# caumente/multi_task_breast_cancer

Hardware: AMD Instinct MI355X
Metric: training images/sec (1-ch 256x256, U-Net++ MT) (higher is better)
Workload: dtype bf16; 1 GPU; MTUNetPlusPlus seg+cls deep-supervision step (Dice+Focal, alpha=0.5, Adam eps 1e-4), per-GPU batch 32, 1x256x256, bf16 MFMA operands (3x3 convs, ConvT) and 16-bit stored conv outputs / activations; fp32 accumulation, gradient sums, statistics, losses, parameters and optimizer, random-init weights (BASELINE.json configs[1]); global_batch=32, parallelism=dp1

## Files before the change

### include/mtbc.h

```cpp
#ifndef MTBC_H
#define MTBC_H

#include <stddef.h>
#include <stdint.h>

#ifdef __cplusplus
extern "C" {
#endif

#define MTBC_VERSION 203
#define MTBC_MAX_SEGS 6
#define MTBC_STEM_MAX_CIN 5

enum {
    MTBC_OK = 0,
    MTBC_E_BADSHAPE = -1,
    MTBC_E_BADARG = -2,
    MTBC_E_WORKSPACE = -3,
    MTBC_E_LAUNCH = -4,
    MTBC_E_UNSUPPORTED = -5
};

int mtbc_version(void);
const char* mtbc_strerror(int code);
// ... 57 lines not shown
size_t mtbc_conv3x3_packed_dgrad_elems(int32_t Cin, int32_t Cout);
int mtbc_conv3x3_pack_fwd(const float* w, float* packed, int32_t Cin, int32_t Cout, void* stream);
int mtbc_conv3x3_pack_dgrad(const float* w, float* packed, int32_t Cin, int32_t Cout, void* stream);
size_t mtbc_conv3x3_packed_lp_elems(int32_t Cin, int32_t Cout, int32_t dgrad);
int mtbc_conv3x3_pack_lp(const float* w, void* packed, int32_t Cin, int32_t Cout, int32_t dgrad, int32_t compute, void* stream);

typedef struct mtbc_pack_desc {
    const float* w;
    void* packed;
    int32_t Cin, Cout;
    int32_t kind, compute;
} mtbc_pack_desc;
int mtbc_conv3x3_pack_many(const mtbc_pack_desc* descs, int32_t n, void* stream);
int32_t mtbc_conv3x3_stats_slots(const mtbc_conv3x3_args* a);
size_t mtbc_conv3x3_wgrad_workspace(const mtbc_conv3x3_args* a);
size_t mtbc_conv3x3_wgrad_sync_bytes(const mtbc_conv3x3_args* a);
int mtbc_conv3x3_kernel_name(const mtbc_conv3x3_args* a, int32_t op, char* buf, int32_t len);
int mtbc_conv3x3_fwd(const mtbc_conv3x3_args* a, void* stream);
int mtbc_conv3x3_dgrad(const mtbc_conv3x3_args* a, void* stream);
int mtbc_conv3x3_wgrad(const mtbc_conv3x3_args* a, void* stream);

typedef struct {
    int32_t N, C, H, W;
    float eps, slope;
    const float* z;
    const float* gamma;
    const float* beta;
    float* y;
    int64_t y_batch_stride;
    float* mean;
    float* rstd;
    const float* dy;
    int64_t dy_batch_stride;
    int32_t n_dy_extra;
    const float* dy_extra[4];
    float* dz;
    float* dgamma;
    float* dbeta;
    float* dbias_pre;
    int32_t accumulate_dparams;
    void* workspace;
    size_t workspace_bytes;
    void* y16;
    void* dz16;
    int32_t out16_type;
    void* y8;
    void* dz8;
    void* coop_state;
    int32_t coop_reserve_cus;
    int32_t z_layout;
    int32_t dy_layout;
    const float* stats_partial;
    int32_t stats_slots;
    int32_t z_type;
    const float* dy_rank1;
    const float* dy_rank1_w;
    float* dy_rank1_dw;
    float* dy_rank1_db;
    int32_t dy_rank1_accumulate;
    const float* dy_pool;
    const void* dy_pool_arg;
    void* pool_y8;
    void* pool_arg;
    int32_t defer_dparams;
} mtbc_instnorm_args;
size_t mtbc_instnorm_coop_state_bytes(void);
size_t mtbc_instnorm_coop_error_offset(void);
int mtbc_instnorm_c8_supported(const mtbc_instnorm_args* a, int32_t backward);
int32_t mtbc_instnorm_bwd_team(const mtbc_instnorm_args* a);
typedef struct mtbc_dparam_desc {
    const float* part;
    float* dgamma;
    float* dbeta;
    float* dbias_pre;
    int32_t N, C, T, accumulate;
} mtbc_dparam_desc;
int mtbc_instnorm_dparam_many(const mtbc_dparam_desc* descs, int32_t n, void* stream);

size_t mtbc_instnorm_fwd_workspace(const mtbc_instnorm_args* a);
int mtbc_instnorm_kernel_name(const mtbc_instnorm_args* a, int32_t backward, char* buf, int32_t len);
int mtbc_instnorm_lrelu_fwd(const mtbc_instnorm_args* a, void* stream);
int mtbc_instnorm_lrelu_bwd(const mtbc_instnorm_args* a, void* stream);

typedef struct {
    int32_t N, C, H, W;
    const float* x;  int64_t x_batch_stride;
    float* y;        int64_t y_batch_stride;
    const float* dy; int64_t dy_batch_stride;
    float* dx;       int64_t dx_batch_stride;
    int32_t accumulate_dx;
    int32_t layout;
    int32_t type16;
    void* argmax;
} mtbc_maxpool_args;

int mtbc_maxpool2_fwd(const mtbc_maxpool_args* a, void* stream);
int mtbc_maxpool2_bwd(const mtbc_maxpool_args* a, void* stream);

typedef struct {
    int32_t N, C, H, W;
    const void* x;   int64_t x_batch_stride;
    void* y;         int64_t y_batch_stride;
    int32_t layout;
    int32_t type16;
    const float* dy; int64_t dy_batch_stride;
    float* dx;       int64_t dx_batch_stride;
    int32_t accumulate_dx;
} mtbc_upsample2_args;
int mtbc_upsample2_fwd(const mtbc_upsample2_args* a, void* stream);
int mtbc_upsample2_bwd(const mtbc_upsample2_args* a, void* stream);

typedef struct {
    int32_t N, H, W, Cin, Cout, k;
    const float* x;  int64_t x_batch_stride;
    const float* w;
    const float* bias;
    float* y;        int64_t y_batch_stride;
    const float* dy; int64_t dy_batch_stride;
    float* dx;       int64_t dx_batch_stride;
    int32_t accumulate_dx;
    float* dw;       float* dbias;
    int32_t accumulate_dw;
    void* workspace; size_t workspace_bytes;
    int32_t compute;
    int32_t y_layout;
    int32_t y_type;
    int32_t x_layout;
    int32_t dy_type16;
    int32_t x_type16;
} mtbc_convT_args;
int mtbc_convT_fwd_c8_supported(const mtbc_convT_args* a);

size_t mtbc_convT_wgrad_workspace(const mtbc_convT_args* a);
int mtbc_convT_fwd(const mtbc_convT_args* a, void* stream);
int mtbc_convT_dgrad(const mtbc_convT_args* a, void* stream);
int mtbc_convT_wgrad(const mtbc_convT_args* a, void* stream);
int mtbc_convT_kernel_name(const mtbc_convT_args* a, int32_t op, const mtbc_convT_args* dgrad_next, char* buf, int32_t len);

typedef struct {
    int32_t N, H, W, Cin, Cout;
    const float* x;  int64_t x_batch_stride;
    const float* w;
    const float* bias;
    float* y;
    const float* dy;
    float* dx;       int64_t dx_batch_stride;
    int32_t accumulate_dx;
    float* dw;       float* dbias;
    int32_t accumulate_dw;
    void* workspace; size_t workspace_bytes;
    int32_t x_layout;
    int32_t x_type;
} mtbc_conv1x1_args;

size_t mtbc_conv1x1_wgrad_workspace(const mtbc_conv1x1_args* a);
int mtbc_conv1x1_fwd(const mtbc_conv1x1_args* a, void* stream);
int mtbc_conv1x1_dgrad(const mtbc_conv1x1_args* a, void* stream);
int mtbc_conv1x1_wgrad(const mtbc_conv1x1_args* a, void* stream);

typedef struct {
    int32_t N, C, H, W;
    const float* x;  float* y;
    const float* dy; float* dx;
} mtbc_gap_args;
int mtbc_gap_fwd(const mtbc_gap_args* a, void* stream);
int mtbc_gap_bwd(const mtbc_gap_args* a, void* stream);
// ... 293 lines not shown
```

### multi_task_breast_cancer_amd/_lib.py

```python
from __future__ import annotations

import ctypes as C
import os
from typing import Optional

_HERE = os.path.dirname(os.path.abspath(__file__))
LIB_PATH = os.environ.get("MTBC_LIB") or os.path.join(_HERE, "libmtbc_hip.so")

MAX_SEGS = 6
STEM_MAX_CIN = 5
c_float_p = C.POINTER(C.c_float)


class MtbcError(RuntimeError):
    pass


LAYOUT_PLANAR, LAYOUT_C8 = 0, 1


class Seg(C.Structure):
    _fields_ = [("ptr", C.c_void_p), ("batch_stride", C.c_int64), ("channels", C.c_int32), ("accumulate", C.c_int32)]


# ... 206 lines not shown
    _fields_ = [("part", C.c_void_p), ("dgamma", C.c_void_p), ("dbeta", C.c_void_p), ("dbias_pre", C.c_void_p),
                ("N", C.c_int32), ("C", C.c_int32), ("T", C.c_int32), ("accumulate", C.c_int32)]


class _SyncArgs(C.Structure):
    _fields_ = [("event", C.c_void_p), ("index", C.c_int32)]


class _WViewArgs(C.Structure):
    _fields_ = [("w", C.c_void_p), ("dst", C.c_void_p), ("Cout", C.c_int32), ("Cin", C.c_int32), ("ci_off", C.c_int32),
                ("ci_cnt", C.c_int32), ("mode", C.c_int32), ("k_off", C.c_int32), ("K", C.c_int32)]


class HeadFuseArgs(C.Structure):
    _fields_ = [("Cin", C.c_int32), ("Cmid", C.c_int32), ("R", C.c_int32), ("k", C.c_int32),
                ("wT", C.c_void_p), ("bT", C.c_void_p), ("w1", C.c_void_p), ("b1", C.c_void_p),
                ("Wc", C.c_void_p), ("bc", C.c_void_p), ("G", C.c_void_p), ("gb", C.c_void_p),
                ("dwT", C.c_void_p), ("dbT", C.c_void_p), ("dw1", C.c_void_p), ("db1", C.c_void_p),
                ("acc_wT", C.c_int32), ("acc_bT", C.c_int32), ("acc_w1", C.c_int32), ("acc_b1", C.c_int32)]


class _OpUnion(C.Union):
    _fields_ = [("conv3", Conv3x3Args), ("inorm", InstNormArgs), ("pool", MaxPoolArgs), ("convT", ConvTArgs),
                ("conv1", Conv1x1Args), ("gap", GapArgs), ("linear", LinearArgs), ("dice", DiceArgs),
                ("focal", FocalArgs), ("optim", OptimArgs), ("pack", _PackArgs), ("mix", _MixArgs),
                ("memset0", _MemsetArgs), ("counts", _CountsArgs), ("head", HeadFuseArgs), ("c8pack", _C8PackArgs), ("wview", _WViewArgs), ("dparam", DparamDesc), ("sync", _SyncArgs),
                ("softmax", SoftmaxArgs), ("up2", Upsample2Args)]


class Op(C.Structure):
    _fields_ = [("kind", C.c_int32), ("tag", C.c_int32), ("u", _OpUnion)]


(OP_CONV3_FWD, OP_CONV3_DGRAD, OP_CONV3_WGRAD, OP_CONV3_PACK_FWD, OP_CONV3_PACK_DGRAD,
 OP_IN_FWD, OP_IN_BWD, OP_POOL_FWD, OP_POOL_BWD, OP_CONVT_FWD, OP_CONVT_DGRAD, OP_CONVT_WGRAD,
 OP_CONV1_FWD, OP_CONV1_DGRAD, OP_CONV1_WGRAD, OP_GAP_FWD, OP_GAP_BWD, OP_LINEAR_FWD, OP_LINEAR_BWD,
 OP_DICE_FWD, OP_DICE_BWD, OP_FOCAL, OP_LOSS_MIX, OP_OPTIM, OP_MEMSET, OP_DICE_COUNTS, OP_CONV3_PACK_LP,
 OP_HEAD_COMBINE, OP_HEAD_EXPAND, OP_C8_PACK, OP_C8_PACK16, OP_CONV3_WVIEW,
 OP_SET_STREAM, OP_EVENT_RECORD, OP_EVENT_WAIT, OP_IN_DPARAM) = range(1, 37)
OP_SOFTMAX = 37
OP_UPSAMPLE2_FWD, OP_UPSAMPLE2_BWD = 38, 39
LINEAR_WIDE_MIN_IN = 4096

OP_UNION_FIELD = {
    OP_CONV3_FWD: "conv3", OP_CONV3_DGRAD: "conv3", OP_CONV3_WGRAD: "conv3",
    OP_CONV3_PACK_FWD: "pack", OP_CONV3_PACK_DGRAD: "pack",
    OP_IN_FWD: "inorm", OP_IN_BWD: "inorm", OP_POOL_FWD: "pool", OP_POOL_BWD: "pool",
    OP_CONVT_FWD: "convT", OP_CONVT_DGRAD: "convT", OP_CONVT_WGRAD: "convT",
    OP_CONV1_FWD: "conv1", OP_CONV1_DGRAD: "conv1", OP_CONV1_WGRAD: "conv1",
    OP_GAP_FWD: "gap", OP_GAP_BWD: "gap", OP_LINEAR_FWD: "linear", OP_LINEAR_BWD: "linear",
    OP_DICE_FWD: "dice", OP_DICE_BWD: "dice", OP_FOCAL: "focal", OP_LOSS_MIX: "mix", OP_OPTIM: "optim",
    OP_MEMSET: "memset0", OP_DICE_COUNTS: "counts", OP_CONV3_PACK_LP: "pack",
    OP_HEAD_COMBINE: "head", OP_HEAD_EXPAND: "head", OP_C8_PACK: "c8pack", OP_C8_PACK16: "c8pack", OP_CONV3_WVIEW: "wview",
    OP_SET_STREAM: "sync", OP_EVENT_RECORD: "sync", OP_EVENT_WAIT: "sync", OP_IN_DPARAM: "dparam",
    OP_SOFTMAX: "softmax", OP_UPSAMPLE2_FWD: "up2", OP_UPSAMPLE2_BWD: "up2",
}

class PackDesc(C.Structure):
    _fields_ = [("w", C.c_void_p), ("packed", C.c_void_p), ("Cin", C.c_int32), ("Cout", C.c_int32),
                ("kind", C.c_int32), ("compute", C.c_int32)]


class WViewDesc(C.Structure):
    _fields_ = [("w", C.c_void_p), ("dst", C.c_void_p), ("Cout", C.c_int32), ("Cin", C.c_int32), ("ci_off", C.c_int32),
                ("ci_cnt", C.c_int32), ("mode", C.c_int32), ("k_off", C.c_int32), ("K", C.c_int32)]


EXPORTS = [
    "mtbc_version", "mtbc_strerror", "mtbc_arch",
    "mtbc_conv3x3_packed_elems", "mtbc_conv3x3_packed_dgrad_elems", "mtbc_conv3x3_pack_fwd",
    "mtbc_conv3x3_pack_dgrad", "mtbc_conv3x3_packed_lp_elems", "mtbc_conv3x3_pack_lp", "mtbc_conv3x3_pack_many", "mtbc_c8_pack", "mtbc_c8_unpack", "mtbc_c8_pack16", "mtbc_conv3x3_weight_view", "mtbc_conv3x3_weight_view_many", "mtbc_augment_flip_rotate", "mtbc_convT_head_combine", "mtbc_convT_head_expand", "mtbc_conv3x3_wgrad_workspace", "mtbc_conv3x3_wgrad_sync_bytes", "mtbc_conv3x3_stats_slots", "mtbc_conv3x3_kernel_name", "mtbc_conv3x3_fwd", "mtbc_conv3x3_dgrad",
    "mtbc_conv3x3_wgrad", "mtbc_instnorm_fwd_workspace", "mtbc_instnorm_coop_state_bytes", "mtbc_instnorm_coop_error_offset", "mtbc_instnorm_c8_supported", "mtbc_instnorm_bwd_team", "mtbc_instnorm_dparam_many", "mtbc_instnorm_kernel_name", "mtbc_instnorm_lrelu_fwd", "mtbc_instnorm_lrelu_bwd", "mtbc_maxpool2_fwd",
    "mtbc_maxpool2_bwd", "mtbc_convT_wgrad_workspace", "mtbc_convT_fwd_c8_supported", "mtbc_convT_kernel_name", "mtbc_convT_fwd", "mtbc_convT_dgrad", "mtbc_convT_wgrad",
    "mtbc_conv1x1_wgrad_workspace", "mtbc_conv1x1_fwd", "mtbc_conv1x1_dgrad", "mtbc_conv1x1_wgrad",
    "mtbc_gap_fwd", "mtbc_gap_bwd", "mtbc_linear_fwd", "mtbc_linear_bwd", "mtbc_dice_fwd", "mtbc_dice_bwd",
    "mtbc_focal_fwd_bwd", "mtbc_loss_mix", "mtbc_loss_scale_begin", "mtbc_loss_scale_check",
    "mtbc_loss_scale_update_host", "mtbc_loss_scale_begin_host", "mtbc_optim_step", "mtbc_optim_dynamic", "mtbc_loss_scale_optim", "mtbc_optim_step_host",
    "mtbc_dice_counts", "mtbc_program_run",
    "mtbc_program_run_ms", "mtbc_event_create", "mtbc_event_destroy", "mtbc_op_kernel_name",
    "mtbc_seg_metrics_workspace_size", "mtbc_seg_metrics", "mtbc_batch_assemble", "mtbc_train_metrics",
    "mtbc_eval_metrics", "mtbc_seg_step_metrics", "mtbc_fill_holes", "mtbc_fill_holes_host",
    "mtbc_softmax_rows", "mtbc_softmax_rows_host", "mtbc_cls_step_metrics", "mtbc_cls_test_rows",
    "mtbc_upsample2_fwd", "mtbc_upsample2_bwd", "mtbc_linear_workspace", "mtbc_linear_wide_enable",
]

ABI_VERSION = 203
_lib: Optional[C.CDLL] = None


def load() -> C.CDLL:
    global _lib
    if _lib is not None:
        return _lib
    if not os.path.exists(LIB_PATH):
        raise MtbcError(
            f"{LIB_PATH} not found: the HIP extension is not built. Run `python -c 'import __graft_entry__ as g; "
            f"g.build()'` (or `make -C multi_task_breast_cancer_amd/csrc`). There is no CPU fallback.")
    import torch
    lib = C.CDLL(LIB_PATH)
    lib.mtbc_version.restype = C.c_int
    if lib.mtbc_version() != ABI_VERSION:
        raise MtbcError(f"{LIB_PATH} reports ABI version {lib.mtbc_version()}, this binding is written for {ABI_VERSION}: rebuild "
                        f"(`make -C multi_task_breast_cancer_amd/csrc`)")
    lib.mtbc_strerror.restype = C.c_char_p
    lib.mtbc_strerror.argtypes = [C.c_int]
    lib.mtbc_arch.restype = C.c_char_p
    for name in ("mtbc_conv3x3_packed_elems", "mtbc_conv3x3_packed_dgrad_elems"):
        getattr(lib, name).restype = C.c_size_t
        getattr(lib, name).argtypes = [C.c_int32, C.c_int32]
    lib.mtbc_conv3x3_packed_lp_elems.restype = C.c_size_t
    lib.mtbc_conv3x3_packed_lp_elems.argtypes = [C.c_int32, C.c_int32, C.c_int32]
    for _n in ("mtbc_convT_head_combine", "mtbc_convT_head_expand"):
        getattr(lib, _n).restype = C.c_int
        getattr(lib, _n).argtypes = [C.POINTER(HeadFuseArgs), C.c_void_p]
    lib.mtbc_conv3x3_stats_slots.restype = C.c_int32
    lib.mtbc_conv3x3_stats_slots.argtypes = [C.POINTER(Conv3x3Args)]
    lib.mtbc_conv3x3_kernel_name.restype = C.c_int
    lib.mtbc_conv3x3_kernel_name.argtypes = [C.POINTER(Conv3x3Args), C.c_int32, C.c_char_p, C.c_int32]
    lib.mtbc_instnorm_kernel_name.restype = C.c_int
    lib.mtbc_instnorm_kernel_name.argtypes = [C.POINTER(InstNormArgs), C.c_int32, C.c_char_p, C.c_int32]
    lib.mtbc_convT_kernel_name.restype = C.c_int
    lib.mtbc_convT_kernel_name.argtypes = [C.POINTER(ConvTArgs), C.c_int32, C.POINTER(ConvTArgs), C.c_char_p, C.c_int32]
    lib.mtbc_instnorm_fwd_workspace.restype = C.c_size_t
    lib.mtbc_instnorm_fwd_workspace.argtypes = [C.POINTER(InstNormArgs)]
    lib.mtbc_augment_flip_rotate.restype = C.c_int
    lib.mtbc_augment_flip_rotate.argtypes = [C.c_void_p, C.c_void_p, C.c_void_p, C.c_int32, C.c_int32, C.c_int32, C.c_int32, C.c_void_p]
    lib.mtbc_conv3x3_pack_many.restype = C.c_int
    lib.mtbc_conv3x3_pack_many.argtypes = [C.POINTER(PackDesc), C.c_int32, C.c_void_p]
    lib.mtbc_c8_pack.restype = C.c_int
    lib.mtbc_c8_pack.argtypes = [C.c_void_p, C.c_int64, C.c_void_p, C.c_int32, C.c_int32, C.c_int32, C.c_int32, C.c_void_p]
    lib.mtbc_conv3x3_weight_view.restype = C.c_int
    lib.mtbc_conv3x3_weight_view.argtypes = [C.c_void_p, C.c_void_p] + [C.c_int32] * 7 + [C.c_void_p]
    lib.mtbc_conv3x3_weight_view_many.restype = C.c_int
    lib.mtbc_conv3x3_weight_view_many.argtypes = [C.POINTER(WViewDesc), C.c_int32, C.c_void_p]
    lib.mtbc_c8_pack16.restype = C.c_int
    lib.mtbc_c8_pack16.argtypes = [C.c_void_p, C.c_int64, C.c_void_p, C.c_int32, C.c_int32, C.c_int32, C.c_void_p]
    lib.mtbc_c8_unpack.restype = C.c_int
    lib.mtbc_c8_unpack.argtypes = [C.c_void_p, C.c_void_p, C.c_int32, C.c_int32, C.c_int32, C.c_int32, C.c_void_p]
    lib.mtbc_conv3x3_pack_lp.restype = C.c_int
    lib.mtbc_conv3x3_pack_lp.argtypes = [C.c_void_p, C.c_void_p, C.c_int32, C.c_int32, C.c_int32, C.c_int32, C.c_void_p]
    for name in ("mtbc_conv3x3_pack_fwd", "mtbc_conv3x3_pack_dgrad"):
        getattr(lib, name).restype = C.c_int
        getattr(lib, name).argtypes = [C.c_void_p, C.c_void_p, C.c_int32, C.c_int32, C.c_void_p]
    for name, typ in (("mtbc_conv3x3_wgrad_workspace", Conv3x3Args), ("mtbc_conv3x3_wgrad_sync_bytes", Conv3x3Args), ("mtbc_convT_wgrad_workspace", ConvTArgs),
                      ("mtbc_conv1x1_wgrad_workspace", Conv1x1Args)):
        getattr(lib, name).restype = C.c_size_t
        getattr(lib, name).argtypes = [C.POINTER(typ)]
    for name, typ in (("mtbc_conv3x3_fwd", Conv3x3Args), ("mtbc_conv3x3_dgrad", Conv3x3Args),
                      ("mtbc_conv3x3_wgrad", Conv3x3Args), ("mtbc_instnorm_lrelu_fwd", InstNormArgs),
                      ("mtbc_instnorm_lrelu_bwd", InstNormArgs), ("mtbc_maxpool2_fwd", MaxPoolArgs),
                      ("mtbc_maxpool2_bwd", MaxPoolArgs), ("mtbc_convT_fwd", ConvTArgs),
                      ("mtbc_convT_dgrad", ConvTArgs), ("mtbc_convT_wgrad", ConvTArgs),
                      ("mtbc_conv1x1_fwd", Conv1x1Args), ("mtbc_conv1x1_dgrad", Conv1x1Args),
                      ("mtbc_conv1x1_wgrad", Conv1x1Args), ("mtbc_gap_fwd", GapArgs), ("mtbc_gap_bwd", GapArgs),
                      ("mtbc_linear_fwd", LinearArgs), ("mtbc_linear_bwd", LinearArgs),
                      ("mtbc_dice_fwd", DiceArgs), ("mtbc_dice_bwd", DiceArgs), ("mtbc_focal_fwd_bwd", FocalArgs)):
        getattr(lib, name).restype = C.c_int
        getattr(lib, name).argtypes = [C.POINTER(typ), C.c_void_p]
    lib.mtbc_instnorm_coop_state_bytes.restype = C.c_size_t
    lib.mtbc_instnorm_coop_state_bytes.argtypes = []
    lib.mtbc_instnorm_coop_error_offset.restype = C.c_size_t
    lib.mtbc_instnorm_coop_error_offset.argtypes = []
    lib.mtbc_instnorm_bwd_team.restype = C.c_int32
    lib.mtbc_instnorm_bwd_team.argtypes = [C.POINTER(InstNormArgs)]
    lib.mtbc_instnorm_dparam_many.restype = C.c_int
    lib.mtbc_instnorm_dparam_many.argtypes = [C.POINTER(DparamDesc), C.c_int32, C.c_void_p]
    lib.mtbc_instnorm_c8_supported.restype = C.c_int
    lib.mtbc_instnorm_c8_supported.argtypes = [C.POINTER(InstNormArgs), C.c_int32]
    lib.mtbc_convT_fwd_c8_supported.restype = C.c_int
    lib.mtbc_convT_fwd_c8_supported.argtypes = [C.POINTER(ConvTArgs)]
    lib.mtbc_loss_mix.restype = C.c_int
    lib.mtbc_loss_mix.argtypes = [C.c_void_p, C.c_void_p, C.c_float, C.c_void_p, C.c_void_p]
    lib.mtbc_dice_counts.restype = C.c_int
    lib.mtbc_dice_counts.argtypes = [C.c_void_p, C.c_void_p, C.c_int64, C.c_void_p, C.c_void_p]
    for name in ("mtbc_loss_scale_begin", "mtbc_loss_scale_check"):
        getattr(lib, name).restype = C.c_int
        getattr(lib, name).argtypes = [C.POINTER(LossScaleArgs), C.c_void_p]
    for name in ("mtbc_loss_scale_update_host", "mtbc_loss_scale_begin_host"):
        getattr(lib, name).restype = C.c_int
        getattr(lib, name).argtypes = [C.POINTER(LossScaleArgs)]
    lib.mtbc_optim_step.restype = C.c_int
    lib.mtbc_optim_step.argtypes = [C.POINTER(OptimArgs), C.c_void_p]
    lib.mtbc_optim_dynamic.restype = C.c_int
    lib.mtbc_optim_dynamic.argtypes = [C.POINTER(OptimArgs), C.POINTER(C.c_float * 4)]
    lib.mtbc_loss_scale_optim.restype = C.c_int
    lib.mtbc_loss_scale_optim.argtypes = [C.POINTER(LossScaleArgs), C.POINTER(OptimArgs), C.c_void_p]
    lib.mtbc_optim_step_host.restype = C.c_int
    lib.mtbc_optim_step_host.argtypes = [C.POINTER(OptimArgs)]
    lib.mtbc_program_run.restype = C.c_int
    lib.mtbc_program_run.argtypes = [C.POINTER(Op), C.c_int32, C.c_int32, C.c_void_p, C.POINTER(C.c_int32)]
    lib.mtbc_program_run_ms.restype = C.c_int
    lib.mtbc_program_run_ms.argtypes = [C.POINTER(Op), C.c_int32, C.c_int32, C.POINTER(C.c_void_p), C.c_int32, C.POINTER(C.c_int32)]
    lib.mtbc_event_create.restype = C.c_int
    lib.mtbc_event_create.argtypes = [C.POINTER(C.c_void_p)]
    lib.mtbc_event_destroy.restype = C.c_int
    lib.mtbc_event_destroy.argtypes = [C.c_void_p]
    lib.mtbc_op_kernel_name.restype = C.c_int
    lib.mtbc_op_kernel_name.argtypes = [C.POINTER(Op), C.c_char_p, C.c_int32]
    lib.mtbc_seg_metrics_workspace_size.restype = C.c_size_t
# ... 50 lines not shown
```

### multi_task_breast_cancer_amd/csrc/common.h

```cpp
#pragma once
#include <hip/hip_runtime.h>
#include <stdint.h>
#include <stdlib.h>
#include "../../include/mtbc.h"

#define MTBC_WAVE 64

typedef float f32x4 __attribute__((ext_vector_type(4)));

#define MTBC_CHECK_LAUNCH()                                   \
    do {                                                      \
        hipError_t e__ = hipGetLastError();                   \
        if (e__ != hipSuccess) return MTBC_E_LAUNCH;          \
    } while (0)

#ifdef MTBC_PROBES
#include <stdlib.h>
static inline int mtbc_probe_int(const char* name, int dflt) { const char* v = getenv(name); return v ? atoi(v) : dflt; }
static inline bool mtbc_probe_set(const char* name) { return getenv(name) != nullptr; }
#define MTBC_DBG_BIT(p, bit) ((p).dbg & (bit))
#else
#define mtbc_probe_int(name, dflt) (dflt)
#define mtbc_probe_set(name) (false)
#define MTBC_DBG_BIT(p, bit) (0)
// ... 45 lines not shown
        t->ptr[i] = nullptr; t->bstride[i] = 0; t->accumulate[i] = 0; t->cbegin[i] = c;
        if (i < n) {
            if (!segs[i].ptr || segs[i].channels <= 0) return MTBC_E_BADARG;
            t->ptr[i] = segs[i].ptr; t->bstride[i] = segs[i].batch_stride;
            t->accumulate[i] = segs[i].accumulate;
            c += segs[i].channels;
        }
    }
    t->cbegin[MTBC_MAX_SEGS] = c;
    for (int i = n; i <= MTBC_MAX_SEGS; ++i) t->cbegin[i] = c;
    t->n = n;
    return c == expect_channels ? MTBC_OK : MTBC_E_BADSHAPE;
}

struct SegRef { float* ptr; long long bs; int cb; int acc; };
__device__ __forceinline__ SegRef seg_ref(const SegTable& t, int c) {
    SegRef r{t.ptr[0], t.bstride[0], 0, t.accumulate[0]};
#pragma unroll
    for (int i = 1; i < MTBC_MAX_SEGS; ++i) {
        const bool hit = i < t.n && c >= t.cbegin[i];
        r.ptr = hit ? t.ptr[i] : r.ptr;
        r.bs = hit ? t.bstride[i] : r.bs;
        r.cb = hit ? t.cbegin[i] : r.cb;
        r.acc = hit ? t.accumulate[i] : r.acc;
    }
    return r;
}

__device__ __forceinline__ float wave_sum(float v) {
#pragma unroll
    for (int o = 32; o > 0; o >>= 1) v += __shfl_xor(v, o, 64);
    return v;
}
__device__ __forceinline__ double wave_sum_d(double v) {
#pragma unroll
    for (int o = 32; o > 0; o >>= 1) v += __shfl_xor(v, o, 64);
    return v;
}

__host__ __device__ __forceinline__ float sigmoidf_(float v) { return 1.0f / (1.0f + expf(-v)); }

__device__ __forceinline__ bool flip_rotate_src(int x, int y, int H, int W, float ca, float sa, bool fh, bool fv, int& xs, int& ys) {
    const float xo = (float)x - 0.5f * (float)W + 0.5f, yo = (float)y - 0.5f * (float)H + 0.5f;
    const float hw = 0.5f * (float)W, hh = 0.5f * (float)H;
    const float gx = fmaf(yo, -sa / hw, xo * (ca / hw));
    const float gy = fmaf(yo, ca / hh, xo * (sa / hh));
    const float ix = ((gx + 1.f) * (float)W - 1.f) * 0.5f, iy = ((gy + 1.f) * (float)H - 1.f) * 0.5f;
    const float rx = nearbyintf(ix), ry = nearbyintf(iy);
    const bool inb = rx >= 0.f && rx < (float)W && ry >= 0.f && ry < (float)H;
    xs = inb ? (int)rx : 0; ys = inb ? (int)ry : 0;
    if (fh) xs = W - 1 - xs;
    if (fv) ys = H - 1 - ys;
    return inb;
}

__device__ __forceinline__ float block_sum(float v, float* red) {
    const int lane = threadIdx.x & 63, wid = threadIdx.x >> 6, nw = (blockDim.x + 63) >> 6;
    v = wave_sum(v);
    __syncthreads();
    if (lane == 0) red[wid] = v;
    __syncthreads();
    float s = 0.f;
    for (int i = 0; i < nw; ++i) s += red[i];
    return s;
}

enum NormKernel {
    NK_FWD_C8, NK_BWD_C8,
    NK_STATS_FIN, NK_APPLY_FWD, NK_BSTATS_FIN, NK_APPLY_BWD,
    NK_R1_FIN, NK_DPARAM,
    NK_FWD_REG, NK_CHUNK_STATS, NK_CHUNK_APPLY, NK_FWD_STREAM, NK_BWD, NK_BWD_REG
};
struct NormLaunch { int k; int t[6]; int threads; int T, rounds; };
struct NormChoice {
    static constexpr int MAX = 4;
    int n; NormLaunch l[MAX];
    void add(int k, int t0 = 0, int t1 = 0, int t2 = 0, int t3 = 0, int t4 = 0, int t5 = 0) { if (n == MAX) abort(); l[n++] = NormLaunch{k, {t0, t1, t2, t3, t4, t5}, 0, 0, 0}; }
    void add(const NormLaunch& k) { if (n == MAX) abort(); l[n++] = k; }
    NormLaunch& last() { return l[n - 1]; }
};
extern "C" int mtbc_i_instnorm_fwd_c8(const mtbc_instnorm_args* a, hipStream_t st, NormChoice* query);
extern "C" int mtbc_i_instnorm_bwd_c8(const mtbc_instnorm_args* a, float* part, hipStream_t st, NormChoice* query);
extern "C" int mtbc_i_instnorm_bwd_c8_team(const mtbc_instnorm_args* a);
#include <stdarg.h>
#include <stdio.h>
struct OpChoice {
    int n, len; char s[512];
    void add(const char* fmt, ...) __attribute__((format(printf, 2, 3))) {
        if (n++ && len < (int)sizeof s - 4) { s[len++] = ' '; s[len++] = '+'; s[len++] = ' '; }
        va_list ap; va_start(ap, fmt);
        const int w = vsnprintf(s + len, sizeof s - len, fmt, ap);
        va_end(ap);
        if (w < 0 || w >= (int)sizeof s - len) abort();
        len += w;
    }
};
static inline const char* mtbc_tf(bool b) { return b ? "true" : "false"; }
int mtbc_i_maxpool_c8_fwd(const mtbc_maxpool_args* a, hipStream_t st, OpChoice* query);
int mtbc_i_maxpool_c8_bwd(const mtbc_maxpool_args* a, hipStream_t st, OpChoice* query);
int mtbc_i_conv1x1_c8_fwd(const mtbc_conv1x1_args* a, hipStream_t st, OpChoice* query);
size_t mtbc_i_conv1x1_c8_wgrad_workspace(const mtbc_conv1x1_args* a);
int mtbc_i_conv1x1_c8_wgrad(const mtbc_conv1x1_args* a, hipStream_t st, OpChoice* query);
int mtbc_i_maxpool2_fwd(const mtbc_maxpool_args* a, hipStream_t st, OpChoice* query);
int mtbc_i_maxpool2_bwd(const mtbc_maxpool_args* a, hipStream_t st, OpChoice* query);
int mtbc_i_upsample2_fwd(const mtbc_upsample2_args* a, hipStream_t st, OpChoice* query);
int mtbc_i_upsample2_bwd(const mtbc_upsample2_args* a, hipStream_t st, OpChoice* query);
int mtbc_i_conv1x1_fwd(const mtbc_conv1x1_args* a, hipStream_t st, OpChoice* query);
int mtbc_i_conv1x1_dgrad(const mtbc_conv1x1_args* a, hipStream_t st, OpChoice* query);
int mtbc_i_conv1x1_wgrad(const mtbc_conv1x1_args* a, hipStream_t st, OpChoice* query);
int mtbc_i_head_combine(const mtbc_head_fuse_args* a, hipStream_t st, OpChoice* query);
int mtbc_i_head_expand(const mtbc_head_fuse_args* a, hipStream_t st, OpChoice* query);
int mtbc_i_gap_fwd(const mtbc_gap_args* a, hipStream_t st, OpChoice* query);
int mtbc_i_gap_bwd(const mtbc_gap_args* a, hipStream_t st, OpChoice* query);
int mtbc_i_linear_fwd(const mtbc_linear_args* a, hipStream_t st, OpChoice* query);
int mtbc_i_linear_bwd(const mtbc_linear_args* a, hipStream_t st, OpChoice* query);
int mtbc_i_splitk_reduce(const float* partial, float* out, int nsplit, size_t elems, int accumulate, hipStream_t st);
int mtbc_i_splitk_reduce2(const float* partial, float* out, float* out2, int nsplit, size_t elems1, size_t elems2, int accumulate, hipStream_t st, OpChoice* query = nullptr);
enum ConvTKernel {
    CTK_FWD_LP_C8, CTK_FWD_C8, CTK_FWD_LDS,
    CTK_DGRAD_LDS, CTK_DGRAD2,
    CTK_WGRAD16, CTK_WGRAD2, CTK_BWD_FUSED,
    CTK_FWD, CTK_DGRAD, CTK_WGRAD,
    CTK_SPLITK, CTK_CHANNEL_SUMS
};
struct ConvTLaunch { int k; int t[4]; int xcd, splits; };
struct ConvTChoice {
    static constexpr int MAX = 4;
    int n; ConvTLaunch l[MAX];
    void add(int k, int t0 = 0, int t1 = 0, int t2 = 0, int t3 = 0) { if (n == MAX) abort(); l[n++] = ConvTLaunch{k, {t0, t1, t2, t3}, 0, 0}; }
    void add(const ConvTLaunch& k) { if (n == MAX) abort(); l[n++] = k; }
    ConvTLaunch& last() { return l[n - 1]; }
};
bool mtbc_i_convT2_fwd_ok(const mtbc_convT_args* a);
int mtbc_i_convT2_fwd(const mtbc_convT_args* a, hipStream_t st, ConvTChoice* query);
bool mtbc_i_convT2_fwd_c8_ok(const mtbc_convT_args* a);
int mtbc_i_convT2_fwd_c8(const mtbc_convT_args* a, hipStream_t st, ConvTChoice* query);
bool mtbc_i_convT2_fwd_lp_c8_ok(const mtbc_convT_args* a);
int mtbc_i_convT2_fwd_lp_c8(const mtbc_convT_args* a, hipStream_t st, ConvTChoice* query);
bool mtbc_i_convT2_dgrad_ok(const mtbc_convT_args* a);
bool mtbc_i_convT2_wgrad_ok(const mtbc_convT_args* a);
void mtbc_i_convT2_wgrad_plan(const mtbc_convT_args* a, int* steps_per_split, int* nsplit);
int mtbc_i_convT2_dgrad(const mtbc_convT_args* a, int compute, hipStream_t st, ConvTChoice* query);
int mtbc_i_convT2_wgrad(const mtbc_convT_args* a, int compute, float* partial, float* dbias_part, int steps_per_split, int nsplit, hipStream_t st, ConvTChoice* query);
bool mtbc_i_convT2_bwd_fused_ok(const mtbc_convT_args* wg, const mtbc_convT_args* dg);
int mtbc_i_convT2_bwd_fused(const mtbc_convT_args* wg, const mtbc_convT_args* dg, float* partial, float* dbias_part, int steps_per_split, int nsplit, hipStream_t st, ConvTChoice* query);
int mtbc_i_convT_bwd_pair(const mtbc_convT_args* wg, const mtbc_convT_args* dg, void* stream, bool* fused, ConvTChoice* query = nullptr);
int mtbc_i_channel_sums(const float* x, float* planes_ws, float* out, int N, int C, int HW, int accumulate, hipStream_t st, OpChoice* query = nullptr);
```

### multi_task_breast_cancer_amd/csrc/conv3x3.hip

```cpp
#include "common.h"
#include <type_traits>
#include <utility>
#include <cstdlib>
#include <cstdio>
#include <cstring>

namespace {

__device__ __forceinline__ void pack_fwd_elem(const float* __restrict__ w, float* __restrict__ p, int Cin, int Cout, int idx) {
    int i = idx & 15, tap = (idx >> 4) % 9, ci = (idx / 144) % Cin, mt = idx / (144 * Cin);
    int co = mt * 16 + i;
    p[idx] = co < Cout ? w[((size_t)co * Cin + ci) * 9 + tap] : 0.f;
}
__device__ __forceinline__ void pack_dgrad_elem(const float* __restrict__ w, float* __restrict__ p, int Cin, int Cout, int idx) {
    int i = idx & 15, tap = (idx >> 4) % 9, co = (idx / 144) % Cout, mt = idx / (144 * Cout);
    int ci = mt * 16 + i;
    p[idx] = ci < Cin ? w[((size_t)co * Cin + ci) * 9 + (8 - tap)] : 0.f;
}
__global__ void pack_fwd_kernel(const float* __restrict__ w, float* __restrict__ p, int Cin, int Cout, int total) {
    int idx = blockIdx.x * blockDim.x + threadIdx.x;
    if (idx < total) pack_fwd_elem(w, p, Cin, Cout, idx);
}
__global__ void pack_dgrad_kernel(const float* __restrict__ w, float* __restrict__ p, int Cin, int Cout, int total) {
    int idx = blockIdx.x * blockDim.x + threadIdx.x;
// ... 727 lines not shown
                        const unsigned voff = ok ? (unsigned)((((mt0 + mt) * nchunks + ch) * (9 * 16 * WROW / 8) + r) * 16) : 0xfffffff0u;
                        if (idx < W16)
                            __builtin_amdgcn_raw_ptr_buffer_load_lds(wrsrc, (lds_ptr_t)(Ws + inst * 512), 16, voff, 0, 0, 0);
                    }
                }
                w_have = ch;
            }
#pragma unroll
            for (int q = 0; q < XQ; ++q) {
                const int hp = lane + 64 * q;
                if (hp < HP) *reinterpret_cast<typename T::frag*>(Xs + hp * LPROW + 8 * wvu) = T::pack(xf[q]);
            }
            bool fetched = false;
            if (ch + 1 < nchunks) { fetch_x(ch + 1); fetched = true; }
            else if (tile + tstep < tend) { tile_geom(tile + tstep); fetch_x(0); fetched = true; }
            if (wload) {
                if (fetched) wait_vmcnt<8 * XQ>(); else wait_vmcnt<0>();
            }
            lds_barrier();
#pragma unroll
            for (int tap = 0; tap < 9; ++tap) {
                const int toff = ((tap / 3) * HC + tap % 3) * LPROW + 8 * kg;
                typename T::frag a[MT], b[4];
#pragma unroll
                for (int m = 0; m < MT; ++m)
                    a[m] = *reinterpret_cast<const typename T::frag*>(Ws + ((m * 9 + tap) * 16 + j) * WROW + 8 * (kg ^ ((j >> 1) & 3)));
#pragma unroll
                for (int g = 0; g < 4; ++g)
                    b[g] = *reinterpret_cast<const typename T::frag*>(Xs + bpix[g] * LPROW + toff);
#pragma unroll
                for (int m = 0; m < MT; ++m)
#pragma unroll
                    for (int g = 0; g < 4; ++g) acc[m][g] = T::mfma(b[g], a[m], acc[m][g]);
            }
        }
        const int n = GEO == 2 ? n0 + wv : n0;
        if MTBC_DBG_BIT(p, 2) { if (acc[0][0][0] != 12345.678f) continue; }
        int poff[4];
#pragma unroll
        for (int g = 0; g < 4; ++g) {
            int y, x;
            if (GEO == 0) { y = y0 + 2 * wv + (g >> 1); x = x0 + 16 * (g & 1) + 4 * kg; }
            else if (GEO == 1) { y = y0 + 4 * wv + g; x = x0 + 4 * kg; }
            else { y = y0 + 2 * g + (kg >> 1); x = x0 + 4 * (kg & 1); }
            poff[g] = (n < p.N && y < p.H && x < p.W) ? y * p.W + x : -1;
        }
#pragma unroll
        for (int m = 0; m < MT; ++m) {
            const int co = (mt0 + m) * 16 + j;
            if (co >= p.Cout) continue;
            const SegL so = segl_ref(seg_out, co);
            gfloat* cb = (gfloat*)so.ptr + (size_t)n * so.bs + (size_t)(co - so.cb) * HW;
            const float bv = bias_s[m * 16 + j];
            if (so.acc) {
                f32x4 old[4];
#pragma unroll
                for (int g = 0; g < 4; ++g) old[g] = poff[g] >= 0 ? *(const gf32x4*)(cb + poff[g]) : (f32x4){0.f, 0.f, 0.f, 0.f};
#pragma unroll
                for (int g = 0; g < 4; ++g)
                    if (poff[g] >= 0) *(gf32x4*)(cb + poff[g]) = old[g] + (acc[m][g] + bv);
            } else {
#pragma unroll
                for (int g = 0; g < 4; ++g)
                    if (poff[g] >= 0) *(gf32x4*)(cb + poff[g]) = acc[m][g] + bv;
            }
        }
    }
}

__device__ __forceinline__ float row16_sum(float v) {
    v += __builtin_bit_cast(float, __builtin_amdgcn_update_dpp(0, __builtin_bit_cast(int, v), 0x118, 0xf, 0xf, true));
    v += __builtin_bit_cast(float, __builtin_amdgcn_update_dpp(0, __builtin_bit_cast(int, v), 0x114, 0xf, 0xf, true));
    v += __builtin_bit_cast(float, __builtin_amdgcn_update_dpp(0, __builtin_bit_cast(int, v), 0x112, 0xf, 0xf, true));
    v += __builtin_bit_cast(float, __builtin_amdgcn_update_dpp(0, __builtin_bit_cast(int, v), 0x111, 0xf, 0xf, true));
    return v;
}

__device__ __forceinline__ float wave_sum_rows(float v) {
    const int r = __builtin_bit_cast(int, row16_sum(v));
    return ((__builtin_bit_cast(float, __builtin_amdgcn_readlane(r, 15)) + __builtin_bit_cast(float, __builtin_amdgcn_readlane(r, 31))) +
            __builtin_bit_cast(float, __builtin_amdgcn_readlane(r, 47))) + __builtin_bit_cast(float, __builtin_amdgcn_readlane(r, 63));
}

template <int MT, int GEO, bool F16, int NW, int O8, bool FULL, typename ZPRE>
__device__ __forceinline__ void c8_epilogue(const ConvP& p, f32x4 (&acc)[MT][4], const SegL* seg_out, const float* bias_s, const int n0,
                                            const int y0, const int x0, const int tx, const int ty, const int mt0, const int wv,
                                            const int j, const int kg, const int HW, ZPRE& zpre) {
    using T = LP<F16>;
    using TO = LP<F16 || O8 == 3>;
    typedef unsigned pre_u32x2 __attribute__((ext_vector_type(2)));
    const int n = GEO == 2 ? n0 + wv : n0;
    if MTBC_DBG_BIT(p, 2) { if (acc[0][0][0] != 12345.678f) return; }
    if constexpr (O8 != 0) {
        typedef unsigned ep_u32x2 __attribute__((ext_vector_type(2)));
        typedef unsigned ep_u32x4 __attribute__((ext_vector_type(4)));
        typedef __attribute__((address_space(1))) ep_u32x2 guint2;
        int pix[4];
#pragma unroll
        for (int g = 0; g < 4; ++g) {
            int y, x;
            if (GEO == 0) { y = y0 + 2 * wv + (g >> 1); x = x0 + 16 * (g & 1) + j; }
            else if (GEO == 1) { y = y0 + 4 * wv + g; x = x0 + j; }
            else { y = y0 + 2 * g + (j >> 3); x = x0 + (j & 7); }
            pix[g] = (FULL || (n < p.N && y < p.H && x < p.W)) ? y * p.W + x : -1;
        }
        const bool want_stats = O8 == 2 || p.stats != nullptr;
#pragma unroll
        for (int m = 0; m < MT; ++m) {
            const int co = (mt0 + m) * 16 + 4 * kg;
            if (co >= p.Cout) continue;
            const SegL so = segl_ref_n(seg_out, co, p.out.n);
            const size_t poff8 = 2 * ((size_t)n * so.bs + (size_t)((co - so.cb) >> 3) * HW * 8) + 2 * ((co - so.cb) & 7);
            gchar* cb = (gchar*)so.ptr + poff8;
            const f32x4 bv = *reinterpret_cast<const f32x4*>(bias_s + m * 16 + 4 * kg);
            f32x4 ss = (f32x4){0.f, 0.f, 0.f, 0.f}, sq = (f32x4){0.f, 0.f, 0.f, 0.f};
            if constexpr (O8 == 2) {
                const size_t plane = (size_t)n * p.Cout + co;
                f32x4 mean4 = (f32x4){0.f, 0.f, 0.f, 0.f}, rstd4 = mean4, ga4 = (f32x4){1.f, 1.f, 1.f, 1.f}, be4 = mean4;
                if (n < p.N) { mean4 = *reinterpret_cast<const f32x4*>(p.nmean + plane); rstd4 = *reinterpret_cast<const f32x4*>(p.nrstd + plane); }
                if (p.ngamma) { ga4 = *reinterpret_cast<const f32x4*>(p.ngamma + co); be4 = *reinterpret_cast<const f32x4*>(p.nbeta + co); }
                const float* eb = p.extra ? p.extra + plane * HW : nullptr;
#pragma unroll
                for (int g = 0; g < 4; ++g)
                    if (FULL || pix[g] >= 0) {
                        const pre_u32x2 zw = zpre[m][g];
                        f32x4 ex = (f32x4){0.f, 0.f, 0.f, 0.f};
                        if (eb) ex = (f32x4){eb[pix[g]], eb[(size_t)HW + pix[g]], eb[2 * (size_t)HW + pix[g]], eb[3 * (size_t)HW + pix[g]]};
                        const f32x4 r = acc[m][g] + ex;
                        const float q[8] = {r[0], r[1], r[2], r[3], 0.f, 0.f, 0.f, 0.f};
                        const ep_u32x4 u = __builtin_bit_cast(ep_u32x4, T::pack(q));
                        *(guint2*)(cb + 16 * (size_t)pix[g]) = (ep_u32x2){u[0], u[1]};
                        const unsigned u0 = u[0], u1 = u[1], z0 = zw[0], z1 = zw[1];
                        const f32x4 dyv = (f32x4){T::lo(u0), T::hi(u0), T::lo(u1), T::hi(u1)};
                        const f32x4 xh = ((f32x4){T::lo(z0), T::hi(z0), T::lo(z1), T::hi(z1)} - mean4) * rstd4;
                        const f32x4 pre = xh * ga4 + be4;
                        f32x4 gg;
#pragma unroll
                        for (int e = 0; e < 4; ++e) gg[e] = dyv[e] * (pre[e] > 0.f ? 1.f : p.nslope);
                        ss += gg; sq += gg * xh;
                    }
            } else {
#pragma unroll
                for (int g = 0; g < 4; ++g)
                    if (FULL || pix[g] >= 0) {
                        f32x4 r = acc[m][g] + bv;
                        if constexpr (O8 == 3) {
#pragma unroll
                            for (int e = 0; e < 4; ++e) r[e] = __builtin_amdgcn_fmed3f(r[e], -65504.f, 65504.f);
                        }
                        const float q[8] = {r[0], r[1], r[2], r[3], 0.f, 0.f, 0.f, 0.f};
                        const ep_u32x4 u = __builtin_bit_cast(ep_u32x4, TO::pack(q));
                        *(guint2*)(cb + 16 * (size_t)pix[g]) = (ep_u32x2){u[0], u[1]};
                        if (p.stats) {
                            const unsigned u0 = u[0], u1 = u[1];
                            const f32x4 v = (f32x4){TO::lo(u0), TO::hi(u0), TO::lo(u1), TO::hi(u1)};
                            ss += v; sq += v * v;
                        }
                    }
            }
            if (want_stats) {
#pragma unroll
                for (int e = 0; e < 4; ++e) { ss[e] = row16_sum(ss[e]); sq[e] = row16_sum(sq[e]); }
                if (j == 15 && (FULL || n < p.N)) {
                    const int slots = GEO == 2 ? 1 : p.tiles_x * p.tiles_y * NW;
                    const int slot = GEO == 2 ? 0 : (ty * p.tiles_x + tx) * NW + wv;
                    float* sp = p.stats + (((size_t)n * slots + slot) * p.Cout + co) * 2;
                    *reinterpret_cast<f32x4*>(sp) = (f32x4){ss[0], sq[0], ss[1], sq[1]};
                    *reinterpret_cast<f32x4*>(sp + 4) = (f32x4){ss[2], sq[2], ss[3], sq[3]};
                }
            }
        }
        return;
    }
    int poff[4];
#pragma unroll
    for (int g = 0; g < 4; ++g) {
        int y, x;
        if (GEO == 0) { y = y0 + 2 * wv + (g >> 1); x = x0 + 16 * (g & 1) + 4 * kg; }
        else if (GEO == 1) { y = y0 + 4 * wv + g; x = x0 + 4 * kg; }
        else { y = y0 + 2 * g + (kg >> 1); x = x0 + 4 * (kg & 1); }
        poff[g] = (FULL || (n < p.N && y < p.H && x < p.W)) ? y * p.W + x : -1;
    }
#pragma unroll
    for (int m = 0; m < MT; ++m) {
        const int co = (mt0 + m) * 16 + j;
        if (co >= p.Cout) continue;
        const SegL so = segl_ref_n(seg_out, co, p.out.n);
        gfloat* cb = (gfloat*)so.ptr + (size_t)n * so.bs + (size_t)(co - so.cb) * HW;
        const float bv = bias_s[m * 16 + j];
        if (so.acc == 2) {
            typedef unsigned ep_u32x2 __attribute__((ext_vector_type(2)));
            typedef unsigned ep_u32x4 __attribute__((ext_vector_type(4)));
            typedef __attribute__((address_space(1))) ep_u32x2 guint2;
            gchar* c16 = (gchar*)so.ptr + 2 * ((size_t)n * so.bs + (size_t)(co - so.cb) * HW);
#pragma unroll
            for (int g = 0; g < 4; ++g)
                if (FULL || poff[g] >= 0) {
                    const float q[8] = {acc[m][g][0] + bv, acc[m][g][1] + bv, acc[m][g][2] + bv, acc[m][g][3] + bv, 0.f, 0.f, 0.f, 0.f};
                    const typename T::frag h = T::pack(q);
                    const ep_u32x4 u = __builtin_bit_cast(ep_u32x4, h);
                    *(guint2*)(c16 + 2 * (size_t)poff[g]) = (ep_u32x2){u[0], u[1]};
                }
        } else if (so.acc) {
            f32x4 old[4];
#pragma unroll
            for (int g = 0; g < 4; ++g) old[g] = (FULL || poff[g] >= 0) ? *(const gf32x4*)(cb + poff[g]) : (f32x4){0.f, 0.f, 0.f, 0.f};
#pragma unroll
            for (int g = 0; g < 4; ++g)
                if (FULL || poff[g] >= 0) *(gf32x4*)(cb + poff[g]) = old[g] + (acc[m][g] + bv);
        } else {
#pragma unroll
            for (int g = 0; g < 4; ++g)
                if (FULL || poff[g] >= 0) *(gf32x4*)(cb + poff[g]) = acc[m][g] + bv;
        }
    }
}

template <int GEO> __device__ __forceinline__ constexpr int c8_goff(int g, int HC) { return GEO == 0 ? (g >> 1) * HC + 16 * (g & 1) : GEO == 1 ? g * HC : 2 * g * HC; }

template <int MT, int GEO, bool F16, int NW, int O8>
__global__ __launch_bounds__(64 * NW, NW == 4 ? 3 : 4) void conv3x3_igemm_c8_kernel(const ConvP p) {
    using G = GeoLP<GEO>;
    using T = LP<F16>;
    static_assert(NW == 4 || (NW == 8 && GEO == 0), "8-wave blocks: wide-map geometry only");
    constexpr int TH = GEO == 0 ? 2 * NW : G::TH;
    constexpr int HR = TH + 2, HC = G::TW + 2, HP = G::IMG * HR * HC;
    constexpr int HPP = (HP + 15) / 16 * 16;
    constexpr int XB = 4 * HPP * 8;
    constexpr int WB = MT * 9 * 16 * WROW;
    constexpr int XQ = (HPP + 63) / 64;
    constexpr int XPW = NW == 4 ? XQ : (XQ + 1) / 2;
    extern __shared__ __attribute__((aligned(16))) unsigned short smem16[];
    unsigned short* Xs = smem16;
    unsigned short* Ws = smem16 + XB;
    SegL* seg_in = reinterpret_cast<SegL*>(smem16 + XB + WB);
    SegL* seg_out = seg_in + MTBC_MAX_SEGS;
    float* bias_s = reinterpret_cast<float*>(seg_out + MTBC_MAX_SEGS);
    const int tid = threadIdx.x, lane = tid & 63, wv = tid >> 6;
    const int wvu = __builtin_amdgcn_readfirstlane(tid >> 6);
    const int HW = p.H * p.W;
    const int mt0 = blockIdx.y * MT;
    float bias_v = 0.f;
    if (tid < MT * 16) { const int co = mt0 * 16 + tid; if (p.bias && co < p.Cout) bias_v = p.bias[co]; }
    segl_fill(seg_in, p.in);
    segl_fill(seg_out, p.out);

    const int nchunks = (p.Cin + LPKC - 1) / LPKC;
    const int j = lane & 15, kg = lane >> 4;
    int bpix0;
    if (GEO == 0) bpix0 = (2 * wvu) * HC + j;
    else if (GEO == 1) bpix0 = (4 * wvu) * HC + j;
    else bpix0 = (wvu * HR + (j >> 3)) * HC + (j & 7);
    const unsigned short* const xlane = Xs + (kg * HPP + bpix0) * 8;
    int w_have = -1;
    constexpr int W16 = WB / 8, WI = (W16 + 63) / 64, WK = (WI + NW - 1) / NW;
    const __amdgpu_buffer_rsrc_t wrsrc = __builtin_amdgcn_make_buffer_rsrc(
        const_cast<float*>(p.wp), 0, (int)((size_t)p.mtiles * nchunks * (9 * 16 * WROW) * 2), 0x00020000);
    unsigned wvoff[WK];
#pragma unroll
    for (int k = 0; k < WK; ++k) {
        const int inst = wvu + NW * k, idx = inst * 64 + lane;
        const int mt = idx / (9 * 16 * WROW / 8), r = idx % (9 * 16 * WROW / 8);
        const bool ok = inst < WI && idx < W16 && (mt0 + mt) < p.mtiles;
        wvoff[k] = ok ? (unsigned)(((mt0 + mt) * nchunks * (9 * 16 * WROW / 8) + r) * 16) : 0xfffffff0u;
    }
    int tile, tstep, tend;
    if ((gridDim.x & 7) == 0 && !MTBC_DBG_BIT(p, 16)) {
        const int per = (p.ntiles + 7) >> 3, xcd = blockIdx.x & 7;
        tile = xcd * per + (blockIdx.x >> 3); tstep = gridDim.x >> 3; tend = min(p.ntiles, (xcd + 1) * per);
    } else { tile = blockIdx.x; tstep = gridDim.x; tend = p.ntiles; }
    const int xgrp_w = NW == 4 ? wvu : (wvu >> 1), xq0 = NW == 4 ? 0 : (wvu & 1) * XPW;
    int hrc[XPW];
#pragma unroll
    for (int q = 0; q < XPW; ++q) {
        const int hp = lane + 64 * (xq0 + q);
        const int img = hp / (HR * HC), rem = hp % (HR * HC);
        hrc[q] = (hp < HP && !MTBC_DBG_BIT(p, 1)) ? ((img << 20) | ((rem / HC) << 10) | (rem % HC)) : -1;
    }
    const int txs = (p.tiles_x & (p.tiles_x - 1)) == 0 ? __builtin_ctz(p.tiles_x) : -1;
    const int tys = (p.tiles_y & (p.tiles_y - 1)) == 0 ? __builtin_ctz(p.tiles_y) : -1;
    int tsk = 0;
    if (tid < MT * 16) bias_s[tid] = bias_v;
    __syncthreads();
    for (; tile < tend; tile += tstep) {
        int t = tile, tx, ty;
        if (txs >= 0 && tys >= 0) { tx = t & (p.tiles_x - 1); t >>= txs; ty = t & (p.tiles_y - 1); t >>= tys; }
        else { tx = t % p.tiles_x; t /= p.tiles_x; ty = t % p.tiles_y; t /= p.tiles_y; }
        const int n0 = t * G::IMG, x0 = tx * G::TW, y0 = ty * TH;
        if (tsk < 3) MTBC_TS(p, 4 * tsk);
        unsigned pixo[XPW];
        int pimg[XPW];
#pragma unroll
        for (int q = 0; q < XPW; ++q) {
            const int rc = hrc[q];
            const int img = G::IMG > 1 ? (rc >> 20) : 0;
            const int y = y0 + ((rc >> 10) & 1023) - 1, x = x0 + (rc & 1023) - 1;
            const bool ok = rc >= 0 && (G::IMG == 1 || n0 + img < p.N) && (unsigned)y < (unsigned)p.H && (unsigned)x < (unsigned)p.W;
            pixo[q] = ok ? 16u * (unsigned)(y * p.W + x) : 0xfffffff0u;
            pimg[q] = ok ? img : 0;
        }
        f32x4 acc[MT][4];
#pragma unroll
        for (int m = 0; m < MT; ++m)
#pragma unroll
            for (int g = 0; g < 4; ++g) acc[m][g] = (f32x4){0.f, 0.f, 0.f, 0.f};
        typedef unsigned pre_u32x2 __attribute__((ext_vector_type(2)));
        typedef __attribute__((address_space(1))) pre_u32x2 gpre2;
        pre_u32x2 zpre[O8 == 2 ? MT : 1][4];
        if constexpr (O8 == 2) {
            const int nn = GEO == 2 ? n0 + wvu : n0;
#pragma unroll
            for (int g = 0; g < 4; ++g) {
                int y, x;
                if (GEO == 0) { y = y0 + 2 * wvu + (g >> 1); x = x0 + 16 * (g & 1) + j; }
                else if (GEO == 1) { y = y0 + 4 * wvu + g; x = x0 + j; }
                else { y = y0 + 2 * g + (j >> 3); x = x0 + (j & 7); }
                const bool ok = nn < p.N && y < p.H && x < p.W;
#pragma unroll
                for (int m = 0; m < MT; ++m) {
                    const int co = (mt0 + m) * 16 + 4 * kg;
                    zpre[m][g] = (pre_u32x2){0u, 0u};
                    if (ok && co < p.Cout)
                        zpre[m][g] = *(const gpre2*)((const gchar*)p.nz + 2 * ((size_t)nn * p.Cout * HW + (size_t)(co >> 3) * HW * 8) + 2 * (co & 7) + 16 * (size_t)(y * p.W + x));
                }
            }
        }

        for (int ch = 0; ch < nchunks; ++ch) {
            lds_barrier();
            {
                const int c0 = ch * LPKC + 8 * xgrp_w;
                const bool xgrp = c0 < p.Cin;
                const SegL sr = segl_ref_n(seg_in, xgrp ? c0 : 0, p.in.n);
                const unsigned long long pu = reinterpret_cast<unsigned long long>(sr.ptr);
                const unsigned plo = __builtin_amdgcn_readfirstlane((unsigned)pu), phi = __builtin_amdgcn_readfirstlane((unsigned)(pu >> 32));
                const unsigned blo = __builtin_amdgcn_readfirstlane((unsigned)sr.bs), bhi = __builtin_amdgcn_readfirstlane((unsigned)((unsigned long long)sr.bs >> 32));
                const int cb = __builtin_amdgcn_readfirstlane(sr.cb);
                const long long bs = (long long)(((unsigned long long)bhi << 32) | blo);
                unsigned short* base = reinterpret_cast<unsigned short*>(((unsigned long long)phi << 32) | plo) +
                                       ((size_t)n0 * bs + (size_t)((xgrp ? c0 : 0) - cb) * HW);
                const unsigned span = (G::IMG > 1 ? (unsigned)((G::IMG - 1) * bs) * 2u : 0u) + (unsigned)HW * 16u;
                const __amdgpu_buffer_rsrc_t xrsrc = __builtin_amdgcn_make_buffer_rsrc(base, 0, xgrp ? (int)span : 0, 0x00020000);
#pragma unroll
                for (int q = 0; q < XPW; ++q) {
                    unsigned off = pixo[q];
                    if (G::IMG > 1) off += 2u * (unsigned)(pimg[q] * bs);
                    if (xq0 + q < XQ && lane + 64 * (xq0 + q) < HPP)
                        __builtin_amdgcn_raw_ptr_buffer_load_lds(xrsrc, (lds_ptr_t)(Xs + (xgrp_w * HPP + 64 * (xq0 + q)) * 8), 16, off, 0, 0, 0);
                }
            }
            if (w_have != ch && !MTBC_DBG_BIT(p, 8)) {
                const int adv = ch * (9 * 16 * WROW * 2);
#pragma unroll
                for (int k = 0; k < WK; ++k) {
                    const int inst = wvu + NW * k;
                    if (inst < WI && inst * 64 + lane < W16)
                        __builtin_amdgcn_raw_ptr_buffer_load_lds(wrsrc, (lds_ptr_t)(Ws + inst * 512), 16, (int)wvoff[k], adv, 0, 0);
                }
                w_have = ch;
            }
            if (ch == 0 && tsk < 3) MTBC_TS(p, 4 * tsk + 1);
            asm volatile("s_waitcnt vmcnt(0)\n\ts_barrier" ::: "memory");
            if (ch == 0 && tsk < 3) MTBC_TS(p, 4 * tsk + 2);
#pragma unroll
            for (int tap = 0; tap < 9; ++tap) {
                const int toff = (tap / 3) * HC + tap % 3;
                typename T::frag a[MT], b[4];
#pragma unroll
                for (int m = 0; m < MT; ++m)
                    a[m] = *reinterpret_cast<const typename T::frag*>(Ws + ((m * 9 + tap) * 16 + j) * WROW + 8 * (kg ^ ((j >> 1) & 3)));
#pragma unroll
                for (int g = 0; g < 4; ++g)
                    b[g] = *reinterpret_cast<const typename T::frag*>(xlane + (c8_goff<GEO>(g, HC) + toff) * 8);
#pragma unroll
                for (int m = 0; m < MT; ++m)
#pragma unroll
                    for (int g = 0; g < 4; ++g) {
                        if constexpr (O8 != 0) acc[m][g] = T::mfma(a[m], b[g], acc[m][g]);
                        else acc[m][g] = T::mfma(b[g], a[m], acc[m][g]);
                    }
            }
        }
        if (tsk < 3) MTBC_TS(p, 4 * tsk + 3);
        if (n0 + G::IMG <= p.N && y0 + TH <= p.H && x0 + G::TW <= p.W) c8_epilogue<MT, GEO, F16, NW, O8, true>(p, acc, seg_out, bias_s, n0, y0, x0, tx, ty, mt0, wvu, j, kg, HW, zpre);
        else c8_epilogue<MT, GEO, F16, NW, O8, false>(p, acc, seg_out, bias_s, n0, y0, x0, tx, ty, mt0, wvu, j, kg, HW, zpre);
        if (tsk < 3) MTBC_TS(p, 12 + tsk);
        ++tsk;
    }
}

typedef int i32x4 __attribute__((ext_vector_type(4)));
__device__ __forceinline__ i32x4 dma_rsrc(const void* base, unsigned bytes) {
    const unsigned long long a = reinterpret_cast<unsigned long long>(base);
    return (i32x4){(int)(unsigned)a, (int)((unsigned)(a >> 32) & 0xffffu), (int)bytes, 0x00020000};
}
__device__ __forceinline__ unsigned lds_addr(const void* p) { return (unsigned)(unsigned long long)(__attribute__((address_space(3))) const void*)p; }
__device__ __forceinline__ void dma16(const i32x4 rsrc, unsigned lds, unsigned voff) {
    asm volatile("s_mov_b32 m0, %0\n\ts_nop 0\n\tbuffer_load_dwordx4 %1, %2, 0 offen lds" ::"s"(lds), "v"(voff), "s"(rsrc) : "memory", "m0");
}
template <typename F, int... I> __device__ __forceinline__ void sfor_c_impl(F&& f, std::integer_sequence<int, I...>) { (f(std::integral_constant<int, I>{}), ...); }
template <int N, typename F> __device__ __forceinline__ void sfor_c(F&& f) { sfor_c_impl(f, std::make_integer_sequence<int, N>{}); }
template <int MT, int GEO> struct RingGeo {
    using G = GeoLP<GEO>;
    static constexpr int HR = G::TH + 2, HC = G::TW + 2, HP = HR * HC, HPP = (HP + 15) / 16 * 16;
    static constexpr int XB = 4 * HPP * 8, WB = MT * 9 * 16 * WROW, PAD = 512;
    static constexpr int XQ = (HPP + 63) / 64, W16 = WB / 8, WI = (W16 + 63) / 64, WPW = (WI + 3) / 4;
    static constexpr int CNT = XQ + WPW;
    static constexpr int SLOT = XB + WB + PAD;
};
template <int MT, int GEO, bool F16, int O8, int R>
__global__ __launch_bounds__(256, 1) void conv3x3_igemm_c8_ring_kernel(const ConvP p) {
    using G = GeoLP<GEO>;
    using T = LP<F16>;
    using RG = RingGeo<MT, GEO>;
    static_assert(GEO != 2 && (O8 == 0 || O8 == 1 || O8 == 3) && R >= 2 && R <= 3, "wide / 16-wide maps, plain epilogues");
    constexpr int NW = 4, TH = G::TH, HR = RG::HR, HC = RG::HC, HP = RG::HP, HPP = RG::HPP, XB = RG::XB, WB = RG::WB, XQ = RG::XQ;
    extern __shared__ __attribute__((aligned(16))) unsigned short smem16[];
    SegL* seg_in = reinterpret_cast<SegL*>(smem16 + R * RG::SLOT);
    SegL* seg_out = seg_in + MTBC_MAX_SEGS;
    float* bias_s = reinterpret_cast<float*>(seg_out + MTBC_MAX_SEGS);
    unsigned long long* xbase_s = reinterpret_cast<unsigned long long*>(bias_s + MT * 16);
    const int tid = threadIdx.x, lane = tid & 63, wv = tid >> 6;
    const int wvu = __builtin_amdgcn_readfirstlane(tid >> 6);
    const int HW = p.H * p.W;
    const int mt0 = blockIdx.y * MT;
    MTBC_TS(p, 0);
    float bias_v = 0.f;
    if (tid < MT * 16) { const int co = mt0 * 16 + tid; if (p.bias && co < p.Cout) bias_v = p.bias[co]; }
    segl_fill(seg_in, p.in);
    segl_fill(seg_out, p.out);
    lds_barrier();
    MTBC_TS(p, 1);

    const int nchunks = (p.Cin + LPKC - 1) / LPKC;
    const int j = lane & 15, kg = lane >> 4;
    const int bpix0 = (GEO == 0 ? 2 * wv : 4 * wv) * HC + j;
    constexpr int WPW = RG::WPW, CNT = RG::CNT;
    const unsigned lds0 = lds_addr(smem16);
    const unsigned wbytes = (unsigned)((size_t)p.mtiles * nchunks * (9 * 16 * WROW) * 2);
    unsigned wvoff[WPW];
#pragma unroll
    for (int k = 0; k < WPW; ++k) {
        const int inst = wvu + NW * k, idx = inst * 64 + lane;
        const int mt = idx / (9 * 16 * WROW / 8), r = idx % (9 * 16 * WROW / 8);
        const bool ok = inst < RG::WI && idx < RG::W16 && (mt0 + mt) < p.mtiles;
        wvoff[k] = ok ? (unsigned)(((mt0 + mt) * nchunks * (9 * 16 * WROW / 8) + r) * 16) : 0xfffffff0u;
    }
    static_assert(RG::W16 % 64 == 0, "whole weight instructions: every wave issues CNT instructions per chunk");
    for (int tile = blockIdx.x; tile < p.ntiles; tile += gridDim.x) {
        int t = tile;
        const int tx = t % p.tiles_x; t /= p.tiles_x;
        const int ty = t % p.tiles_y; t /= p.tiles_y;
        const int n0 = t, x0 = tx * G::TW, y0 = ty * TH;
        unsigned pixo[XQ];
#pragma unroll
        for (int q = 0; q < XQ; ++q) {
            const int hp = lane + 64 * q;
            const int row = hp / HC, col = hp % HC;
            const int y = y0 + row - 1, x = x0 + col - 1;
            const bool ok = hp < HP && y >= 0 && y < p.H && x >= 0 && x < p.W;
            pixo[q] = ok ? 16u * (unsigned)(y * p.W + x) : 0xfffffff0u;
        }
        f32x4 acc[MT][4];
#pragma unroll
        for (int m = 0; m < MT; ++m)
#pragma unroll
            for (int g = 0; g < 4; ++g) acc[m][g] = (f32x4){0.f, 0.f, 0.f, 0.f};
        if (tid < 4 * nchunks) {
            const int c0 = (tid >> 2) * LPKC + 8 * (tid & 3);
            unsigned long long b = 0;
            if (c0 < p.Cin) {
                const SegL sr = segl_ref(seg_in, c0);
                b = reinterpret_cast<unsigned long long>(reinterpret_cast<unsigned short*>(sr.ptr) + ((size_t)n0 * sr.bs + (size_t)(c0 - sr.cb) * HW));
            }
            xbase_s[tid] = b;
        }
        if (tid < MT * 16) bias_s[tid] = bias_v;
        lds_barrier();
        auto chunk_rsrc = [&](int c, i32x4& xr, i32x4& wr) {
            const unsigned long long b = xbase_s[4 * c + wvu];
            const unsigned lo = __builtin_amdgcn_readfirstlane((unsigned)b), hi = __builtin_amdgcn_readfirstlane((unsigned)(b >> 32));
            xr = (i32x4){(int)lo, (int)(hi & 0xffffu), (lo | hi) ? (int)((unsigned)HW * 16u) : 0, 0x00020000};
            const unsigned adv = (unsigned)c * (unsigned)(9 * 16 * WROW * 2);
            wr = dma_rsrc(reinterpret_cast<const char*>(p.wp) + adv, wbytes - adv);
        };
        auto piece = [&](auto i_, int sl, const i32x4& xr, const i32x4& wr) {
            constexpr int i = decltype(i_)::value;
            const unsigned slot0 = lds0 + 2u * (unsigned)(sl * RG::SLOT);
            if constexpr (i < XQ) {
                if (lane + 64 * i < HPP) dma16(xr, slot0 + 2u * (unsigned)((wvu * HPP + 64 * i) * 8), pixo[i]);
            } else {
                constexpr int k = i - XQ;
                const int inst = wvu + NW * k;
                dma16(wr, slot0 + 2u * (unsigned)(XB + (inst < RG::WI ? inst * 512 : WB)), wvoff[k]);
            }
        };
#pragma unroll
        for (int s0 = 0; s0 < R - 1; ++s0)
            if (s0 < nchunks) {
                i32x4 xr, wr;
                chunk_rsrc(s0, xr, wr);
                sfor_c<CNT>([&](auto I) { piece(I, s0, xr, wr); });
            }
        MTBC_TS(p, 2);
        for (int ch = 0; ch < nchunks; ++ch) {
            const int rem = min(R - 2, nchunks - 1 - ch);
            if (rem >= 1) asm volatile("s_waitcnt vmcnt(%0)" ::"n"(RG::CNT) : "memory");
            else asm volatile("s_waitcnt vmcnt(0)" ::: "memory");
            asm volatile("s_waitcnt lgkmcnt(0)\n\ts_barrier" ::: "memory");
            if (ch == 0) MTBC_TS(p, 3);
            if (ch == 1) MTBC_TS(p, 4);
            if (ch == nchunks - 1) MTBC_TS(p, 5);
            const bool more = ch + R - 1 < nchunks;
            const int sl_next = (ch + R - 1) % R;
            i32x4 xr_n = (i32x4){0, 0, 0, 0}, wr_n = xr_n;
            if (more) chunk_rsrc(ch + R - 1, xr_n, wr_n);
            const unsigned short* Xs = smem16 + (ch % R) * RG::SLOT;
            const unsigned short* Ws = Xs + XB;
            typename T::frag fa[2][MT], fb[2][4];
            auto load_tap = [&](int tap, int set) {
                const int toff = (tap / 3) * HC + tap % 3;
#pragma unroll
                for (int m = 0; m < MT; ++m)
                    fa[set][m] = *reinterpret_cast<const typename T::frag*>(Ws + ((m * 9 + tap) * 16 + j) * WROW + 8 * (kg ^ ((j >> 1) & 3)));
#pragma unroll
                for (int g = 0; g < 4; ++g)
                    fb[set][g] = *reinterpret_cast<const typename T::frag*>(Xs + (kg * HPP + bpix0) * 8 + (c8_goff<GEO>(g, HC) + toff) * 8);
            };
            load_tap(0, 0);
            constexpr int PPS = (CNT + 9 * MT - 1) / (9 * MT);
            sfor_c<9>([&](auto TAP) {
                constexpr int tap = decltype(TAP)::value, set = tap & 1;
                if (tap + 1 < 9) load_tap(tap + 1, set ^ 1);
                __builtin_amdgcn_sched_barrier(0);
                sfor_c<MT>([&](auto M) {
                    constexpr int m = decltype(M)::value;
#pragma unroll
                    for (int g = 0; g < 4; ++g) {
                        if constexpr (O8 != 0) acc[m][g] = T::mfma(fa[set][m], fb[set][g], acc[m][g]);
                        else acc[m][g] = T::mfma(fb[set][g], fa[set][m], acc[m][g]);
                    }
                    __builtin_amdgcn_sched_barrier(0);
                    if (more)
                        sfor_c<PPS>([&](auto U) {
                            constexpr int i = (tap * MT + m) * PPS + decltype(U)::value;
                            if constexpr (i < CNT) piece(std::integral_constant<int, i>{}, sl_next, xr_n, wr_n);
                        });
                    __builtin_amdgcn_sched_barrier(0);
                });
            });
        }
        int zpre = 0;
        MTBC_TS(p, 6);
        if (y0 + TH <= p.H && x0 + G::TW <= p.W) c8_epilogue<MT, GEO, F16, NW, O8, true>(p, acc, seg_out, bias_s, n0, y0, x0, tx, ty, mt0, wvu, j, kg, HW, zpre);
        else c8_epilogue<MT, GEO, F16, NW, O8, false>(p, acc, seg_out, bias_s, n0, y0, x0, tx, ty, mt0, wvu, j, kg, HW, zpre);
        MTBC_TS(p, 7);
        asm volatile("s_waitcnt vmcnt(0)" ::: "memory");
        MTBC_TS(p, 8);
    }
}

template <int GEO> struct WGeo;
template <> struct WGeo<0> { static constexpr int TH = 4, TW = 32, ROWS = 6, LW = 40, IMG = 1, IMGS = 240, PSX = 258; };
template <> struct WGeo<1> { static constexpr int TH = 8, TW = 16, ROWS = 10, LW = 24, IMG = 1, IMGS = 240, PSX = 258; };
template <> struct WGeo<2> { static constexpr int TH = 8, TW = 8, ROWS = 10, LW = 16, IMG = 2, IMGS = 160, PSX = 322; };
constexpr int PSZ = 130;

struct WgP {
    int N, H, W, Cin, Cout;
    SegTable in;
    const float* dz;
    float* partial;
    int tiles_x, tiles_y, total_tiles, tiles_per_split;
    int ciblocks;
    int dbg;
#ifdef MTBC_PROBES
    unsigned long long* ts;
#endif
};

template <int GEO, int COT, bool PACK>
__global__ __launch_bounds__(128 * COT, 3) void conv3x3_wgrad_mfma_kernel(const WgP p) {
    using G = WGeo<GEO>;
    constexpr int XS = 32 * G::PSX;
    constexpr int XF4_PER_CH = G::IMG * G::ROWS * G::LW / 4;
    constexpr int XSLOTS = (XF4_PER_CH + 7) / 8;
    extern __shared__ __attribute__((aligned(16))) float smem[];
    float* Xs = smem;
    float* Zs = smem + XS;

    const int tid = threadIdx.x, lane = tid & 63, wv = tid >> 6;
    const int HW = p.H * p.W;
    constexpr int CIB = PACK ? 24 : 32, NTW = PACK ? 7 : 9;
    const int co0 = (blockIdx.y / p.ciblocks) * (16 * COT), ci0 = (blockIdx.y % p.ciblocks) * CIB;
    const int split = blockIdx.x;
    const int t_begin = split * p.tiles_per_split;
    const int t_end = min(p.total_tiles, t_begin + p.tiles_per_split);

    const int ch = tid >> 3, q = tid & 7;
    const int my_ci = ci0 + ch, my_co = co0 + ch;
    const bool ci_ok = ch < CIB && my_ci < p.Cin, co_ok = my_co < p.Cout;
    const SegRef sr = seg_ref(p.in, ci_ok ? my_ci : 0);
    const float* xplane = sr.ptr + (size_t)((ci_ok ? my_ci : 0) - sr.cb) * HW;
    const long long xbs = sr.bs;
    const float* zplane = p.dz + (size_t)(co_ok ? my_co : 0) * HW;
    float4 xr[XSLOTS], zr[4];
    unsigned live = 0;
    unsigned slots_ok = 0;
    if (G::IMG == 1) {
#pragma unroll
        for (int s = 0; s < XSLOTS; ++s) slots_ok |= (q + 8 * s < XF4_PER_CH && ci_ok) ? (1u << s) : 0u;
#pragma unroll
        for (int s = 0; s < 4; ++s) slots_ok |= co_ok ? (1u << (XSLOTS + s)) : 0u;
    }

    auto prefetch = [&](int tile) {
        int t = tile;
        const int tx = t % p.tiles_x; t /= p.tiles_x;
        const int ty = t % p.tiles_y; t /= p.tiles_y;
        const int n0 = t * G::IMG, x0 = tx * G::TW, y0 = ty * G::TH;
        if (G::IMG == 1) {
            const bool interior = y0 >= 1 && y0 + G::TH + 1 <= p.H && x0 >= 4 && x0 + G::TW + 4 <= p.W && !MTBC_DBG_BIT(p, 1);
            if (interior) {
                live = slots_ok;
                int qq = q;
                asm volatile("" : "+v"(qq));
                const long long xo = (long long)((size_t)n0 * xbs) + y0 * p.W + x0, zo = (long long)((size_t)n0 * p.Cout * HW) + y0 * p.W + x0;
#pragma unroll
                for (int s = 0; s < XSLOTS; ++s) {
                    const int f = qq + 8 * s, row = f / (G::LW / 4), c4 = f % (G::LW / 4);
                    long long off = ((slots_ok >> s) & 1u) ? xo + ((row - 1) * p.W + (c4 * 4 - 4)) : 0;
                    asm volatile("" : "+v"(off));
                    xr[s] = *reinterpret_cast<const float4*>(xplane + off);
                }
#pragma unroll
                for (int s = 0; s < 4; ++s) {
                    const int px = (qq + 8 * s) * 4;
                    long long off = co_ok ? zo + ((px / G::TW) * p.W + px % G::TW) : 0;
// ... 1784 lines not shown
    MTBC_ENSURE_DYN_LDS((&conv3x3_igemm_lp_kernel<MT, GEO, false>), 160 * 1024);
    MTBC_ENSURE_DYN_LDS((&conv3x3_igemm_lp_kernel<MT, GEO, true>), 160 * 1024);
    const int per_cu = lds * 3 <= 160 * 1024 ? 3 : 2;
    int gx = (256 * per_cu / mblocks) / 8 * 8;
    if (gx < 8) gx = 8;
    if (gx > p.ntiles) gx = p.ntiles;
    const dim3 grid(gx, mblocks);
    if (f16) hipLaunchKernelGGL((conv3x3_igemm_lp_kernel<MT, GEO, true>), grid, dim3(256), lds, st, p);
    else hipLaunchKernelGGL((conv3x3_igemm_lp_kernel<MT, GEO, false>), grid, dim3(256), lds, st, p);
    MTBC_CHECK_LAUNCH();
    return MTBC_OK;
}
template <int GEO>
int launch_igemm_lp_mt(int MT, const ConvP& p, int mblocks, bool f16, hipStream_t st) {
    switch (MT) {
        case 1: return launch_igemm_lp<1, GEO>(p, mblocks, f16, st);
        case 2: return launch_igemm_lp<2, GEO>(p, mblocks, f16, st);
        default: return launch_igemm_lp<3, GEO>(p, mblocks, f16, st);
    }
}

template <int MT, int GEO, int NW, int O8>
int launch_igemm_c8(const ConvP& p, int mblocks, bool f16, hipStream_t st) {
    using G = GeoLP<GEO>;
    constexpr int TH = GEO == 0 ? 2 * NW : G::TH;
    constexpr int HP = G::IMG * (TH + 2) * (G::TW + 2), HPP = (HP + 15) / 16 * 16;
    const size_t lds = ((size_t)4 * HPP * 8 + (size_t)MT * 9 * 16 * WROW) * 2 + (SEGL_FLOATS + MT * 16) * sizeof(float);
    MTBC_ENSURE_DYN_LDS((&conv3x3_igemm_c8_kernel<MT, GEO, false, NW, O8>), 160 * 1024);
    MTBC_ENSURE_DYN_LDS((&conv3x3_igemm_c8_kernel<MT, GEO, true, NW, O8>), 160 * 1024);
    static const int per_cu_env = mtbc_probe_int("MTBC_C8_BLOCKS_PER_CU", 0);
    const int per_cu = per_cu_env ? per_cu_env : (NW == 8 ? 2 : (lds * 3 <= 160 * 1024 ? 3 : 2));
    int gx = (256 * per_cu / mblocks) / 8 * 8;
    if (gx < 8) gx = 8;
    if (gx > p.ntiles) gx = p.ntiles;
    const dim3 grid(gx, mblocks);
#ifdef MTBC_PROBES
    static const int ts_env = mtbc_probe_int("MTBC_C8_TS", 0);
    if (ts_env && (size_t)gx * mblocks <= 4096) {
        ConvP q = p;
        const size_t nb = (size_t)gx * mblocks;
        static unsigned long long* dts = nullptr;
        if (!dts) (void)hipMalloc(&dts, 4096 * 16 * sizeof(unsigned long long));
        (void)hipMemsetAsync(dts, 0, nb * 16 * sizeof(unsigned long long), st);
        q.ts = dts;
        if (f16) hipLaunchKernelGGL((conv3x3_igemm_c8_kernel<MT, GEO, true, NW, O8>), grid, dim3(64 * NW), lds, st, q);
        else hipLaunchKernelGGL((conv3x3_igemm_c8_kernel<MT, GEO, false, NW, O8>), grid, dim3(64 * NW), lds, st, q);
        (void)hipStreamSynchronize(st);
        static unsigned long long hts[4096 * 16];
        (void)hipMemcpy(hts, dts, nb * 16 * sizeof(unsigned long long), hipMemcpyDeviceToHost);
        unsigned long long t0 = ~0ull;
        for (size_t b = 0; b < nb; ++b) if (hts[b * 16] && hts[b * 16] < t0) t0 = hts[b * 16];
        double mean[15] = {0}; int cnt[15] = {0};
        for (size_t b = 0; b < nb; ++b)
            for (int k = 0; k < 15; ++k) if (hts[b * 16 + k]) { mean[k] += (double)(hts[b * 16 + k] - t0) * 0.01; ++cnt[k]; }
        for (int k = 0; k < 15; ++k) if (cnt[k]) mean[k] /= cnt[k];
        fprintf(stderr, "c8_ts %d->%d @%dx%d MT%d NW%d O8=%d blocks %zu tiles %d | mean us since the first block's start:", p.Cin, p.Cout, p.H, p.W, MT, NW, O8, nb, p.ntiles);
        for (int k = 0; k < 3; ++k)
            fprintf(stderr, "  tile%d: start %.2f issued %.2f landed %.2f mfma done %.2f epilogue done %.2f", k, mean[4 * k], mean[4 * k + 1], mean[4 * k + 2], mean[4 * k + 3], mean[12 + k]);
        fprintf(stderr, "\n");
        return MTBC_OK;
    }
#endif
    if (f16) hipLaunchKernelGGL((conv3x3_igemm_c8_kernel<MT, GEO, true, NW, O8>), grid, dim3(64 * NW), lds, st, p);
    else hipLaunchKernelGGL((conv3x3_igemm_c8_kernel<MT, GEO, false, NW, O8>), grid, dim3(64 * NW), lds, st, p);
    MTBC_CHECK_LAUNCH();
    return MTBC_OK;
}
template <int GEO, int O8>
int launch_igemm_c8_mt(int MT, const ConvP& p, int mblocks, bool f16, hipStream_t st) {
    if (MT == 1) return launch_igemm_c8<1, GEO, 4, O8>(p, mblocks, f16, st);
    if (MT == 3) return launch_igemm_c8<3, GEO, 4, O8>(p, mblocks, f16, st);
    return launch_igemm_c8<2, GEO, 4, O8>(p, mblocks, f16, st);
}
template <int GEO>
int launch_igemm_c8_o8(int MT, int O8, const ConvP& p, int mblocks, bool f16, hipStream_t st) {
    switch (O8) {
        case 0: return launch_igemm_c8_mt<GEO, 0>(MT, p, mblocks, f16, st);
        case 1: return launch_igemm_c8_mt<GEO, 1>(MT, p, mblocks, f16, st);
        case 2: return launch_igemm_c8_mt<GEO, 2>(MT, p, mblocks, f16, st);
        default: return launch_igemm_c8_mt<GEO, 3>(MT, p, mblocks, f16, st);
    }
}

template <int MT, int GEO, int O8>
int launch_igemm_c8_ring(const ConvP& p, int mblocks, bool f16, hipStream_t st) {
    constexpr int R = 3;
    using RG = RingGeo<MT, GEO>;
    const size_t lds = (size_t)R * RG::SLOT * 2 + (SEGL_FLOATS + MT * 16) * sizeof(float) + 64 * 4 * sizeof(unsigned long long);
    static_assert((size_t)R * RG::SLOT * 2 + (SEGL_FLOATS + MT * 16) * sizeof(float) + 2048 <= 160 * 1024, "ring slots + tables must fit a CU's LDS");
    MTBC_ENSURE_DYN_LDS((&conv3x3_igemm_c8_ring_kernel<MT, GEO, false, O8, R>), 160 * 1024);
    MTBC_ENSURE_DYN_LDS((&conv3x3_igemm_c8_ring_kernel<MT, GEO, true, O8, R>), 160 * 1024);
    int gx = 256 / mblocks;
    if (gx < 1) gx = 1;
    if (gx > p.ntiles) gx = p.ntiles;
    const dim3 grid(gx, mblocks);
#ifdef MTBC_PROBES
    static const int ts_env = mtbc_probe_int("MTBC_RING_TS", 0);
    if (ts_env) {
        ConvP q = p;
        const size_t nb = (size_t)gx * mblocks;
        static unsigned long long* dts = nullptr;
        if (!dts) (void)hipMalloc(&dts, 4096 * 16 * sizeof(unsigned long long));
        (void)hipMemsetAsync(dts, 0, nb * 16 * sizeof(unsigned long long), st);
        q.ts = dts;
        if (f16) hipLaunchKernelGGL((conv3x3_igemm_c8_ring_kernel<MT, GEO, true, O8, R>), grid, dim3(256), lds, st, q);
        else hipLaunchKernelGGL((conv3x3_igemm_c8_ring_kernel<MT, GEO, false, O8, R>), grid, dim3(256), lds, st, q);
        (void)hipStreamSynchronize(st);
        static unsigned long long hts[4096 * 16];
        (void)hipMemcpy(hts, dts, nb * 16 * sizeof(unsigned long long), hipMemcpyDeviceToHost);
        unsigned long long t0 = ~0ull, t1 = 0;
        for (size_t b = 0; b < nb; ++b) { if (hts[b * 16] < t0) t0 = hts[b * 16]; if (hts[b * 16 + 8] > t1) t1 = hts[b * 16 + 8]; }
        double mean[9] = {0}, mx[9] = {0};
        for (size_t b = 0; b < nb; ++b)
            for (int k = 0; k < 9; ++k) { const double d = (double)(hts[b * 16 + k] - t0) * 0.01; mean[k] += d / nb; if (d > mx[k]) mx[k] = d; }
        fprintf(stderr, "ring_ts %d->%d @%dx%d MT%d O8=%d blocks %zu span %.2f us | mean (max) us since the first block's entry: entry %.2f (%.2f) prologue %.2f (%.2f) issued %.2f (%.2f) "
                        "chunk0 landed %.2f (%.2f) chunk1 %.2f (%.2f) last chunk %.2f (%.2f) mfma done %.2f (%.2f) stores issued %.2f (%.2f) stores done %.2f (%.2f)\n",
                p.Cin, p.Cout, p.H, p.W, MT, O8, nb, (double)(t1 - t0) * 0.01, mean[0], mx[0], mean[1], mx[1], mean[2], mx[2], mean[3], mx[3], mean[4], mx[4], mean[5], mx[5],
                mean[6], mx[6], mean[7], mx[7], mean[8], mx[8]);
        return MTBC_OK;
    }
#endif
    if (f16) hipLaunchKernelGGL((conv3x3_igemm_c8_ring_kernel<MT, GEO, true, O8, R>), grid, dim3(256), lds, st, p);
    else hipLaunchKernelGGL((conv3x3_igemm_c8_ring_kernel<MT, GEO, false, O8, R>), grid, dim3(256), lds, st, p);
    MTBC_CHECK_LAUNCH();
    return MTBC_OK;
}
template <int GEO, int O8>
int launch_igemm_c8_ring_mt(int MT, const ConvP& p, int mblocks, bool f16, hipStream_t st) {
    if (MT == 1) return launch_igemm_c8_ring<1, GEO, O8>(p, mblocks, f16, st);
    if (MT == 3) return launch_igemm_c8_ring<3, GEO, O8>(p, mblocks, f16, st);
    return launch_igemm_c8_ring<2, GEO, O8>(p, mblocks, f16, st);
}

enum KernelFamily {
    KF_IGEMM, KF_IGEMM_DMA, KF_IGEMM_LP, KF_IGEMM_C8, KF_IGEMM_C8_RING, KF_STEM_FWD, KF_STEM_FWD_C8, KF_DIRECT,
    KF_WGRAD_STEM_C8, KF_WGRAD_C8, KF_WGRAD_C8W, KF_WGRAD_C8I, KF_WGRAD_MFMA, KF_WGRAD_LP, KF_WGRAD_LP2, KF_WGRAD_SMALLCIN, KF_WGRAD_DIRECT,
    KF_STEM_MC_FWD, KF_STEM_MC_FWD_C8, KF_WGRAD_STEM_MC_C8
};
struct KernelFamilyInfo { const char* name; int nargs; unsigned bools; };
constexpr KernelFamilyInfo KFAM[] = {
    {"conv3x3_igemm_kernel", 2, 0}, {"conv3x3_igemm_dma_kernel", 3, 0}, {"conv3x3_igemm_lp_kernel", 3, 4}, {"conv3x3_igemm_c8_kernel", 5, 4},
    {"conv3x3_igemm_c8_ring_kernel", 5, 4}, {"conv3x3_stem_fwd_kernel", 0, 0}, {"conv3x3_stem_fwd_c8_kernel", 1, 1}, {"conv3x3_direct_kernel", 0, 0},
    {"conv3x3_wgrad_stem_c8_kernel", 1, 1}, {"conv3x3_wgrad_c8_kernel", 2, 1}, {"conv3x3_wgrad_c8w_kernel", 3, 5}, {"conv3x3_wgrad_c8i_kernel", 3, 5},
    {"conv3x3_wgrad_mfma_kernel", 3, 4}, {"conv3x3_wgrad_lp_kernel", 3, 4}, {"conv3x3_wgrad_lp2_kernel", 1, 1}, {"conv3x3_wgrad_smallcin_kernel", 0, 0},
    {"conv3x3_wgrad_direct_kernel", 0, 0}, {"conv3x3_stem_mc_fwd_kernel", 1, 0}, {"conv3x3_stem_mc_fwd_c8_kernel", 2, 2}, {"conv3x3_wgrad_stem_mc_c8_kernel", 2, 2},
};
enum { KR_SPLITK = 1, KR_FIXUP = 2, KR_CHANNEL_SUMS = 4 };
struct KernelChoice { int fam; int t[5]; int red; };
inline KernelChoice kchoice(int fam, int t0 = 0, int t1 = 0, int t2 = 0, int t3 = 0, int t4 = 0) { return KernelChoice{fam, {t0, t1, t2, t3, t4}, 0}; }
int kernel_name(const KernelChoice& k, char* buf, int len) {
    const KernelFamilyInfo& f = KFAM[k.fam];
    char tmp[160];
    int n = snprintf(tmp, sizeof tmp, "%s", f.name);
    for (int i = 0; i < f.nargs; ++i) {
        const char* sep = i ? ", " : "<";
        if (f.bools >> i & 1) n += snprintf(tmp + n, sizeof tmp - n, "%s%s", sep, k.t[i] ? "true" : "false");
        else n += snprintf(tmp + n, sizeof tmp - n, "%s%d", sep, k.t[i]);
    }
    if (f.nargs) n += snprintf(tmp + n, sizeof tmp - n, ">");
    if (k.red & KR_SPLITK) n += snprintf(tmp + n, sizeof tmp - n, " + splitk_reduce");
    if (k.red & KR_FIXUP) n += snprintf(tmp + n, sizeof tmp - n, " + splitk_fixup");
    if (k.red & KR_CHANNEL_SUMS) n += snprintf(tmp + n, sizeof tmp - n, " + channel_sums");
    if (!buf || len <= n) return MTBC_E_BADARG;
    memcpy(buf, tmp, (size_t)n + 1);
    return MTBC_OK;
}
// ... 356 lines not shown
        return run_igemm(a->N, a->H, a->W, a->Cin, a->Cout, in, out, a->w_packed, a->bias, a->compute, st, true, of16 ? 3 : (o8 ? 1 : 0), a->stats_partial, nullptr, query);
    }
    if (a->stats_partial || a->norm_z || a->out_partial) return MTBC_E_UNSUPPORTED;
    if (a->operand_layout != MTBC_LAYOUT_PLANAR) return MTBC_E_BADARG;
    if (a->w_packed && !a->force_direct && mfma_ok(a->in, a->n_in, a->H, a->W))
        return run_igemm(a->N, a->H, a->W, a->Cin, a->Cout, in, out, a->w_packed, a->bias, a->compute, st, false, 0, nullptr, nullptr, query);
    if (!a->w) return MTBC_E_BADARG;
    if (stem && a->Cin > 1) {
        if (query) { *query = kchoice(KF_STEM_MC_FWD, a->Cin); return MTBC_OK; }
        const dim3 grid(cdiv(a->H * (a->W / 4), 128), cdiv(a->Cout, 8), a->N);
#define MTBC_STEM_MC(CIN_) hipLaunchKernelGGL((conv3x3_stem_mc_fwd_kernel<CIN_>), grid, dim3(128), 0, st, a->in[0].ptr, (long long)a->in[0].batch_stride, a->w, a->bias, a->out, a->N, a->H, a->W, a->Cout)
        switch (a->Cin) {
        case 2: MTBC_STEM_MC(2); break;
        case 3: MTBC_STEM_MC(3); break;
        case 4: MTBC_STEM_MC(4); break;
        default: MTBC_STEM_MC(5); break;
        }
#undef MTBC_STEM_MC
        MTBC_CHECK_LAUNCH();
        return MTBC_OK;
    }
    if (stem) {
        if (query) { *query = kchoice(KF_STEM_FWD); return MTBC_OK; }
        hipLaunchKernelGGL(conv3x3_stem_fwd_kernel, dim3(cdiv(a->H * (a->W / 4), 128), cdiv(a->Cout, 8), a->N), dim3(128), 0, st,
                           a->in[0].ptr, (long long)a->in[0].batch_stride, a->w, a->bias, a->out, a->N, a->H, a->W, a->Cout);
        MTBC_CHECK_LAUNCH();
        return MTBC_OK;
    }
    if (query) { *query = kchoice(KF_DIRECT); return MTBC_OK; }
    DirP p; p.N = a->N; p.H = a->H; p.W = a->W; p.Cin = a->Cin; p.Cout = a->Cout; p.in = in; p.out = out;
    p.w = a->w; p.bias = a->bias; p.mode = 0; p.wCin = a->Cin;
    hipLaunchKernelGGL(conv3x3_direct_kernel, dim3(cdiv(a->H * a->W, 128), cdiv(a->Cout, 8), a->N), dim3(128), 0, st, p);
    MTBC_CHECK_LAUNCH();
    return MTBC_OK;
}

int mtbc_conv3x3_fwd(const mtbc_conv3x3_args* a, void* stream) { return conv_fwd(a, (hipStream_t)stream, nullptr); }

static int conv_dgrad(const mtbc_conv3x3_args* a, hipStream_t st, KernelChoice* query) {
    int rc = check_conv(a); if (rc) return rc;
    if (!a->dout || (!a->w && !a->w_packed)) return MTBC_E_BADARG;
    SegTable in, out;
    mtbc_seg g{const_cast<float*>(a->dout), (int64_t)a->Cout * a->H * a->W, a->Cout, 0};
    rc = make_segtable(&g, 1, a->Cout, &in); if (rc) return rc;
    rc = make_segtable(a->in, a->n_in, a->Cin, &out); if (rc) return rc;
    if (a->operand_layout == MTBC_LAYOUT_C8) {
        if (!a->w_packed || (a->compute != 1 && a->compute != 2) || !c8_segs_ok(&g, 1)) return MTBC_E_BADARG;
        if (!mfma_ok(a->in, a->n_in, a->H, a->W)) return MTBC_E_UNSUPPORTED;
        int n3 = 0;
        for (int i = 0; i < a->n_in; ++i) {
            if (a->in[i].accumulate == 2 && ((reinterpret_cast<uintptr_t>(a->in[i].ptr) & 7) || (a->in[i].batch_stride & 3))) return MTBC_E_BADARG;
            if (a->in[i].accumulate == 3) ++n3;
        }
        if (n3 != 0 && (n3 != a->n_in || !c8_segs_ok(a->in, a->n_in))) return MTBC_E_BADARG;
        return run_igemm(a->N, a->H, a->W, a->Cout, a->Cin, in, out, a->w_packed, nullptr, a->compute, st, true, n3 != 0 ? 1 : 0, nullptr, nullptr, query);
    }
    if (a->operand_layout != MTBC_LAYOUT_PLANAR) return MTBC_E_BADARG;
    for (int i = 0; i < a->n_in; ++i)
        if (a->in[i].accumulate >= 2) return MTBC_E_UNSUPPORTED;
    bool ok = a->w_packed && !a->force_direct && mfma_ok(&g, 1, a->H, a->W) && a->Cout % KC == 0;
    for (int i = 0; ok && i < a->n_in; ++i) ok = a->in[i].ptr != nullptr && a->in[i].channels % 4 == 0;
    if (ok) return run_igemm(a->N, a->H, a->W, a->Cout, a->Cin, in, out, a->w_packed, nullptr, a->compute, st, false, 0, nullptr, nullptr, query);
    if (!a->w) return MTBC_E_BADARG;
    if (query) { *query = kchoice(KF_DIRECT); return MTBC_OK; }
    DirP p; p.N = a->N; p.H = a->H; p.W = a->W; p.Cin = a->Cout; p.Cout = a->Cin; p.in = in; p.out = out;
    p.w = a->w; p.bias = nullptr; p.mode = 1; p.wCin = a->Cin;
    hipLaunchKernelGGL(conv3x3_direct_kernel, dim3(cdiv(a->H * a->W, 128), cdiv(a->Cin, 8), a->N), dim3(128), 0, st, p);
    MTBC_CHECK_LAUNCH();
    return MTBC_OK;
}

int mtbc_conv3x3_dgrad(const mtbc_conv3x3_args* a, void* stream) { return conv_dgrad(a, (hipStream_t)stream, nullptr); }

int32_t mtbc_conv3x3_stats_slots(const mtbc_conv3x3_args* a) {
    if (check_conv(a) || a->out_layout != MTBC_LAYOUT_C8 || (a->compute != 1 && a->compute != 2)) return 0;
    if (a->operand_layout == MTBC_LAYOUT_PLANAR)
        return (a->Cin <= MTBC_STEM_MAX_CIN && a->n_in == 1 && a->W % 4 == 0 && a->Cout % 8 == 0) ? cdiv(a->H * (a->W / 4), 128) : 0;
    if (a->operand_layout != MTBC_LAYOUT_C8) return 0;
    if (a->W % 4 || a->W < 8 || a->H < 8 || a->Cout % 8) return 0;
    const IgemmPlan q = plan_igemm(a->N, a->H, a->W, a->Cout, a->compute, true, a->norm_z == nullptr, a->Cin);
    return q.geo == 2 ? 1 : q.tiles_x * q.tiles_y * (q.nw8 ? 8 : 4);
}

size_t mtbc_conv3x3_wgrad_workspace(const mtbc_conv3x3_args* a) {
    if (check_conv(a)) return 0;
    WgPlan w = plan_wgrad(a);
    return (w.partial_elems + w.dbias_elems) * sizeof(float);
}

size_t mtbc_conv3x3_wgrad_sync_bytes(const mtbc_conv3x3_args* a) {
    if (check_conv(a) || a->operand_layout != MTBC_LAYOUT_C8 || a->Cin <= MTBC_STEM_MAX_CIN) return 0;
    const WgPlan w = plan_wgrad(a);
    SplitKFix f{};
    return (size_t)splitk_fix_plan(w.nsplit, &f) * w.coblocks * w.ciblocks * sizeof(int);
}

static int conv_wgrad(const mtbc_conv3x3_args* a, hipStream_t st, KernelChoice* query) {
    int rc = check_conv(a); if (rc) return rc;
    if (!a->dout || !a->dw) return MTBC_E_BADARG;
    SegTable in;
    rc = make_segtable(a->in, a->n_in, a->Cin, &in); if (rc) return rc;
    WgPlan w = plan_wgrad(a);
    if (!a->workspace || a->workspace_bytes < (w.partial_elems + w.dbias_elems) * sizeof(float)) return MTBC_E_WORKSPACE;
    float* partial = reinterpret_cast<float*>(a->workspace);
    const size_t wel = (size_t)a->Cout * a->Cin * 9;
    if (a->operand_layout == MTBC_LAYOUT_C8 && a->Cin <= MTBC_STEM_MAX_CIN) {
        if ((a->compute != 1 && a->compute != 2) || a->n_in != 1 || a->Cout % 8 || a->W % 4 || a->dbias || a->in[0].batch_stride % 4 ||
            ((reinterpret_cast<uintptr_t>(a->in[0].ptr) | reinterpret_cast<uintptr_t>(a->dout)) & 15)) return MTBC_E_UNSUPPORTED;
        const int S = w.nsplit / a->N;
        const dim3 grid(a->N * (a->Cout / 8) * S);
        const unsigned short* dz8 = reinterpret_cast<const unsigned short*>(a->dout);
        KernelChoice k = a->Cin == 1 ? kchoice(KF_WGRAD_STEM_C8, a->compute == 2) : kchoice(KF_WGRAD_STEM_MC_C8, a->Cin, a->compute == 2);
        k.red = KR_SPLITK;
        if (query) { *query = k; return MTBC_OK; }
        if (k.fam == KF_WGRAD_STEM_MC_C8) {
#define MTBC_WG_STEM_MC(CIN_)                                                                                                                  \
            do {                                                                                                                               \
                if (k.t[1]) hipLaunchKernelGGL((conv3x3_wgrad_stem_mc_c8_kernel<CIN_, true>), grid, dim3(384), 0, st, a->in[0].ptr, (long long)a->in[0].batch_stride, dz8, partial, a->N, a->H, a->W, a->Cout, S); \
                else hipLaunchKernelGGL((conv3x3_wgrad_stem_mc_c8_kernel<CIN_, false>), grid, dim3(384), 0, st, a->in[0].ptr, (long long)a->in[0].batch_stride, dz8, partial, a->N, a->H, a->W, a->Cout, S); \
            } while (0)
            switch (a->Cin) {
            case 2: MTBC_WG_STEM_MC(2); break;
            case 3: MTBC_WG_STEM_MC(3); break;
            case 4: MTBC_WG_STEM_MC(4); break;
            default: MTBC_WG_STEM_MC(5); break;
            }
#undef MTBC_WG_STEM_MC
        } else if (k.t[0]) hipLaunchKernelGGL(conv3x3_wgrad_stem_c8_kernel<true>, grid, dim3(256), 0, st, a->in[0].ptr, (long long)a->in[0].batch_stride, dz8, partial, a->N, a->H, a->W, a->Cout, S);
        else hipLaunchKernelGGL(conv3x3_wgrad_stem_c8_kernel<false>, grid, dim3(256), 0, st, a->in[0].ptr, (long long)a->in[0].batch_stride, dz8, partial, a->N, a->H, a->W, a->Cout, S);
        MTBC_CHECK_LAUNCH();
        return mtbc_i_splitk_reduce(partial, a->dw, w.nsplit, wel, a->accumulate_dw, st);
    }
    if (a->operand_layout == MTBC_LAYOUT_C8) {
        mtbc_seg g{const_cast<float*>(a->dout), (int64_t)a->Cout * a->H * a->W, a->Cout, 0};
        if ((a->compute != 1 && a->compute != 2) || !c8_segs_ok(a->in, a->n_in) || !c8_segs_ok(&g, 1)) return MTBC_E_BADARG;
        WgC8P p; p.N = a->N; p.H = a->H; p.W = a->W; p.Cin = a->Cin; p.Cout = a->Cout; p.in = in;
        p.dz = reinterpret_cast<const unsigned short*>(a->dout); p.partial = partial;
        p.want_bias = a->dbias ? 1 : 0; p.prow = (long long)wel + (a->dbias ? a->Cout : 0);
        const bool direct = w.nsplit == 1 && !a->dbias && !a->accumulate_dw;
        if (direct) p.partial = a->dw;
        p.fix = SplitKFix{};
        if (a->wgrad_sync && !direct) {
            const size_t need = (size_t)splitk_fix_plan(w.nsplit, &p.fix) * w.coblocks * w.ciblocks * sizeof(int);
            if (a->wgrad_sync_bytes < need || (reinterpret_cast<uintptr_t>(a->wgrad_sync) & 3)) return MTBC_E_WORKSPACE;
            p.fix.ctr = a->wgrad_sync; p.fix.dw = a->dw; p.fix.dbias = a->dbias; p.fix.accumulate = a->accumulate_dw;
        }
        p.tiles_x = w.tiles_x; p.tiles_y = w.tiles_y; p.total_tiles = w.total_tiles; p.tiles_per_split = w.tiles_per_split;
        p.ciblocks = w.ciblocks; p.coblocks = w.coblocks; p.cit = w.cit; p.segs = w.segs; p.seg_tiles = w.seg_tiles; p.depth = w.depth;
        { static const int hk = mtbc_probe_int("MTBC_C8W_HACK", 0); p.hack = hk; }
        const dim3 grid = (w.c8w || w.c8i) ? dim3(w.nsplit * w.coblocks * w.ciblocks) : dim3(w.nsplit, w.coblocks * w.ciblocks);
        const bool f16 = a->compute == 2, bias = a->dbias != nullptr;
        KernelChoice k = w.c8i ? kchoice(KF_WGRAD_C8I, f16, w.cot, bias) : w.c8w ? kchoice(KF_WGRAD_C8W, f16, w.cot, bias) : kchoice(KF_WGRAD_C8, f16, w.geo);
        k.red = direct ? 0 : p.fix.ctr ? KR_FIXUP : KR_SPLITK;
        if (query) { *query = k; return MTBC_OK; }
#ifdef MTBC_PROBES
        static const int wts_env = mtbc_probe_int("MTBC_WG_TS", 0);
        static unsigned long long* wdts = nullptr;
        const size_t wnb = (size_t)grid.x * grid.y;
        p.ts = nullptr;
        if (wts_env && wnb <= 4096) {
            if (!wdts) (void)hipMalloc(&wdts, 4096 * 16 * sizeof(unsigned long long));
            (void)hipMemsetAsync(wdts, 0, wnb * 16 * sizeof(unsigned long long), st);
            p.ts = wdts;
        }
#endif
        if (k.fam == KF_WGRAD_C8I) {
// ... 241 lines not shown
```

### multi_task_breast_cancer_amd/csrc/norm_coop.hip

```cpp
#include "common.h"
#include <stddef.h>
#include <type_traits>

namespace {

constexpr int CO_THREADS = 512, CO_WAVES = CO_THREADS / 64;
constexpr int CO_MAXT = 128, CO_NV = 16;
constexpr unsigned CO_SPIN_MAX = 1u << 26;
constexpr size_t CO_MAILBOX_OFF = 256;
constexpr int CO_MAX_TEAMS = 1024;
constexpr size_t CO_TEAM_WORDS = 2 * CO_MAXT * CO_NV;
struct CoopHdr { unsigned epoch, done, err, pad; };

struct CoP {
    int N, C, HW, G8, T, items, nteams, f16;
    float eps, slope;
    const float* z; const float* gamma; const float* beta;
    float* y; long long ybs;
    unsigned short* y8;
    float* mean; float* rstd;
    const float* dy; long long dybs;
    unsigned short* dz8;
    float* part;
    float* part3;
// ... 506 lines not shown
#pragma unroll
                for (int h = 0; h < 4; ++h) o[h] = co_pk<F16>(v[2 * h], v[2 * h + 1]);
                *reinterpret_cast<co_u32x4*>(ob + pos[e] * 8) = o;
                if (yb) {
#pragma unroll
                    for (int c = 0; c < 8; ++c) yb[(size_t)c * p.HW + pos[e]] = v[c];
                }
                if (yh) {
                    if (e & 1) {
#pragma unroll
                        for (int c = 0; c < 8; ++c) {
                            const unsigned lo = (oprev[c >> 1] >> (16 * (c & 1))) & 0xffffu, hi = (o[c >> 1] >> (16 * (c & 1))) & 0xffffu;
                            *reinterpret_cast<unsigned*>(yh + (size_t)c * p.HW + pos[e - 1]) = lo | (hi << 16);
                        }
                    } else oprev = o;
                }
                float r[8];
                co_unpk<F16>(o, r);
#pragma unroll
                for (int c = 0; c < 8; ++c) {
                    if (e == 0) best[c] = r[c];
                    else if (r[c] > best[c] || r[c] != r[c]) { best[c] = r[c]; code = (code & ~(3u << (2 * c))) | ((unsigned)e << (2 * c)); }
                }
            }
            co_u32x4 o;
#pragma unroll
            for (int h = 0; h < 4; ++h) o[h] = co_pk<F16>(best[2 * h], best[2 * h + 1]);
            *reinterpret_cast<co_u32x4*>(pb + (size_t)q * 8) = o;
            if (p.parg) p.parg[((size_t)n * p.G8 + g) * oHW + q] = (unsigned short)code;
        }
        return;
    }
    static_assert(AP_PPT == 2, "the 16-bit planes pair a thread's two pixels");
    const int pxb = blockIdx.x * (AP_THREADS * AP_PPT), pstep = yh ? 1 : AP_THREADS;
    const int px0 = pxb + (yh ? 2 * (int)threadIdx.x : (int)threadIdx.x);
    co_u32x4 w[AP_PPT], okeep = {0u, 0u, 0u, 0u};
#pragma unroll
    for (int k = 0; k < AP_PPT; ++k) {
        const int px = px0 + pstep * k;
        if (px < p.HW) w[k] = *reinterpret_cast<const co_u32x4*>(zg + (size_t)px * 8);
    }
#pragma unroll
    for (int k = 0; k < AP_PPT; ++k) {
        const int px = px0 + pstep * k;
        if (px >= p.HW) continue;
        float v[8];
        co_unpk<ZF16>(w[k], v);
#pragma unroll
        for (int c = 0; c < 8; ++c) { const float t = (v[c] - mu[c]) * ga[c] + be[c]; v[c] = t > 0.f ? t : t * p.slope; }
        co_u32x4 o;
#pragma unroll
        for (int h = 0; h < 4; ++h) o[h] = co_pk<F16>(v[2 * h], v[2 * h + 1]);
        *reinterpret_cast<co_u32x4*>(ob + (size_t)px * 8) = o;
        if (yb) {
#pragma unroll
            for (int c = 0; c < 8; ++c) yb[(size_t)c * p.HW + px] = v[c];
        }
        if (yh) {
            if (k == 1) {
#pragma unroll
                for (int c = 0; c < 8; ++c) {
                    const unsigned lo = (okeep[c >> 1] >> (16 * (c & 1))) & 0xffffu, hi = (o[c >> 1] >> (16 * (c & 1))) & 0xffffu;
                    *reinterpret_cast<unsigned*>(yh + (size_t)c * p.HW + px - 1) = lo | (hi << 16);
                }
            } else okeep = o;
        }
    }
}

__global__ void in_bstats_finalize_kernel(const float* __restrict__ part, int slots, int C, int HW, float* __restrict__ m12,
                                          float* __restrict__ dparam_part, int planes) {
    const int plane = blockIdx.x * (blockDim.x >> 6) + (threadIdx.x >> 6), lane = threadIdx.x & 63;
    if (plane >= planes) return;
    const int n = plane / C, c = plane % C;
    const float* q = part + ((size_t)n * slots * C + c) * 2;
    double s1 = 0.0, s2 = 0.0;
    for (int t = lane; t < slots; t += 64) { const float2 v = *reinterpret_cast<const float2*>(q + (size_t)t * C * 2); s1 += (double)v.x; s2 += (double)v.y; }
    s1 = wave_sum_d(s1); s2 = wave_sum_d(s2);
    if (lane == 0) {
        m12[2 * plane] = (float)(s1 / (double)HW); m12[2 * plane + 1] = (float)(s2 / (double)HW);
        if (dparam_part) { dparam_part[3 * plane] = (float)s1; dparam_part[3 * plane + 1] = (float)s2; dparam_part[3 * plane + 2] = 0.f; }
    }
}
template <bool F16, bool ZF16>
__global__ __launch_bounds__(AP_THREADS) void in_apply_bwd_c8_kernel(const CoP p, const float* __restrict__ m12) {
    const int item = blockIdx.y, n = item / p.G8, g = item % p.G8;
    float mu[8], rs[8], ga[8], be[8], m1[8], m2[8];
#pragma unroll
    for (int c = 0; c < 8; ++c) {
        const size_t pl = (size_t)n * p.C + 8 * g + c;
        mu[c] = p.mean[pl]; rs[c] = p.rstd[pl]; ga[c] = p.gamma ? p.gamma[8 * g + c] : 1.f; be[c] = p.beta ? p.beta[8 * g + c] : 0.f;
        m1[c] = m12[2 * pl]; m2[c] = m12[2 * pl + 1];
    }
    const unsigned short* zg = p.z8 + ((size_t)n * p.G8 + g) * p.HW * 8;
    const unsigned short* dg = p.dy8 + (size_t)n * p.dy8bs + (size_t)g * p.HW * 8;
    unsigned short* ob = p.dz8 + ((size_t)n * p.G8 + g) * p.HW * 8;
    const int px0 = blockIdx.x * (AP_THREADS * AP_PPT) + threadIdx.x;
    co_u32x4 wz[AP_PPT], wd[AP_PPT];
#pragma unroll
    for (int k = 0; k < AP_PPT; ++k) {
        const int px = px0 + AP_THREADS * k;
        if (px < p.HW) { wz[k] = *reinterpret_cast<const co_u32x4*>(zg + (size_t)px * 8); wd[k] = *reinterpret_cast<const co_u32x4*>(dg + (size_t)px * 8); }
    }
#pragma unroll
    for (int k = 0; k < AP_PPT; ++k) {
        const int px = px0 + AP_THREADS * k;
        if (px >= p.HW) continue;
        float z[8], d[8];
        co_unpk<ZF16>(wz[k], z);
        co_unpk<F16>(wd[k], d);
#pragma unroll
        for (int c = 0; c < 8; ++c) {
            const float xh = (z[c] - mu[c]) * rs[c];
            const float gg = d[c] * ((xh * ga[c] + be[c]) > 0.f ? 1.f : p.slope);
            d[c] = rs[c] * ga[c] * (gg - m1[c] - xh * m2[c]);
        }
        co_u32x4 o;
#pragma unroll
        for (int h = 0; h < 4; ++h) o[h] = co_pk<F16>(d[2 * h], d[2 * h + 1]);
        *reinterpret_cast<co_u32x4*>(ob + (size_t)px * 8) = o;
    }
}

__global__ void in_r1_finalize_kernel(const float* __restrict__ dwp, const float* __restrict__ dbp, float* __restrict__ dw, float* __restrict__ db,
                                      int N, int C, int T, int accumulate) {
    const int c = blockIdx.x, lane = threadIdx.x;
    float s = 0.f;
    if (c < C) { for (int i = lane; i < N * T; i += 64) s += dwp[((size_t)(i / T) * C + c) * T + i % T]; }
    else { for (int i = lane; i < N * T; i += 64) s += dbp[i]; }
    s = wave_sum(s);
    if (lane != 0) return;
    if (c < C) dw[c] = accumulate ? dw[c] + s : s;
    else if (db) db[0] = accumulate ? db[0] + s : s;
}

struct CoPlan { bool ok; int ppt, T, grid, nteams; };
template <typename K> int resident_blocks(K kernel) {
    int per_cu = 0, dev = 0;
    if (hipOccupancyMaxActiveBlocksPerMultiprocessor(&per_cu, kernel, CO_THREADS, 0) != hipSuccess || per_cu < 1) return 0;
    hipDeviceProp_t prop;
    if (hipGetDevice(&dev) != hipSuccess || hipGetDeviceProperties(&prop, dev) != hipSuccess) return 0;
    if (per_cu > 3) per_cu = 3;
    return per_cu * prop.multiProcessorCount;
}
int device_cus() {
    static DevInts cache;
    return mtbc_per_device(cache, [] { int dev = 0; hipDeviceProp_t prop; return (hipGetDevice(&dev) == hipSuccess && hipGetDeviceProperties(&prop, dev) == hipSuccess) ? prop.multiProcessorCount : 0; });
}
int usable(int cap_all_cus, int reserve) {
    const int cus = device_cus();
    if (reserve <= 0 || cus <= 0) return cap_all_cus;
    const int keep = cus - reserve;
    return keep < 8 ? cap_all_cus / cus * 8 : cap_all_cus / cus * keep;
}
CoPlan plan_coop(int items, int HW, int max_ppt, const int* cap_by_ppt, int reserve) {
    CoPlan best{false, 0, 0, 0, 0};
    double best_eff = -1.0;
    for (int ppt = max_ppt; ppt >= 1; ppt >>= 1) {
        int T;
        if (HW <= CO_THREADS * ppt) { if (ppt > 1 && HW <= CO_THREADS * (ppt / 2)) continue; T = 1; }
        else { if (HW % (CO_THREADS * ppt)) continue; T = HW / (CO_THREADS * ppt); }
        if (T > CO_MAXT) continue;
        const int cap = usable(cap_by_ppt[ppt], reserve);
        if (cap < T) continue;
        int teams = cap / T;
        if (teams > items) teams = items;
// ... 101 lines not shown
    const int threads = k.t[0], ppt = k.t[1];
    if (k.t[3]) {
        p.T = pl.T; p.nteams = pl.nteams;
        if (ppt == 4) launch_c8<BWD, CO_THREADS, 4, true>(p, v, pl.grid, st);
        else if (ppt == 2) launch_c8<BWD, CO_THREADS, 2, true>(p, v, pl.grid, st);
        else launch_c8<BWD, CO_THREADS, 1, true>(p, v, pl.grid, st);
    } else {
        p.T = 1; p.nteams = p.items;
        if (threads == 64) launch_c8<BWD, 64, 1, false>(p, v, p.items, st);
        else if (threads == 256 && ppt == 1) launch_c8<BWD, 256, 1, false>(p, v, p.items, st);
        else if (threads == 256) launch_c8<BWD, 256, 4, false>(p, v, p.items, st);
        else launch_c8<BWD, 1024, 4, false>(p, v, p.items, st);
    }
}
void launch_apply_fwd(const NormLaunch& k, const dim3 g, hipStream_t st, const CoP& p, const float* part, int slots) {
    const bool f16 = k.t[0], fin = k.t[1], zf16 = k.t[2], pool = k.t[3];
#define MTBC_AP(F16_, FIN_, ZF_, POOL_) hipLaunchKernelGGL((in_apply_fwd_c8_kernel<F16_, FIN_, ZF_, POOL_>), g, dim3(AP_THREADS), 0, st, p, part, slots)
#define MTBC_APT(FIN_, POOL_) do { if (f16) MTBC_AP(true, FIN_, true, POOL_); else if (zf16) MTBC_AP(false, FIN_, true, POOL_); else MTBC_AP(false, FIN_, false, POOL_); } while (0)
    if (pool) { if (fin) MTBC_APT(true, true); else MTBC_APT(false, true); }
    else { if (fin) MTBC_APT(true, false); else MTBC_APT(false, false); }
#undef MTBC_APT
#undef MTBC_AP
}

}

extern "C" {

size_t mtbc_instnorm_coop_error_offset(void) { return offsetof(CoopHdr, err); }

size_t mtbc_instnorm_coop_state_bytes(void) { return CO_MAILBOX_OFF + (size_t)CO_MAX_TEAMS * CO_TEAM_WORDS * sizeof(unsigned long long); }

int mtbc_instnorm_c8_supported(const mtbc_instnorm_args* a, int32_t backward) {
    if (!a || a->N <= 0 || a->C <= 0 || a->H <= 0 || a->W <= 0 || a->C % 8) return 0;
    if (backward && a->n_dy_extra != 0 && a->n_dy_extra != 1) return 0;
    if (a->H * a->W <= SOLO_MAX_HW) return 1;
    const CoPlan pl = backward ? plan_team<true>(a->N * (a->C / 8), a->H * a->W, var_of(a), a->coop_reserve_cus)
                               : plan_team<false>(a->N * (a->C / 8), a->H * a->W, var_of(a), a->coop_reserve_cus);
    return pl.ok ? 1 : 0;
}

int mtbc_i_instnorm_fwd_c8(const mtbc_instnorm_args* a, hipStream_t st, NormChoice* query) {
    CoP p; int rc = fill_coop(a, &p); if (rc) return rc;
    if ((!p.z && !p.z8) || !p.y8 || !p.mean || !p.rstd || (reinterpret_cast<uintptr_t>(p.y8) & 15)) return MTBC_E_BADARG;
    if (p.y16 && !a->stats_partial) return MTBC_E_UNSUPPORTED;
    NormChoice ch{};
    CoPlan pl{false, 0, 0, 0, 0};
    dim3 g(1);
    const int planes = a->N * a->C;
    if (a->stats_partial) {
        if (!p.z8 || a->stats_slots <= 0) return MTBC_E_BADARG;
        if (p.py8) {
            if (((a->H | a->W) & 1) || (reinterpret_cast<uintptr_t>(p.py8) & 15)) return MTBC_E_BADARG;
            int gx = cdiv(p.HW / 4, AP_THREADS * 2); if (gx < 1) gx = 1;
            g = dim3(gx, p.items);
        } else g = dim3(cdiv(p.HW, AP_THREADS * AP_PPT), p.items);
        const bool fin = a->stats_slots <= 64;
        if (!fin) ch.add(NK_STATS_FIN);
        ch.add(NK_APPLY_FWD, p.f16, fin, p.f16 || p.zf16, p.py8 != nullptr);
    } else if (p.HW <= SOLO_MAX_HW) choose_c8(&ch, false, p.HW, p.items, var_of(a), nullptr);
    else {
        if (!p.state) return MTBC_E_BADARG;
        pl = plan_team<false>(p.items, p.HW, var_of(a), a->coop_reserve_cus);
        if (!pl.ok) return MTBC_E_UNSUPPORTED;
        choose_c8(&ch, false, p.HW, p.items, var_of(a), &pl);
    }
    if (query) { for (int i = 0; i < ch.n; ++i) query->add(ch.l[i]); return MTBC_OK; }
    for (int i = 0; i < ch.n; ++i) {
        const NormLaunch& k = ch.l[i];
        if (k.k == NK_STATS_FIN) hipLaunchKernelGGL(in_stats_finalize_kernel, dim3(cdiv(planes, 4)), dim3(256), 0, st, a->stats_partial, a->stats_slots, a->C, p.HW, a->eps, a->mean, a->rstd, planes);
        else if (k.k == NK_APPLY_FWD) launch_apply_fwd(k, g, st, p, a->stats_partial, a->stats_slots);
        else launch_chosen_c8<false>(k, p, pl, st);
        MTBC_CHECK_LAUNCH();
    }
    return MTBC_OK;
}

int mtbc_i_instnorm_bwd_c8_team(const mtbc_instnorm_args* a) {
    if (!a || a->N <= 0 || a->C <= 0 || a->C % 8) return 0;
    if (a->H * a->W <= SOLO_MAX_HW) return 1;
    const CoPlan pl = plan_team<true>(a->N * (a->C / 8), a->H * a->W, var_of(a), a->coop_reserve_cus);
    return pl.ok ? pl.T : 0;
}
int mtbc_i_instnorm_bwd_c8(const mtbc_instnorm_args* a, float* part, hipStream_t st, NormChoice* query) {
    CoP p; int rc = fill_coop(a, &p); if (rc) return rc;
    if ((!p.z && !p.z8) || (!p.dy && !p.r1 && !p.pg) || !p.dz8 || !p.mean || !p.rstd || (reinterpret_cast<uintptr_t>(p.dz8) & 15)) return MTBC_E_BADARG;
    if (!p.dy && a->dy_layout == MTBC_LAYOUT_C8) return MTBC_E_BADARG;
    if ((p.r1 || p.pg) && a->stats_partial) return MTBC_E_UNSUPPORTED;
    if (a->dy_layout == MTBC_LAYOUT_C8) {
        if ((reinterpret_cast<uintptr_t>(a->dy) & 15) || a->dy_batch_stride % 8 || a->n_dy_extra < 0 || a->n_dy_extra > 1) return MTBC_E_BADARG;
        p.dy8 = reinterpret_cast<const unsigned short*>(a->dy); p.dy8bs = a->dy_batch_stride; p.dy = nullptr;
        if (a->n_dy_extra == 1) { if (!a->dy_extra[0]) return MTBC_E_BADARG; p.dyx = a->dy_extra[0]; }
    } else if (a->n_dy_extra == 1 && p.dy) {
        if (!a->dy_extra[0]) return MTBC_E_BADARG;
        p.dyx = a->dy_extra[0];
    } else if (a->n_dy_extra != 0) return MTBC_E_BADARG;
    p.part = part;
    const bool head_dw = a->dy_rank1 && a->dy_rank1_dw;
    const int planes = a->N * a->C;
    CoPlan pl{false, 0, 1, 0, 0};
    if (p.HW > SOLO_MAX_HW) { pl = plan_team<true>(p.items, p.HW, var_of(a), a->coop_reserve_cus); if (!pl.ok) return MTBC_E_UNSUPPORTED; }
    const int T_ = pl.T;
    if (head_dw) {
        const size_t need = ((size_t)planes * (3 + 2 * T_) + (size_t)a->N * T_) * sizeof(float);
        if (!a->workspace || a->workspace_bytes < need || a->stats_partial) return MTBC_E_WORKSPACE;
        p.r1dw = reinterpret_cast<float*>(a->workspace) + (size_t)planes * (3 + T_);
        p.r1db = p.r1dw + (size_t)planes * T_;
    }
    NormChoice ch{};
    float* m12 = nullptr;
    if (a->stats_partial) {
        if (!p.z8 || !p.dy8 || p.dyx || a->stats_slots <= 0 || !a->workspace || a->workspace_bytes < (size_t)a->N * a->C * 5 * sizeof(float)) return MTBC_E_BADARG;
        m12 = reinterpret_cast<float*>(a->workspace) + (size_t)3 * planes;
        ch.add(NK_BSTATS_FIN);
        ch.add(NK_APPLY_BWD, p.f16, p.f16 || p.zf16);
    } else {
        if (p.HW > SOLO_MAX_HW && !p.state) return MTBC_E_BADARG;
        p.part3 = part ? part + (size_t)3 * a->N * a->C : nullptr;
        choose_c8(&ch, true, p.HW, p.items, var_of(a), p.HW > SOLO_MAX_HW ? &pl : nullptr);
        if (head_dw) ch.add(NK_R1_FIN);
    }
    if (query) { for (int i = 0; i < ch.n; ++i) query->add(ch.l[i]); return MTBC_OK; }
    for (int i = 0; i < ch.n; ++i) {
        const NormLaunch& k = ch.l[i];
        if (k.k == NK_BSTATS_FIN) hipLaunchKernelGGL(in_bstats_finalize_kernel, dim3(cdiv(planes, 4)), dim3(256), 0, st, a->stats_partial, a->stats_slots, a->C, p.HW, m12, part, planes);
        else if (k.k == NK_APPLY_BWD) {
            const dim3 g(cdiv(p.HW, AP_THREADS * AP_PPT), p.items);
            if (k.t[0]) hipLaunchKernelGGL((in_apply_bwd_c8_kernel<true, true>), g, dim3(AP_THREADS), 0, st, p, m12);
            else if (k.t[1]) hipLaunchKernelGGL((in_apply_bwd_c8_kernel<false, true>), g, dim3(AP_THREADS), 0, st, p, m12);
            else hipLaunchKernelGGL((in_apply_bwd_c8_kernel<false, false>), g, dim3(AP_THREADS), 0, st, p, m12);
        } else if (k.k == NK_R1_FIN) hipLaunchKernelGGL(in_r1_finalize_kernel, dim3(a->C + 1), dim3(64), 0, st, p.r1dw, p.r1db, a->dy_rank1_dw, a->dy_rank1_db, a->N, a->C, T_, a->dy_rank1_accumulate);
        else launch_chosen_c8<true>(k, p, pl, st);
        MTBC_CHECK_LAUNCH();
    }
    return MTBC_OK;
}

}
```

### multi_task_breast_cancer_amd/csrc/program.hip

```cpp
#include "common.h"
#include <cstring>

extern "C" {

int mtbc_version(void) { return MTBC_VERSION; }
const char* mtbc_arch(void) { return "gfx950"; }

const char* mtbc_strerror(int code) {
    switch (code) {
        case MTBC_OK: return "ok";
        case MTBC_E_BADSHAPE: return "bad shape";
        case MTBC_E_BADARG: return "bad argument (null or misaligned pointer)";
        case MTBC_E_WORKSPACE: return "workspace missing or too small";
        case MTBC_E_LAUNCH: return "kernel launch failed";
        case MTBC_E_UNSUPPORTED: return "unsupported configuration";
        default: return "unknown error";
    }
}

static inline bool is_pack(int32_t k) { return k == MTBC_OP_CONV3_PACK_FWD || k == MTBC_OP_CONV3_PACK_DGRAD || k == MTBC_OP_CONV3_PACK_LP; }

int mtbc_event_create(void** event) {
    if (!event) return MTBC_E_BADARG;
    hipEvent_t e;
// ... 25 lines not shown
        case MTBC_OP_HEAD_COMBINE: rc = mtbc_i_head_combine(&op->u.head, nullptr, &ch); break;
        case MTBC_OP_HEAD_EXPAND: rc = mtbc_i_head_expand(&op->u.head, nullptr, &ch); break;
        default: return MTBC_E_BADARG;
    }
    if (rc) return rc;
    if (!buf || len <= ch.len) return MTBC_E_BADARG;
    memcpy(buf, ch.s, (size_t)ch.len + 1);
    return MTBC_OK;
}

int mtbc_program_run(const mtbc_op* ops, int32_t first, int32_t count, void* stream, int32_t* failed_index) {
    void* one[1] = {stream};
    return mtbc_program_run_ms(ops, first, count, one, 1, failed_index);
}

int mtbc_program_run_ms(const mtbc_op* ops, int32_t first, int32_t count, void* const* streams, int32_t n_streams, int32_t* failed_index) {
    if (!ops || first < 0 || count < 0 || !streams || n_streams < 1) return MTBC_E_BADARG;
    void* stream = streams[0];
    for (int32_t i = first; i < first + count; ++i) {
        const mtbc_op* o = &ops[i];
        int rc;
        if (o->kind == MTBC_OP_SET_STREAM) {
            if (o->u.sync.index < 0) { if (failed_index) *failed_index = i; return MTBC_E_BADARG; }
            stream = streams[o->u.sync.index < n_streams ? o->u.sync.index : 0];
            continue;
        }
        if (o->kind == MTBC_OP_EVENT_RECORD || o->kind == MTBC_OP_EVENT_WAIT) {
            hipError_t e = hipErrorInvalidValue;
            if (o->u.sync.event)
                e = o->kind == MTBC_OP_EVENT_RECORD ? hipEventRecord((hipEvent_t)o->u.sync.event, (hipStream_t)stream)
                                                    : hipStreamWaitEvent((hipStream_t)stream, (hipEvent_t)o->u.sync.event, 0);
            if (e != hipSuccess) { if (failed_index) *failed_index = i; return o->u.sync.event ? MTBC_E_LAUNCH : MTBC_E_BADARG; }
            continue;
        }
        if (is_pack(o->kind)) {
            mtbc_pack_desc d[128];
            int32_t n = 0;
            while (n < 128 && i + n < first + count && is_pack(ops[i + n].kind)) {
                const mtbc_op* q = &ops[i + n];
                d[n].w = q->u.pack.w; d[n].packed = q->u.pack.packed; d[n].Cin = q->u.pack.Cin; d[n].Cout = q->u.pack.Cout;
                d[n].compute = q->u.pack.compute;
                d[n].kind = q->kind == MTBC_OP_CONV3_PACK_FWD ? 0 : q->kind == MTBC_OP_CONV3_PACK_DGRAD ? 1 : (q->u.pack.dgrad ? 3 : 2);
                ++n;
            }
            if (n > 1) {
                rc = mtbc_conv3x3_pack_many(d, n, stream);
                if (rc != MTBC_OK) { if (failed_index) *failed_index = i; return rc; }
                i += n - 1;
                continue;
            }
        }
        if (o->kind == MTBC_OP_CONV3_WVIEW) {
            mtbc_wview_desc d[128];
            int32_t n = 0;
            while (n < 128 && i + n < first + count && ops[i + n].kind == MTBC_OP_CONV3_WVIEW) {
                const mtbc_op* q = &ops[i + n];
                d[n].w = q->u.wview.w; d[n].dst = q->u.wview.dst; d[n].Cout = q->u.wview.Cout; d[n].Cin = q->u.wview.Cin;
                d[n].ci_off = q->u.wview.ci_off; d[n].ci_cnt = q->u.wview.ci_cnt; d[n].mode = q->u.wview.mode;
                d[n].k_off = q->u.wview.k_off; d[n].K = q->u.wview.K;
                ++n;
            }
            if (n > 1) {
                rc = mtbc_conv3x3_weight_view_many(d, n, stream);
                if (rc != MTBC_OK) { if (failed_index) *failed_index = i; return rc; }
                i += n - 1;
                continue;
            }
        }
        if (o->kind == MTBC_OP_IN_DPARAM) {
            mtbc_dparam_desc d[64];
            int32_t n = 0;
            while (n < 64 && i + n < first + count && ops[i + n].kind == MTBC_OP_IN_DPARAM) { d[n] = ops[i + n].u.dparam; ++n; }
            rc = mtbc_instnorm_dparam_many(d, n, stream);
            if (rc != MTBC_OK) { if (failed_index) *failed_index = i; return rc; }
            i += n - 1;
            continue;
        }
        if (o->kind == MTBC_OP_CONVT_WGRAD && i + 1 < first + count && ops[i + 1].kind == MTBC_OP_CONVT_DGRAD) {
            bool fused = false;
            rc = mtbc_i_convT_bwd_pair(&o->u.convT, &ops[i + 1].u.convT, stream, &fused);
            if (rc != MTBC_OK) { if (failed_index) *failed_index = i; return rc; }
            if (fused) { ++i; continue; }
        }
        switch (o->kind) {
            case MTBC_OP_CONV3_FWD: rc = mtbc_conv3x3_fwd(&o->u.conv3, stream); break;
            case MTBC_OP_CONV3_DGRAD: rc = mtbc_conv3x3_dgrad(&o->u.conv3, stream); break;
            case MTBC_OP_CONV3_WGRAD: rc = mtbc_conv3x3_wgrad(&o->u.conv3, stream); break;
            case MTBC_OP_CONV3_PACK_FWD: rc = mtbc_conv3x3_pack_fwd(o->u.pack.w, o->u.pack.packed, o->u.pack.Cin, o->u.pack.Cout, stream); break;
            case MTBC_OP_CONV3_PACK_DGRAD: rc = mtbc_conv3x3_pack_dgrad(o->u.pack.w, o->u.pack.packed, o->u.pack.Cin, o->u.pack.Cout, stream); break;
            case MTBC_OP_HEAD_COMBINE: rc = mtbc_convT_head_combine(&o->u.head, stream); break;
            case MTBC_OP_HEAD_EXPAND: rc = mtbc_convT_head_expand(&o->u.head, stream); break;
            case MTBC_OP_CONV3_WVIEW: rc = mtbc_conv3x3_weight_view(o->u.wview.w, o->u.wview.dst, o->u.wview.Cout, o->u.wview.Cin, o->u.wview.ci_off, o->u.wview.ci_cnt, o->u.wview.mode, o->u.wview.k_off, o->u.wview.K, stream); break;
            case MTBC_OP_C8_PACK16: rc = mtbc_c8_pack16(o->u.c8pack.src, o->u.c8pack.src_batch_stride, o->u.c8pack.dst, o->u.c8pack.N, o->u.c8pack.C, o->u.c8pack.HW, stream); break;
            case MTBC_OP_C8_PACK: rc = mtbc_c8_pack(o->u.c8pack.src, o->u.c8pack.src_batch_stride, o->u.c8pack.dst, o->u.c8pack.N, o->u.c8pack.C, o->u.c8pack.HW, o->u.c8pack.compute, stream); break;
            case MTBC_OP_CONV3_PACK_LP: rc = mtbc_conv3x3_pack_lp(o->u.pack.w, o->u.pack.packed, o->u.pack.Cin, o->u.pack.Cout, o->u.pack.dgrad, o->u.pack.compute, stream); break;
            case MTBC_OP_IN_FWD: rc = mtbc_instnorm_lrelu_fwd(&o->u.inorm, stream); break;
            case MTBC_OP_IN_BWD: rc = mtbc_instnorm_lrelu_bwd(&o->u.inorm, stream); break;
            case MTBC_OP_POOL_FWD: rc = mtbc_maxpool2_fwd(&o->u.pool, stream); break;
            case MTBC_OP_POOL_BWD: rc = mtbc_maxpool2_bwd(&o->u.pool, stream); break;
            case MTBC_OP_CONVT_FWD: rc = mtbc_convT_fwd(&o->u.convT, stream); break;
            case MTBC_OP_CONVT_DGRAD: rc = mtbc_convT_dgrad(&o->u.convT, stream); break;
            case MTBC_OP_CONVT_WGRAD: rc = mtbc_convT_wgrad(&o->u.convT, stream); break;
            case MTBC_OP_CONV1_FWD: rc = mtbc_conv1x1_fwd(&o->u.conv1, stream); break;
            case MTBC_OP_CONV1_DGRAD: rc = mtbc_conv1x1_dgrad(&o->u.conv1, stream); break;
            case MTBC_OP_CONV1_WGRAD: rc = mtbc_conv1x1_wgrad(&o->u.conv1, stream); break;
            case MTBC_OP_GAP_FWD: rc = mtbc_gap_fwd(&o->u.gap, stream); break;
            case MTBC_OP_GAP_BWD: rc = mtbc_gap_bwd(&o->u.gap, stream); break;
            case MTBC_OP_LINEAR_FWD: rc = mtbc_linear_fwd(&o->u.linear, stream); break;
            case MTBC_OP_LINEAR_BWD: rc = mtbc_linear_bwd(&o->u.linear, stream); break;
            case MTBC_OP_DICE_FWD: rc = mtbc_dice_fwd(&o->u.dice, stream); break;
            case MTBC_OP_DICE_BWD: rc = mtbc_dice_bwd(&o->u.dice, stream); break;
            case MTBC_OP_FOCAL: rc = mtbc_focal_fwd_bwd(&o->u.focal, stream); break;
            case MTBC_OP_LOSS_MIX: rc = mtbc_loss_mix(o->u.mix.seg, o->u.mix.cls, o->u.mix.alpha, o->u.mix.out4, stream); break;
            case MTBC_OP_SOFTMAX: rc = mtbc_softmax_rows(&o->u.softmax, stream); break;
            case MTBC_OP_UPSAMPLE2_FWD: rc = mtbc_upsample2_fwd(&o->u.up2, stream); break;
            case MTBC_OP_UPSAMPLE2_BWD: rc = mtbc_upsample2_bwd(&o->u.up2, stream); break;
            case MTBC_OP_OPTIM: rc = mtbc_optim_step(&o->u.optim, stream); break;
            case MTBC_OP_MEMSET:
                rc = hipMemsetAsync(o->u.memset0.ptr, 0, o->u.memset0.bytes, (hipStream_t)stream) == hipSuccess ? MTBC_OK : MTBC_E_LAUNCH;
                break;
            case MTBC_OP_DICE_COUNTS: rc = mtbc_dice_counts(o->u.counts.logits, o->u.counts.target, o->u.counts.n, o->u.counts.out3, stream); break;
            default: rc = MTBC_E_BADARG;
        }
        if (rc != MTBC_OK) {
            if (failed_index) *failed_index = i;
            return rc;
        }
    }
    return MTBC_OK;
}

}
```

### multi_task_breast_cancer_amd/engine.py

```python
from __future__ import annotations

import ctypes as C
from dataclasses import dataclass, field
from typing import Callable, Dict, List, Optional, Sequence, Tuple

import torch

from . import _lib as L
from . import ops as _ops


from . import switches as _sw

_sw.refuse_removed()
_NO_COOP = _sw.flag("MTBC_NO_COOP")
_NO_GATHER = _sw.flag("MTBC_NO_GATHER")
_NO_Z16 = _sw.flag("MTBC_NO_Z16")
_Z_BF16 = _sw.flag("MTBC_Z_BF16")
_NO_STEM_MC = _sw.flag("MTBC_NO_STEM_MC")
_DA16 = _sw.flag("MTBC_DA16")
_COOP_MIN_FWD, _COOP_MIN_BWD = 16384, 65536
_IN_KERNEL_SPLITK = False
_DPARAM_BATCH = 12


def _ptr(t: Optional[torch.Tensor]) -> Optional[int]:
    return None if t is None else t.data_ptr()


@dataclass
class Act:
    name: str
    data: torch.Tensor
    needs_grad: bool = True
    grad: Optional[torch.Tensor] = None
    grad_written: bool = False
    c8: Optional[torch.Tensor] = None
    planar_valid: bool = True
    planar_used: bool = False
    p16_users: list = field(default_factory=list)
    c8_used: bool = False
    conv_consumers: int = 0
    no_gather: bool = False
    pending: List[tuple] = field(default_factory=list)
    readers: int = 0
    grad16_ok: bool = False
    grad16: Optional[torch.Tensor] = None
    dy8_ok: bool = False
    grad8: Optional[torch.Tensor] = None
    z16: bool = False
    r1: Optional[tuple] = None
    pool: Optional[tuple] = None
    pooled: Optional["Act"] = None
    parent: Optional["Act"] = None
    view_index: int = 0
    views: list = field(default_factory=list)
    c8_filled: bool = False
    in_op: Optional[object] = None
    pack_op: Optional[object] = None

    @property
    def N(self): return self.data.shape[0]
    @property
    def C(self): return self.data.shape[1]
    @property
    def H(self): return self.data.shape[2]
    @property
    def W(self): return self.data.shape[3]
    @property
    def bstride(self): return self.data.shape[1] * self.data.shape[2] * self.data.shape[3]


@dataclass
class _Cell:
    inputs: List["Act"]
    y: "Act"
    N: int
    cin: int
    cout: int
    H: int
    W: int
    tag: int
    w: torch.Tensor
    wname: str
    bname: Optional[str]
    gname: Optional[str]
    betaname: Optional[str]
    slope: float
    mean: torch.Tensor
    rstd: torch.Tensor
    use_packed: bool
    wp_d: Optional[torch.Tensor] = None
    wp_d_op: Optional[object] = None
    c8: bool = False
    c8_bwd: bool = False
    stem16: bool = False
    old_mc: bool = False
    z16: bool = False
    zf16: bool = False
    z: Optional[torch.Tensor] = None


@dataclass
class ParamSlot:
    name: str
# ... 352 lines not shown
            arr[i].ptr = self.c8_of(a_).data_ptr()
            arr[i].batch_stride, arr[i].channels, arr[i].accumulate = a_.bstride, a_.C, 0

    def _cell_conv_op(self, cell: "_Cell", kind: int) -> L.Op:
        op = _mk(kind, cell.tag)
        a = op.u.conv3
        a.N, a.H, a.W, a.Cin, a.Cout, a.n_in = cell.N, cell.H, cell.W, cell.cin, cell.cout, len(cell.inputs)
        a.w = cell.w.data_ptr()
        a.force_direct = self.force_direct
        a.compute = self.compute if cell.use_packed else 0
        return op

    def _cell_norm_op(self, cell: "_Cell", kind: int) -> L.Op:
        op = _mk(kind, cell.tag)
        a = op.u.inorm
        a.N, a.C, a.H, a.W, a.eps, a.slope = cell.N, cell.cout, cell.H, cell.W, 1e-5, cell.slope
        a.z = cell.z.data_ptr()
        a.z_layout = L.LAYOUT_C8 if cell.z16 else L.LAYOUT_PLANAR
        a.z_type = 2 if cell.zf16 else 0
        a.gamma = _ptr(self.pv(cell.gname)) if cell.gname else None
        a.beta = _ptr(self.pv(cell.betaname)) if cell.betaname else None
        a.mean, a.rstd = cell.mean.data_ptr(), cell.rstd.data_ptr()
        a.coop_reserve_cus = self.coop_reserve_cus
        return op

    def _gathered_dgrad(self, cell: "_Cell") -> None:
        y, cout, N, H, W = cell.y, cell.cout, cell.N, cell.H, cell.W
        K = sum(pj[4] for pj in y.pending)
        wg = self.alloc(cout, K, 3, 3)
        koff = 0
        for (dzj, wj, offj, cinj, coutj) in y.pending:
            self._wview(wj, wg, coutj, cinj, offj, cout, 1, koff, K)
            koff += coutj
        wpg, _ = self._pack_lp(wg, K, cout, 0)
        if y.dy8_ok:
            y.grad8 = self.alloc(N, cout // 8, H * W, 8, dtype=torch.int16)
            gbuf, acc = y.grad8, 0
        else:
            gbuf, acc = self.grad_slot(y)
        op = _mk(L.OP_CONV3_FWD, cell.tag)
        a = op.u.conv3
        a.N, a.H, a.W, a.Cin, a.Cout, a.n_in = N, H, W, K, cout, len(y.pending)
        for i_, (dzj, wj, offj, cinj, coutj) in enumerate(y.pending):
            a.in_[i_].ptr, a.in_[i_].batch_stride, a.in_[i_].channels, a.in_[i_].accumulate = dzj.data_ptr(), coutj * H * W, coutj, 0
        a.w, a.w_packed, a.out = wg.data_ptr(), wpg.data_ptr(), gbuf.data_ptr()
        a.compute, a.operand_layout, a.out_accumulate = self.compute, L.LAYOUT_C8, acc
        if y.dy8_ok:
            a.out_layout = L.LAYOUT_C8
        self.bwd_ops.append(op)

    def _conv_cell_backward(self, cell: "_Cell") -> None:
        y, inputs, cout, N, H, W = cell.y, cell.inputs, cell.cout, cell.N, cell.H, cell.W
        gname, betaname, bname, z16, c8_bwd = cell.gname, cell.betaname, cell.bname, cell.z16, cell.c8_bwd
        if not y.grad_written and not y.pending and y.r1 is None and y.pool is None:
            return
        written_before = y.grad_written
        g8 = bool(y.pending) and y.dy8_ok
        if y.pending:
            self._gathered_dgrad(cell)
        only_folded = (y.r1 is not None or y.pool is not None) and not g8 and not y.grad_written
        dy = y.grad8 if g8 else (None if only_folded else self.grad_of(y))
        op = self._cell_norm_op(cell, L.OP_IN_BWD)
        a = op.u.inorm
        a.dy, a.dy_batch_stride, a.dz = _ptr(dy), y.bstride, _ptr(dy)
        if y.pool is not None:
            a.dy_pool, a.dy_pool_arg = y.pool[0].data_ptr(), y.pool[1].data_ptr()
        if y.r1 is not None:
            a.dy_rank1, a.dy_rank1_w = y.r1[0].data_ptr(), y.r1[1].data_ptr()
            a.dy_rank1_dw, a.dy_rank1_db, a.dy_rank1_accumulate = y.r1[2].data_ptr(), y.r1[3].data_ptr(), y.r1[4]
        if g8:
            a.dy_layout, a.dz = L.LAYOUT_C8, None
            if written_before:
                a.n_dy_extra = 1
                a.dy_extra[0] = y.grad.data_ptr()
        defer: List[Act] = []
        if c8_bwd and cell.wp_d is not None and not _NO_GATHER:
            for a_ in inputs:
                if a_.in_op is not None and a_.needs_grad and a_.conv_consumers >= (1 if a_.dy8_ok else 2) and not a_.no_gather and a_.C % 8 == 0:
                    defer.append(a_)
                else:
                    break

        def dz8_buffer() -> torch.Tensor:
            return self.alloc(N * cout * H * W, dtype=torch.int16) if defer else self._scratch16("_dz8_buf", N * cout * H * W)

        coop = z16 or (c8_bwd and not _NO_COOP and H * W >= _COOP_MIN_BWD and bool(self.lib.mtbc_instnorm_c8_supported(C.byref(a), 1)))
        dz8 = dz16 = None
        if coop:
            dz8 = dz8_buffer()
            a.dz8, a.out16_type, a.coop_state = dz8.data_ptr(), self.compute, self._coop_state()
        p16 = c8_bwd and not coop and (H * W) % 4 == 0 and H * W <= 65536
        if p16:
            dz16 = self._scratch16("_dz16_buf", N * cout * H * W)
            a.dz16, a.out16_type = dz16.data_ptr(), self.compute
        if gname or bname:
            acc = None
            if gname:
                acc = self._mark_param(gname)
                self._mark_param(betaname)
                a.dgamma, a.dbeta = self.gv(gname).data_ptr(), self.gv(betaname).data_ptr()
            if bname:
                accb = self._mark_param(bname)
                acc = accb if acc is None else acc
                assert acc == accb
                a.dbias_pre = self.gv(bname).data_ptr()
            a.accumulate_dparams = acc
            self._need_ws(op, "inorm", N * cout * (131 if coop else 3) * 4)
        if y.r1 is not None:
            self._need_ws(op, "inorm", N * (cout + 1) * 262 * 4)
        dop = None
        if (gname or bname) and z16 and self.dev.type == "cuda":
            if a.accumulate_dparams:
                self.flush_dparams()
            buf = self.alloc(N * (cout + 1) * 262)
            self.ws_users = [u for u in self.ws_users if u[0] is not op]
            a.workspace, a.workspace_bytes, a.defer_dparams = buf.data_ptr(), buf.numel() * 4, 1
            dop = _mk(L.OP_IN_DPARAM, cell.tag)
            d = dop.u.dparam
            d.part, d.dgamma, d.dbeta, d.dbias_pre = buf.data_ptr(), a.dgamma, a.dbeta, a.dbias_pre
            d.N, d.C, d.T, d.accumulate = N, cout, int(self.lib.mtbc_instnorm_bwd_team(C.byref(a))), a.accumulate_dparams
        self.bwd_ops.append(op)
        if dop is not None:
            self._pending_dparams.append((dop, tuple(n_ for n_ in (gname, betaname, bname) if n_)))
            if len(self._pending_dparams) >= _DPARAM_BATCH:
                self.flush_dparams()
        if y.r1 is not None:
            for name in y.r1[5]:
                self.slots[name].ready_at = len(self.bwd_ops) - 1
        if c8_bwd and not coop:
            dz8 = dz8_buffer()
            pk = self._c8_pack_op(dz16 if p16 else dy, dz8, cout, H * W, N)
            if p16:
                pk.kind = L.OP_C8_PACK16
            self.bwd_ops.append(pk)
        op = self._cell_conv_op(cell, L.OP_CONV3_WGRAD)
        a = op.u.conv3
        if c8_bwd:
            self._segs_c8(a.in_, inputs)
            a.dout, a.operand_layout = dz8.data_ptr(), L.LAYOUT_C8
        elif cell.stem16:
            self._segs(a.in_, inputs)
            a.dout, a.operand_layout, a.compute = dz8.data_ptr(), L.LAYOUT_C8, self.compute
        else:
            self._segs(a.in_, inputs)
            a.dout = dy.data_ptr()
            if cell.old_mc and cell.cin > 4:
                a.force_direct = 1
        a.accumulate_dw = self._mark_param(cell.wname)
        a.dw = self.gv(cell.wname).data_ptr()
        self._need_ws(op, "conv3", self.lib.mtbc_conv3x3_wgrad_workspace(C.byref(a)))
        nsync = int(self.lib.mtbc_conv3x3_wgrad_sync_bytes(C.byref(a))) if _IN_KERNEL_SPLITK else 0
        if nsync:
            self._sync_users.append(op)
            self._sync_bytes = max(self._sync_bytes, nsync)
        self.bwd_ops.append(op)
        need = [a_ for a_ in inputs if a_.needs_grad]
        if need and defer:
            off = 0
            for a_ in defer:
                a_.pending.append((dz8, cell.w, off, cell.cin, cout))
                off += a_.C
            self.pack_ops.remove(cell.wp_d_op)
            rest = inputs[len(defer):]
            if rest:
                crest = cell.cin - off
                ws = self.alloc(cout, crest, 3, 3)
                self._wview(cell.w, ws, cout, cell.cin, off, crest, 0, 0, 0)
                wps, _ = self._pack_lp(ws, crest, cout, 1)
                op = self._cell_conv_op(cell, L.OP_CONV3_DGRAD)
                a = op.u.conv3
                a.Cin, a.n_in, a.w = crest, len(rest), ws.data_ptr()
                self._segs(a.in_, rest, grads=True, g16=True)
                a.dout, a.operand_layout, a.w_packed = dz8.data_ptr(), L.LAYOUT_C8, wps.data_ptr()
                self.bwd_ops.append(op)
        elif need:
            if len(need) != len(inputs):
                raise NotImplementedError("mixed grad / no-grad concat inputs")
            op = self._cell_conv_op(cell, L.OP_CONV3_DGRAD)
            a = op.u.conv3
            self._segs(a.in_, inputs, grads=True, g16=bool(c8_bwd and cell.wp_d is not None))
            a.dout = _ptr(dy)
            if c8_bwd and cell.wp_d is not None:
                a.dout, a.operand_layout = dz8.data_ptr(), L.LAYOUT_C8
            a.w_packed = _ptr(cell.wp_d)
            self.bwd_ops.append(op)

    def _c8_small_ok(self, x: Act) -> bool:
        return bool(self.compute) and not self.force_direct and x.C % 8 == 0 and (x.H * x.W) % 4 == 0

    def maxpool(self, x: Act, out_name: str, out: Optional[Act] = None) -> Act:
        if x.pooled is not None:
            assert out is None or out is x.pooled
            self.acts[out_name] = x.pooled
            return x.pooled
        x.readers += 1
        if out is not None:
            assert out.N == x.N and (out.C, out.H, out.W) == (x.C, x.H // 2, x.W // 2)
# ... 506 lines not shown
```

### multi_task_breast_cancer_amd/switches.py

```python
from __future__ import annotations

import os
from typing import Dict, List

PLAN_SWITCHES: Dict[str, tuple] = {
    "MTBC_NO_COOP": ("0", "InstanceNorm by one-plane workgroups (fp32 conv outputs) + pack instead of the channel-group / cooperative kernels: "
                          "the fallback when their teams cannot be co-resident (the cooperative error message names it)",
                     "tests/test_model_gpu.py::test_16bit_mfma_modes_match_their_emulation[...-no_coop-40]"),
    "MTBC_NO_GATHER": ("0", "every 3x3 conv back-propagates into all its inputs (fan-in by read-modify-write) instead of one gathered launch per dense-skip tensor",
                       "tests/test_model_gpu.py::test_16bit_mfma_modes_match_their_emulation[...-no_gather]"),
    "MTBC_NO_Z16": ("0", "16-bit modes keep the conv outputs z as fp32 planes (InstanceNorm reads 4 bytes per element in both directions): the storage arm of the quality sweeps",
                    "tests/test_model_gpu.py::test_16bit_mfma_modes_match_their_emulation[...-no_z16]"),
    "MTBC_Z_BF16": ("0", "bf16 mode stores the conv outputs as bf16 instead of fp16 (same bytes, 8 instead of 11 significant bits)",
                    "tests/test_model_gpu.py::test_16bit_mfma_modes_match_their_emulation[...-z_bf16]"),
    "MTBC_DA16": ("0", "the gradient a conv-cell activation gets from its 3x3 consumers is written by ONE gathered launch as a 16-bit channel-blocked tensor (fp32 sum in the MFMA "
                       "accumulators, one RNE) instead of fp32 planar fan-in: -0.36 ms per step.  Default in round 3 on the easy task's evidence (-0.010 +- 0.025 pt); OFF again since "
                       "round 4: on the task that can fail it ends at the same Dice (-0.012 +- 0.042 pt against fp32, 10 paired seeds) but reaches the plateau LATER -- mid-run "
                       "-5.6 +- 2.9 pt against fp32 where the fp32-gradient plan is at -0.5 +- 1.4 and tracks the fp32 runs seed by seed (profiles/r04_quality_hard.md)",
                  "tests/test_model_gpu.py::test_16bit_mfma_modes_match_their_emulation[...-da16]"),
    "MTBC_NOFUSE_HEADS": ("0", "MTnnUNet deep-supervision heads as ConvT + 1x1 (the reference's two layers) instead of one combined ConvT",
                          "tests/test_model_gpu.py::test_mtnnunet_two_layer_heads_match_the_fused_heads_and_the_oracle"),
    "MTBC_GRAPH": ("0", "trainer.FusedTrainStep (single process) captures each compiled step -- weight images, forward, losses, backward, Adam -- into ONE hipGraph at its third call "
                        "and replays it from then on: the host issues a step in 0.1 ms instead of 8.4 (profiles/r04_graph_replay.txt); the GPU time is the same, the results are the same bits "
                        "(the optimizer's per-step scalars travel through device memory, mtbc_optim_args.dynamic)",
                   "tests/test_model_gpu.py::test_graph_replayed_steps_are_the_eager_steps"),
    "MTBC_DYN_SCALE": ("0", "trainer.FusedTrainStep(loss_scale=None) trains with the device-side dynamic loss scale (loss_scale.DynamicLossScale(): start 2^16, found-inf check "
                            "over the flat gradients, skip + halve on overflow, double after 2000 clean steps) instead of the static scale baked into the loss ops: three more "
                            "launches per step; without an overflow the same bits as the static 2^16 of fp16 mode",
                       "tests/test_loss_scale_gpu.py::test_dynamic_steps_without_overflow_are_the_static_steps"),
    "MTBC_NO_STEM_MC": ("0", "a first conv with intensity channels (data.augmentation: Cin 2 .. 5) takes the launches it took before the multi-channel stem kernels: "
                             "conv3x3_direct_kernel, an fp32 conv output under the one-plane InstanceNorm, the small-Cin (Cin = 5: the direct) weight gradient from fp32 dz -- "
                             "the A arm of tools/stem_cost.py",
                        "tests/test_stem_multichannel_gpu.py::test_whole_model_against_the_emulation[...-no_stem_mc]"),
    "MTBC_COOP_RESERVE_CUS": ("64", "CUs kept out of the cooperative InstanceNorm grids under data parallel",
                              "tests/test_coop_safety_gpu.py::test_cooperative_step_beside_a_cu_hogging_kernel"),
}
REMOVED = ("MTBC_NO_C8", "MTBC_NO_CT_LP", "MTBC_COOP_MIN_FWD", "MTBC_COOP_MIN_BWD", "MTBC_NO_P16", "MTBC_FANIN", "MTBC_NO_C8_SMALL_OPS", "MTBC_NO_X16",
           "MTBC_NO_G16", "MTBC_NO_EPI_STATS", "MTBC_EPI_BSTATS", "MTBC_NO_R1", "MTBC_NO_POOLFOLD", "MTBC_SPLIT_FANIN", "MTBC_NO_STEM16",
           "MTBC_NO_DEFER_DPARAM", "MTBC_DPARAM_BATCH", "MTBC_NO_POOLFWD_FOLD", "MTBC_BWD_OVERLAP", "MTBC_BWD_OVERLAP_MAX_HW",
           "MTBC_NO_DA16")
RESULT_ALTERING = ("MTBC_DBG", "MTBC_NOACC", "MTBC_LOWP", "MTBC_LP_MT", "MTBC_RING", "MTBC_NODMA", "MTBC_C8_BLOCKS_PER_CU",
                   "MTBC_WGRAD_LP1", "MTBC_CT_WG_TASKS", "MTBC_IN_BWD_STREAM", "MTBC_CONVT_GENERIC", "MTBC_C8_NW", "MTBC_C8_RING",
                   "MTBC_CT_DEPTH", "MTBC_CT_WG_CT", "MTBC_CT_WG_XCD", "MTBC_CT_DGRAD_DIRECT", "MTBC_WGRAD_C8W", "MTBC_C8W_BPC", "MTBC_C8W_DEPTH", "MTBC_C8W_HACK",
                   "MTBC_WGRAD_PACK24", "MTBC_WGRAD_C8I", "MTBC_WG_NS8", "MTBC_WG_TS", "MTBC_C8_TS", "MTBC_RING_TS", "MTBC_INB_TS",
                   "MTBC_CT_UNFUSED", "MTBC_CT_FUSE_ALL")


def get(name: str) -> str:
    return os.environ.get(name, PLAN_SWITCHES[name][0])


def flag(name: str) -> bool:
    v = get(name)
    return v not in ("", "0")


def active() -> Dict[str, str]:
    return {k: v for k, v in sorted(os.environ.items()) if k.startswith("MTBC_")}


def removed() -> List[str]:
    return [k for k in REMOVED if k in os.environ]


def refuse_removed() -> None:
    bad = removed()
    if bad:
        raise RuntimeError(f"removed plan switch(es) set: {bad} -- these arms no longer exist (switches.py REMOVED; the 16-bit gathered gradients are the opt-in MTBC_DA16=1 since round 4, "
                           "MTBC_NO_DA16 is gone); unset them")


def result_altering() -> List[str]:
    bad = [k for k in RESULT_ALTERING if k in os.environ]
    if "MTBC_LIB" in os.environ:
        bad.append("MTBC_LIB")
    return bad
```

Measured before the change: 2876 images/sec.

## Fuse conv3x3 dgrad with InstanceNorm+LeakyReLU backward in paired C8 kernels

Adds a paired path in which the conv3x3 data-gradient kernel's epilogue applies the LeakyReLU mask and InstanceNorm backward directly. A stats pass accumulates per-plane sums, a finalize kernel reduces them, and an apply pass recomputes the dgrad and writes the 16-bit dz. This avoids writing an fp32 planar dy and having the cooperative norm backward read it back, for large maps (HW >= 65536). In exchange the dgrad GEMM runs twice and there are extra launches and workspace. The program runner detects adjacent DGRAD and IN_BWD ops and takes the pair when it is eligible.

New measurement: 2903 images/sec, median of 6. About the same (+0.9%).

```diff
diff --git a/include/mtbc.h b/include/mtbc.h
--- a/include/mtbc.h
+++ b/include/mtbc.h
@@ -163,6 +163,8 @@
 int mtbc_instnorm_lrelu_fwd(const mtbc_instnorm_args* a, void* stream);
 int mtbc_instnorm_lrelu_bwd(const mtbc_instnorm_args* a, void* stream);
 
+size_t mtbc_conv3x3_dgrad_normbwd_pair_workspace(const mtbc_conv3x3_args* dgrad, const mtbc_instnorm_args* norm);
+
 typedef struct {
     int32_t N, C, H, W;
     const float* x;  int64_t x_batch_stride;
diff --git a/multi_task_breast_cancer_amd/_lib.py b/multi_task_breast_cancer_amd/_lib.py
--- a/multi_task_breast_cancer_amd/_lib.py
+++ b/multi_task_breast_cancer_amd/_lib.py
@@ -312,6 +312,7 @@
     "mtbc_eval_metrics", "mtbc_seg_step_metrics", "mtbc_fill_holes", "mtbc_fill_holes_host",
     "mtbc_softmax_rows", "mtbc_softmax_rows_host", "mtbc_cls_step_metrics", "mtbc_cls_test_rows",
     "mtbc_upsample2_fwd", "mtbc_upsample2_bwd", "mtbc_linear_workspace", "mtbc_linear_wide_enable",
+    "mtbc_conv3x3_dgrad_normbwd_pair_workspace",
 ]
 
 ABI_VERSION = 203
@@ -345,6 +346,8 @@
         getattr(lib, _n).argtypes = [C.POINTER(HeadFuseArgs), C.c_void_p]
     lib.mtbc_conv3x3_stats_slots.restype = C.c_int32
     lib.mtbc_conv3x3_stats_slots.argtypes = [C.POINTER(Conv3x3Args)]
+    lib.mtbc_conv3x3_dgrad_normbwd_pair_workspace.restype = C.c_size_t
+    lib.mtbc_conv3x3_dgrad_normbwd_pair_workspace.argtypes = [C.POINTER(Conv3x3Args), C.POINTER(InstNormArgs)]
     lib.mtbc_conv3x3_kernel_name.restype = C.c_int
     lib.mtbc_conv3x3_kernel_name.argtypes = [C.POINTER(Conv3x3Args), C.c_int32, C.c_char_p, C.c_int32]
     lib.mtbc_instnorm_kernel_name.restype = C.c_int
diff --git a/multi_task_breast_cancer_amd/csrc/common.h b/multi_task_breast_cancer_amd/csrc/common.h
--- a/multi_task_breast_cancer_amd/csrc/common.h
+++ b/multi_task_breast_cancer_amd/csrc/common.h
@@ -151,6 +151,8 @@
 extern "C" int mtbc_i_instnorm_fwd_c8(const mtbc_instnorm_args* a, hipStream_t st, NormChoice* query);
 extern "C" int mtbc_i_instnorm_bwd_c8(const mtbc_instnorm_args* a, float* part, hipStream_t st, NormChoice* query);
 extern "C" int mtbc_i_instnorm_bwd_c8_team(const mtbc_instnorm_args* a);
+extern "C" int mtbc_i_instnorm_bstats_finalize(const float* part, int slots, int N, int C, int HW, float* m12, float* dparam_part, int T, hipStream_t st);
+extern "C" int mtbc_i_conv3x3_dgrad_normbwd_pair(const mtbc_conv3x3_args* dgrad, const mtbc_instnorm_args* norm, void* stream, bool* fused);
 #include <stdarg.h>
 #include <stdio.h>
 struct OpChoice {
diff --git a/multi_task_breast_cancer_amd/csrc/conv3x3.hip b/multi_task_breast_cancer_amd/csrc/conv3x3.hip
--- a/multi_task_breast_cancer_amd/csrc/conv3x3.hip
+++ b/multi_task_breast_cancer_amd/csrc/conv3x3.hip
@@ -833,10 +833,10 @@
             __builtin_bit_cast(float, __builtin_amdgcn_readlane(r, 47))) + __builtin_bit_cast(float, __builtin_amdgcn_readlane(r, 63));
 }
 
-template <int MT, int GEO, bool F16, int NW, int O8, bool FULL, typename ZPRE>
+template <int MT, int GEO, bool F16, int NW, int O8, bool FULL, typename ZPRE, typename MPRE>
 __device__ __forceinline__ void c8_epilogue(const ConvP& p, f32x4 (&acc)[MT][4], const SegL* seg_out, const float* bias_s, const int n0,
                                             const int y0, const int x0, const int tx, const int ty, const int mt0, const int wv,
-                                            const int j, const int kg, const int HW, ZPRE& zpre) {
+                                            const int j, const int kg, const int HW, ZPRE& zpre, MPRE& mpre) {
     using T = LP<F16>;
     using TO = LP<F16 || O8 == 3>;
     typedef unsigned pre_u32x2 __attribute__((ext_vector_type(2)));
@@ -855,7 +855,7 @@
             else { y = y0 + 2 * g + (j >> 3); x = x0 + (j & 7); }
             pix[g] = (FULL || (n < p.N && y < p.H && x < p.W)) ? y * p.W + x : -1;
         }
-        const bool want_stats = O8 == 2 || p.stats != nullptr;
+        const bool want_stats = O8 == 2 || O8 == 4 || O8 == 6 || (O8 < 4 && p.stats != nullptr);
 #pragma unroll
         for (int m = 0; m < MT; ++m) {
             const int co = (mt0 + m) * 16 + 4 * kg;
@@ -890,6 +890,38 @@
                         for (int e = 0; e < 4; ++e) gg[e] = dyv[e] * (pre[e] > 0.f ? 1.f : p.nslope);
                         ss += gg; sq += gg * xh;
                     }
+            } else if constexpr (O8 >= 4) {
+                using TZ = LP<F16 || O8 >= 6>;
+                constexpr bool APPLY = O8 == 5 || O8 == 7;
+                asm volatile("" ::: "memory");
+                const int cl = m * 16 + 4 * kg;
+                const f32x4 mean4 = *reinterpret_cast<const f32x4*>(mpre + cl), rstd4 = *reinterpret_cast<const f32x4*>(mpre + MT * 16 + cl);
+                const f32x4 ga4 = *reinterpret_cast<const f32x4*>(mpre + 2 * MT * 16 + cl), be4 = *reinterpret_cast<const f32x4*>(mpre + 3 * MT * 16 + cl);
+                f32x4 k4 = mean4, m1 = mean4, m2 = mean4;
+                if constexpr (APPLY) {
+                    k4 = rstd4 * ga4;
+                    const float* mq = mpre + 4 * MT * 16 + 2 * cl;
+                    const f32x4 ma = *reinterpret_cast<const f32x4*>(mq), mb = *reinterpret_cast<const f32x4*>(mq + 4);
+                    m1 = (f32x4){ma[0], ma[2], mb[0], mb[2]};
+                    m2 = (f32x4){ma[1], ma[3], mb[1], mb[3]};
+                }
+#pragma unroll
+                for (int g = 0; g < 4; ++g)
+                    if (FULL || pix[g] >= 0) {
+                        const pre_u32x2 zw = zpre[m][g];
+                        const unsigned z0 = zw[0], z1 = zw[1];
+                        const f32x4 xh = ((f32x4){TZ::lo(z0), TZ::hi(z0), TZ::lo(z1), TZ::hi(z1)} - mean4) * rstd4;
+                        const f32x4 pre = xh * ga4 + be4;
+                        f32x4 gg;
+#pragma unroll
+                        for (int e = 0; e < 4; ++e) gg[e] = acc[m][g][e] * (pre[e] > 0.f ? 1.f : p.nslope);
+                        if constexpr (APPLY) {
+                            const f32x4 d = k4 * (gg - m1 - xh * m2);
+                            const float q[8] = {d[0], d[1], d[2], d[3], 0.f, 0.f, 0.f, 0.f};
+                            const ep_u32x4 u = __builtin_bit_cast(ep_u32x4, T::pack(q));
+                            *(guint2*)(cb + 16 * (size_t)pix[g]) = (ep_u32x2){u[0], u[1]};
+                        } else { ss += gg; sq += gg * xh; }
+                    }
             } else {
 #pragma unroll
                 for (int g = 0; g < 4; ++g)
@@ -974,6 +1006,7 @@
     using G = GeoLP<GEO>;
     using T = LP<F16>;
     static_assert(NW == 4 || (NW == 8 && GEO == 0), "8-wave blocks: wide-map geometry only");
+    static_assert(O8 < 4 || (GEO == 0 && NW == 4 && (O8 < 6 || !F16)), "dgrad + norm-backward pair: wide maps, 4 waves; 6 / 7 = fp16 z beside bf16 operands");
     constexpr int TH = GEO == 0 ? 2 * NW : G::TH;
     constexpr int HR = TH + 2, HC = G::TW + 2, HP = G::IMG * HR * HC;
     constexpr int HPP = (HP + 15) / 16 * 16;
@@ -987,12 +1020,23 @@
     SegL* seg_in = reinterpret_cast<SegL*>(smem16 + XB + WB);
     SegL* seg_out = seg_in + MTBC_MAX_SEGS;
     float* bias_s = reinterpret_cast<float*>(seg_out + MTBC_MAX_SEGS);
+    constexpr bool APPLY = O8 == 5 || O8 == 7;
+    constexpr bool PAIR = O8 >= 4;
+    float* cst_s = bias_s + MT * 16;
+    float* m12_s = cst_s + 4 * MT * 16;
     const int tid = threadIdx.x, lane = tid & 63, wv = tid >> 6;
     const int wvu = __builtin_amdgcn_readfirstlane(tid >> 6);
     const int HW = p.H * p.W;
     const int mt0 = blockIdx.y * MT;
     float bias_v = 0.f;
     if (tid < MT * 16) { const int co = mt0 * 16 + tid; if (p.bias && co < p.Cout) bias_v = p.bias[co]; }
+    if constexpr (PAIR) {
+        const int co = mt0 * 16 + tid;
+        if (tid < MT * 16) {
+            const bool ok = p.ngamma && co < p.Cout;
+            cst_s[2 * MT * 16 + tid] = ok ? p.ngamma[co] : 1.f; cst_s[3 * MT * 16 + tid] = ok ? p.nbeta[co] : 0.f;
+        }
+    }
     segl_fill(seg_in, p.in);
     segl_fill(seg_out, p.out);
 
@@ -1057,8 +1101,19 @@
             for (int g = 0; g < 4; ++g) acc[m][g] = (f32x4){0.f, 0.f, 0.f, 0.f};
         typedef unsigned pre_u32x2 __attribute__((ext_vector_type(2)));
         typedef __attribute__((address_space(1))) pre_u32x2 gpre2;
-        pre_u32x2 zpre[O8 == 2 ? MT : 1][4];
-        if constexpr (O8 == 2) {
+        pre_u32x2 zpre[(O8 == 2 || O8 >= 4) ? MT : 1][4];
+        float mean_v = 0.f, rstd_v = 0.f;
+        f32x2 m12_v = (f32x2){0.f, 0.f};
+        const float* mpre = cst_s;
+        if constexpr (PAIR) {
+            const int co = mt0 * 16 + tid;
+            if (tid < MT * 16 && co < p.Cout && n0 < p.N) {
+                const size_t plane = (size_t)n0 * p.Cout + co;
+                mean_v = p.nmean[plane]; rstd_v = p.nrstd[plane];
+                if constexpr (APPLY) m12_v = *reinterpret_cast<const f32x2*>(p.extra + 2 * plane);
+            }
+        }
+        if constexpr (O8 == 2 || O8 >= 4) {
             const int nn = GEO == 2 ? n0 + wvu : n0;
 #pragma unroll
             for (int g = 0; g < 4; ++g) {
@@ -1111,7 +1166,14 @@
                 w_have = ch;
             }
             if (ch == 0 && tsk < 3) MTBC_TS(p, 4 * tsk + 1);
-            asm volatile("s_waitcnt vmcnt(0)\n\ts_barrier" ::: "memory");
+            if (PAIR && ch == 0) {
+                asm volatile("s_waitcnt vmcnt(0)" ::: "memory");
+                if (tid < MT * 16) {
+                    cst_s[tid] = mean_v; cst_s[MT * 16 + tid] = rstd_v;
+                    if constexpr (APPLY) *reinterpret_cast<f32x2*>(m12_s + 2 * tid) = m12_v;
+                }
+                lds_barrier();
+            } else asm volatile("s_waitcnt vmcnt(0)\n\ts_barrier" ::: "memory");
             if (ch == 0 && tsk < 3) MTBC_TS(p, 4 * tsk + 2);
 #pragma unroll
             for (int tap = 0; tap < 9; ++tap) {
@@ -1133,8 +1195,8 @@
             }
         }
         if (tsk < 3) MTBC_TS(p, 4 * tsk + 3);
-        if (n0 + G::IMG <= p.N && y0 + TH <= p.H && x0 + G::TW <= p.W) c8_epilogue<MT, GEO, F16, NW, O8, true>(p, acc, seg_out, bias_s, n0, y0, x0, tx, ty, mt0, wvu, j, kg, HW, zpre);
-        else c8_epilogue<MT, GEO, F16, NW, O8, false>(p, acc, seg_out, bias_s, n0, y0, x0, tx, ty, mt0, wvu, j, kg, HW, zpre);
+        if (n0 + G::IMG <= p.N && y0 + TH <= p.H && x0 + G::TW <= p.W) c8_epilogue<MT, GEO, F16, NW, O8, true>(p, acc, seg_out, bias_s, n0, y0, x0, tx, ty, mt0, wvu, j, kg, HW, zpre, mpre);
+        else c8_epilogue<MT, GEO, F16, NW, O8, false>(p, acc, seg_out, bias_s, n0, y0, x0, tx, ty, mt0, wvu, j, kg, HW, zpre, mpre);
         if (tsk < 3) MTBC_TS(p, 12 + tsk);
         ++tsk;
     }
@@ -1301,10 +1363,10 @@
                 });
             });
         }
-        int zpre = 0;
+        int zpre = 0, mpre = 0;
         MTBC_TS(p, 6);
-        if (y0 + TH <= p.H && x0 + G::TW <= p.W) c8_epilogue<MT, GEO, F16, NW, O8, true>(p, acc, seg_out, bias_s, n0, y0, x0, tx, ty, mt0, wvu, j, kg, HW, zpre);
-        else c8_epilogue<MT, GEO, F16, NW, O8, false>(p, acc, seg_out, bias_s, n0, y0, x0, tx, ty, mt0, wvu, j, kg, HW, zpre);
+        if (y0 + TH <= p.H && x0 + G::TW <= p.W) c8_epilogue<MT, GEO, F16, NW, O8, true>(p, acc, seg_out, bias_s, n0, y0, x0, tx, ty, mt0, wvu, j, kg, HW, zpre, mpre);
+        else c8_epilogue<MT, GEO, F16, NW, O8, false>(p, acc, seg_out, bias_s, n0, y0, x0, tx, ty, mt0, wvu, j, kg, HW, zpre, mpre);
         MTBC_TS(p, 7);
         asm volatile("s_waitcnt vmcnt(0)" ::: "memory");
         MTBC_TS(p, 8);
@@ -3255,6 +3317,32 @@
     }
 }
 
+template <int MT, int O8>
+int launch_igemm_c8_pair(const ConvP& p, int mblocks, bool f16, hipStream_t st) {
+    using G = GeoLP<0>;
+    constexpr int HP = (8 + 2) * (G::TW + 2), HPP = (HP + 15) / 16 * 16;
+    const size_t lds = ((size_t)4 * HPP * 8 + (size_t)MT * 9 * 16 * WROW) * 2 + (SEGL_FLOATS + MT * 16 * 7) * sizeof(float);
+    const int per_cu = lds * 3 <= 160 * 1024 ? 3 : 2;
+    int gx = (256 * per_cu / mblocks) / 8 * 8;
+    if (gx < 8) gx = 8;
+    if (gx > p.ntiles) gx = p.ntiles;
+    const dim3 grid(gx, mblocks);
+    if constexpr (O8 < 6) {
+        MTBC_ENSURE_DYN_LDS((&conv3x3_igemm_c8_kernel<MT, 0, true, 4, O8>), 160 * 1024);
+        if (f16) { hipLaunchKernelGGL((conv3x3_igemm_c8_kernel<MT, 0, true, 4, O8>), grid, dim3(256), lds, st, p); MTBC_CHECK_LAUNCH(); return MTBC_OK; }
+    } else if (f16) return MTBC_E_UNSUPPORTED;
+    MTBC_ENSURE_DYN_LDS((&conv3x3_igemm_c8_kernel<MT, 0, false, 4, O8>), 160 * 1024);
+    hipLaunchKernelGGL((conv3x3_igemm_c8_kernel<MT, 0, false, 4, O8>), grid, dim3(256), lds, st, p);
+    MTBC_CHECK_LAUNCH();
+    return MTBC_OK;
+}
+template <int O8>
+int launch_igemm_c8_pair_mt(int MT, const ConvP& p, int mblocks, bool f16, hipStream_t st) {
+    if (MT == 1) return launch_igemm_c8_pair<1, O8>(p, mblocks, f16, st);
+    if (MT == 3) return launch_igemm_c8_pair<3, O8>(p, mblocks, f16, st);
+    return launch_igemm_c8_pair<2, O8>(p, mblocks, f16, st);
+}
+
 template <int MT, int GEO, int O8>
 int launch_igemm_c8_ring(const ConvP& p, int mblocks, bool f16, hipStream_t st) {
     constexpr int R = 3;
@@ -3777,6 +3865,77 @@
     return q.geo == 2 ? 1 : q.tiles_x * q.tiles_y * (q.nw8 ? 8 : 4);
 }
 
+static bool pair_eligible(const mtbc_conv3x3_args* c, const mtbc_instnorm_args* n, IgemmPlan* plan) {
+    if (check_conv(c) || !n) return false;
+    if (c->operand_layout != MTBC_LAYOUT_C8 || (c->compute != 1 && c->compute != 2) || !c->w_packed || !c->dout) return false;
+    if (c->n_in != 1 || c->in[0].accumulate != 0 || !c->in[0].ptr || c->in[0].channels != c->Cin || c->Cin % 8 || c->Cout % 8) return false;
+    const mtbc_seg g{const_cast<float*>(c->dout), (int64_t)c->Cout * c->H * c->W, c->Cout, 0};
+    if (!c8_segs_ok(&g, 1) || !mfma_ok(c->in, 1, c->H, c->W)) return false;
+    if (n->N != c->N || n->C != c->Cin || n->H != c->H || n->W != c->W) return false;
+    if (n->z_layout != MTBC_LAYOUT_C8 || n->dy_layout != MTBC_LAYOUT_PLANAR || !n->z || !n->dz8 || !n->mean || !n->rstd) return false;
+    if (n->dy != c->in[0].ptr || n->dy_batch_stride != c->in[0].batch_stride) return false;
+    if (n->n_dy_extra != 0 || n->dy_rank1 || n->dy_rank1_w || n->dy_pool || n->dy_pool_arg || n->stats_partial || n->dz16 || n->y16) return false;
+    if (n->out16_type != c->compute || (n->z_type != 0 && !(n->z_type == 2 && c->compute == 1))) return false;
+    if ((n->gamma == nullptr) != (n->beta == nullptr)) return false;
+    if ((reinterpret_cast<uintptr_t>(n->z) | reinterpret_cast<uintptr_t>(n->dz8) | reinterpret_cast<uintptr_t>(n->mean) | reinterpret_cast<uintptr_t>(n->rstd) |
+         reinterpret_cast<uintptr_t>(n->gamma) | reinterpret_cast<uintptr_t>(n->beta)) & 15) return false;
+    if ((n->dgamma || n->dbeta || n->dbias_pre) && !n->defer_dparams) return false;
+    {
+        const uintptr_t d0 = reinterpret_cast<uintptr_t>(c->dout), d1 = d0 + (size_t)c->N * c->Cout * c->H * c->W * 2;
+        const uintptr_t o0 = reinterpret_cast<uintptr_t>(n->dz8), o1 = o0 + (size_t)n->N * n->C * n->H * n->W * 2;
+        if (o0 < d1 && d0 < o1) return false;
+    }
+    *plan = plan_igemm(c->N, c->H, c->W, c->Cin, c->compute, true, false, c->Cout);
+    return !plan->ring && plan->geo == 0 && !plan->nw8;
+}
+constexpr int PAIR_PARAM_FLOATS = 131;
+
+size_t mtbc_conv3x3_dgrad_normbwd_pair_workspace(const mtbc_conv3x3_args* c, const mtbc_instnorm_args* n) {
+    IgemmPlan q;
+    if (!pair_eligible(c, n, &q)) return 0;
+    const size_t planes = (size_t)n->N * n->C, slots = (size_t)q.tiles_x * q.tiles_y * 4;
+    return (planes * (PAIR_PARAM_FLOATS + 2) + (size_t)n->N * slots * n->C * 2) * sizeof(float);
+}
+
+int mtbc_i_conv3x3_dgrad_normbwd_pair(const mtbc_conv3x3_args* c, const mtbc_instnorm_args* n, void* stream, bool* fused) {
+    *fused = false;
+    IgemmPlan q;
+    if (!pair_eligible(c, n, &q)) return MTBC_OK;
+    const size_t need = mtbc_conv3x3_dgrad_normbwd_pair_workspace(c, n);
+    if (!n->workspace || n->workspace_bytes < need || (reinterpret_cast<uintptr_t>(n->workspace) & 15)) return MTBC_OK;
+    const bool want = n->dgamma || n->dbeta || n->dbias_pre;
+    int T = 0;
+    if (want) { T = mtbc_i_instnorm_bwd_c8_team(n); if (T < 1 || T > PAIR_PARAM_FLOATS - 3) return MTBC_OK; }
+    hipStream_t st = (hipStream_t)stream;
+    const size_t planes = (size_t)n->N * n->C;
+    const int slots = q.tiles_x * q.tiles_y * 4, HW = c->H * c->W;
+    float* ws = reinterpret_cast<float*>(n->workspace);
+    float* m12 = ws + planes * PAIR_PARAM_FLOATS;
+    float* part = m12 + planes * 2;
+    ConvP p;
+#ifdef MTBC_PROBES
+    p.ts = nullptr;
+#endif
+    const mtbc_seg g{const_cast<float*>(c->dout), (int64_t)c->Cout * HW, c->Cout, 0};
+    const mtbc_seg o{reinterpret_cast<float*>(n->dz8), (int64_t)n->C * HW, n->C, 3};
+    int rc = make_segtable(&g, 1, c->Cout, &p.in); if (rc) return rc;
+    rc = make_segtable(&o, 1, n->C, &p.out); if (rc) return rc;
+    p.N = c->N; p.H = c->H; p.W = c->W; p.Cin = c->Cout; p.Cout = c->Cin; p.wp = c->w_packed; p.bias = nullptr; p.dbg = 0;
+    p.mtiles = q.mtiles; p.tiles_x = q.tiles_x; p.tiles_y = q.tiles_y; p.ntiles = q.ntiles;
+    p.nz = reinterpret_cast<const unsigned short*>(n->z); p.nmean = n->mean; p.nrstd = n->rstd; p.ngamma = n->gamma; p.nbeta = n->beta; p.nslope = n->slope;
+    const bool f16 = c->compute == 2, zf16 = c->compute == 1 && n->z_type == 2;
+    p.stats = part; p.extra = nullptr;
+    rc = zf16 ? launch_igemm_c8_pair_mt<6>(q.MT, p, q.mblocks, f16, st) : launch_igemm_c8_pair_mt<4>(q.MT, p, q.mblocks, f16, st);
+    if (rc) return rc;
+    rc = mtbc_i_instnorm_bstats_finalize(part, slots, n->N, n->C, HW, m12, want ? ws : nullptr, T, st);
+    if (rc) return rc;
+    p.stats = nullptr; p.extra = m12;
+    rc = zf16 ? launch_igemm_c8_pair_mt<7>(q.MT, p, q.mblocks, f16, st) : launch_igemm_c8_pair_mt<5>(q.MT, p, q.mblocks, f16, st);
+    if (rc) return rc;
+    *fused = true;
+    return MTBC_OK;
+}
+
 size_t mtbc_conv3x3_wgrad_workspace(const mtbc_conv3x3_args* a) {
     if (check_conv(a)) return 0;
     WgPlan w = plan_wgrad(a);
diff --git a/multi_task_breast_cancer_amd/csrc/norm_coop.hip b/multi_task_breast_cancer_amd/csrc/norm_coop.hip
--- a/multi_task_breast_cancer_amd/csrc/norm_coop.hip
+++ b/multi_task_breast_cancer_amd/csrc/norm_coop.hip
@@ -612,6 +612,25 @@
         if (dparam_part) { dparam_part[3 * plane] = (float)s1; dparam_part[3 * plane + 1] = (float)s2; dparam_part[3 * plane + 2] = 0.f; }
     }
 }
+__global__ __launch_bounds__(256) void in_bstats_finalize_wide_kernel(const float* __restrict__ part, int slots, int C, int HW, float* __restrict__ m12,
+                                                                      float* __restrict__ dparam_part, int planes, int T) {
+    __shared__ double red[2][4];
+    const int plane = blockIdx.x, tid = threadIdx.x, lane = tid & 63, wv = tid >> 6;
+    const int n = plane / C, c = plane % C;
+    const float* q = part + ((size_t)n * slots * C + c) * 2;
+    double s1 = 0.0, s2 = 0.0;
+    for (int t = tid; t < slots; t += 256) { const float2 v = *reinterpret_cast<const float2*>(q + (size_t)t * C * 2); s1 += (double)v.x; s2 += (double)v.y; }
+    s1 = wave_sum_d(s1); s2 = wave_sum_d(s2);
+    if (lane == 0) { red[0][wv] = s1; red[1][wv] = s2; }
+    __syncthreads();
+    if (tid == 0) {
+        s1 = ((red[0][0] + red[0][1]) + red[0][2]) + red[0][3]; s2 = ((red[1][0] + red[1][1]) + red[1][2]) + red[1][3];
+        m12[2 * plane] = (float)(s1 / (double)HW); m12[2 * plane + 1] = (float)(s2 / (double)HW);
+        if (dparam_part) { dparam_part[3 * plane] = (float)s1; dparam_part[3 * plane + 1] = (float)s2; dparam_part[3 * plane + 2] = 0.f; }
+    }
+    if (dparam_part)
+        for (int m = tid; m < T; m += 256) dparam_part[(size_t)3 * planes + (size_t)plane * T + m] = 0.f;
+}
 template <bool F16, bool ZF16>
 __global__ __launch_bounds__(AP_THREADS) void in_apply_bwd_c8_kernel(const CoP p, const float* __restrict__ m12) {
     const int item = blockIdx.y, n = item / p.G8, g = item % p.G8;
@@ -879,6 +898,12 @@
     const CoPlan pl = plan_team<true>(a->N * (a->C / 8), a->H * a->W, var_of(a), a->coop_reserve_cus);
     return pl.ok ? pl.T : 0;
 }
+int mtbc_i_instnorm_bstats_finalize(const float* part, int slots, int N, int C, int HW, float* m12, float* dparam_part, int T, hipStream_t st) {
+    const int planes = N * C;
+    hipLaunchKernelGGL(in_bstats_finalize_wide_kernel, dim3(planes), dim3(256), 0, st, part, slots, C, HW, m12, dparam_part, planes, T);
+    MTBC_CHECK_LAUNCH();
+    return MTBC_OK;
+}
 int mtbc_i_instnorm_bwd_c8(const mtbc_instnorm_args* a, float* part, hipStream_t st, NormChoice* query) {
     CoP p; int rc = fill_coop(a, &p); if (rc) return rc;
     if ((!p.z && !p.z8) || (!p.dy && !p.r1 && !p.pg) || !p.dz8 || !p.mean || !p.rstd || (reinterpret_cast<uintptr_t>(p.dz8) & 15)) return MTBC_E_BADARG;
diff --git a/multi_task_breast_cancer_amd/csrc/program.hip b/multi_task_breast_cancer_amd/csrc/program.hip
--- a/multi_task_breast_cancer_amd/csrc/program.hip
+++ b/multi_task_breast_cancer_amd/csrc/program.hip
@@ -131,6 +131,12 @@
             if (rc != MTBC_OK) { if (failed_index) *failed_index = i; return rc; }
             if (fused) { ++i; continue; }
         }
+        if (o->kind == MTBC_OP_CONV3_DGRAD && i + 1 < first + count && ops[i + 1].kind == MTBC_OP_IN_BWD) {
+            bool fused = false;
+            rc = mtbc_i_conv3x3_dgrad_normbwd_pair(&o->u.conv3, &ops[i + 1].u.inorm, stream, &fused);
+            if (rc != MTBC_OK) { if (failed_index) *failed_index = i; return rc; }
+            if (fused) { ++i; continue; }
+        }
         switch (o->kind) {
             case MTBC_OP_CONV3_FWD: rc = mtbc_conv3x3_fwd(&o->u.conv3, stream); break;
             case MTBC_OP_CONV3_DGRAD: rc = mtbc_conv3x3_dgrad(&o->u.conv3, stream); break;
diff --git a/multi_task_breast_cancer_amd/engine.py b/multi_task_breast_cancer_amd/engine.py
--- a/multi_task_breast_cancer_amd/engine.py
+++ b/multi_task_breast_cancer_amd/engine.py
@@ -21,6 +21,7 @@
 _DA16 = _sw.flag("MTBC_DA16")
 _COOP_MIN_FWD, _COOP_MIN_BWD = 16384, 65536
 _IN_KERNEL_SPLITK = False
+_PAIR_MIN_HW = 65536
 _DPARAM_BATCH = 12
 
 
@@ -539,7 +540,16 @@
                     break
 
         def dz8_buffer() -> torch.Tensor:
-            return self.alloc(N * cout * H * W, dtype=torch.int16) if defer else self._scratch16("_dz8_buf", N * cout * H * W)
+            if defer:
+                return self.alloc(N * cout * H * W, dtype=torch.int16)
+            buf = self._scratch16("_dz8_buf", N * cout * H * W)
+            prev = self.bwd_ops[-1] if self.bwd_ops else None
+            if prev is not None and prev.kind == L.OP_CONV3_DGRAD and _PAIR_MIN_HW is not None and H * W >= _PAIR_MIN_HW:
+                c3 = prev.u.conv3
+                d0 = int(c3.dout or 0)
+                if d0 < buf.data_ptr() + buf.numel() * 2 and buf.data_ptr() < d0 + c3.N * c3.Cout * c3.H * c3.W * 2:
+                    buf = self._scratch16("_dz8_buf_b", N * cout * H * W)
+            return buf
 
         coop = z16 or (c8_bwd and not _NO_COOP and H * W >= _COOP_MIN_BWD and bool(self.lib.mtbc_instnorm_c8_supported(C.byref(a), 1)))
         dz8 = dz16 = None
@@ -565,11 +575,27 @@
             self._need_ws(op, "inorm", N * cout * (131 if coop else 3) * 4)
         if y.r1 is not None:
             self._need_ws(op, "inorm", N * (cout + 1) * 262 * 4)
+        pair_bytes = 0
+        prev = self.bwd_ops[-1] if self.bwd_ops else None
+        if prev is not None and prev.kind == L.OP_CONV3_DGRAD and coop and self.dev.type == "cuda":
+            a.defer_dparams = 1 if (gname or bname) else 0
+            pair_bytes = int(self.lib.mtbc_conv3x3_dgrad_normbwd_pair_workspace(C.byref(prev.u.conv3), C.byref(a)))
+            a.defer_dparams = 0
+        want_pair = pair_bytes > 0 and not _sw.ab_flag("MTBC_NO_DGRAD_NORM_PAIR") and _PAIR_MIN_HW is not None and H * W >= _PAIR_MIN_HW
+        if want_pair and not (gname or bname):
+            buf = self.alloc((pair_bytes + 3) // 4)
+            a.workspace, a.workspace_bytes = buf.data_ptr(), buf.numel() * 4
         dop = None
         if (gname or bname) and z16 and self.dev.type == "cuda":
             if a.accumulate_dparams:
                 self.flush_dparams()
-            buf = self.alloc(N * (cout + 1) * 262)
+            nfl = N * (cout + 1) * 262
+            if want_pair:
+                nfl = max(nfl, (pair_bytes + 3) // 4)
+            elif pair_bytes and nfl * 4 >= pair_bytes:
+                nfl = N * cout * (3 + int(self.lib.mtbc_instnorm_bwd_team(C.byref(a))))
+                assert 0 < nfl * 4 < pair_bytes
+            buf = self.alloc(nfl)
             self.ws_users = [u for u in self.ws_users if u[0] is not op]
             a.workspace, a.workspace_bytes, a.defer_dparams = buf.data_ptr(), buf.numel() * 4, 1
             dop = _mk(L.OP_IN_DPARAM, cell.tag)
diff --git a/multi_task_breast_cancer_amd/switches.py b/multi_task_breast_cancer_amd/switches.py
--- a/multi_task_breast_cancer_amd/switches.py
+++ b/multi_task_breast_cancer_amd/switches.py
@@ -35,6 +35,12 @@
     "MTBC_COOP_RESERVE_CUS": ("64", "CUs kept out of the cooperative InstanceNorm grids under data parallel",
                               "tests/test_coop_safety_gpu.py::test_cooperative_step_beside_a_cu_hogging_kernel"),
 }
+AB_SWITCHES: Dict[str, tuple] = {
+    "MTBC_NO_DGRAD_NORM_PAIR": ("0", "no InstanceNorm backward op gets the workspace of the runner's dgrad + norm-backward pair (mtbc_conv3x3_dgrad_normbwd_pair_workspace): "
+                                     "every cell-internal dgrad writes its fp32 planar dy and the cooperative norm backward reads it back -- the two launches "
+                                     "of before the pair, the A arm of tools/dgrad_norm_pair_cost.py and of the step A/B",
+                                "tests/test_dgrad_norm_pair_gpu.py::test_step_program_with_and_without_the_pair"),
+}
 REMOVED = ("MTBC_NO_C8", "MTBC_NO_CT_LP", "MTBC_COOP_MIN_FWD", "MTBC_COOP_MIN_BWD", "MTBC_NO_P16", "MTBC_FANIN", "MTBC_NO_C8_SMALL_OPS", "MTBC_NO_X16",
            "MTBC_NO_G16", "MTBC_NO_EPI_STATS", "MTBC_EPI_BSTATS", "MTBC_NO_R1", "MTBC_NO_POOLFOLD", "MTBC_SPLIT_FANIN", "MTBC_NO_STEM16",
            "MTBC_NO_DEFER_DPARAM", "MTBC_DPARAM_BATCH", "MTBC_NO_POOLFWD_FOLD", "MTBC_BWD_OVERLAP", "MTBC_BWD_OVERLAP_MAX_HW",
@@ -53,6 +59,10 @@
 def flag(name: str) -> bool:
     v = get(name)
     return v not in ("", "0")
+
+
+def ab_flag(name: str) -> bool:
+    return os.environ.get(name, AB_SWITCHES[name][0]) not in ("", "0")
 
 
 def active() -> Dict[str, str]:
```
